# amazon-science/instruct-video-to-video

Hardware: AMD Instinct MI355X
Metric: denoised video-frames/sec (16f@256x384, 50 DDIM steps) (higher is better)
Workload: dtype fp16; 1 GPU; C2: 1 clip/step = VAE-encode + 50 DDIM steps (3-way CFG, text 7.5 / video 1.5) + VAE-decode, 16 frames @ 256x384, random-init full-width UNet+VAE; 5 independent clips in flight per GPU (stacked into every UNet launch, B = 3 x clips); frames=16, height=256, width=384, ddim_steps=50, clips_per_gpu=5, parallelism=clip-parallel x1, one all_gather, hip_graph=True, cfg_branch_streams=False, concurrent_clips=5, clip_mode=stacked, driver_mode=False, full=False

## Files before the change

### include/insv2v_hip.h

```cpp
#ifndef INSV2V_HIP_H
#define INSV2V_HIP_H

#include <stdint.h>

#ifdef __cplusplus
extern "C" {
#endif

typedef void* insv2v_stream_t;

#define INSV2V_OK 0
#define INSV2V_EINVAL (-1)
#define INSV2V_EUNSUPPORTED (-2)

#define INSV2V_ACT_NONE 0
#define INSV2V_ACT_SILU 1
#define INSV2V_ACT_GEGLU 2
#define INSV2V_ACT_QUICK_GELU 3

#define INSV2V_ACT_RELU 4
#define INSV2V_ACT_SIGMOID 5
#define INSV2V_ACT_TANH 6

#define INSV2V_MODE_LINEAR 0
#define INSV2V_MODE_CONV3X3 1

int insv2v_abi_version(void);
int insv2v_init(void);

typedef struct insv2v_gemm_desc {
    const void* a;
    const void* a2;
    const void* w;
    void* c;
    const float* bias;
    const float* row_bias;
    const void* residual;
    const float* row_stats;
    const float* col_sum;
    int64_t lda, lda2, ldw, ldc, ldr, ld_rb;
    int64_t a_bs, w_bs, c_bs, r_bs;
    void* workspace;
    int64_t workspace_bytes;
    int32_t M, N, K;
    int32_t k_split;
    int32_t rows_per_group;
    int32_t rb_mod;
    int32_t act;
    int32_t c_fp32;
    int32_t mode;
    int32_t NB, IH, IW, OH, OW, Cin;
    int32_t stride, pad_t, pad_l, upsample;
    int32_t batch;
    int32_t tile;
    int32_t split_k;
    float alpha;
    const float* gn_ab;
    int32_t gn_images_per_sample;
    int32_t gn_silu;
    float* stats_out;
    float* stats_scratch;
    int32_t stats_parts;
    float ln_eps;
    int64_t w_group_stride;
    int32_t w_group_rows;
    int32_t reserved0;
} insv2v_gemm_desc;
int insv2v_gemm(const insv2v_gemm_desc* d, insv2v_stream_t stream);
int64_t insv2v_set_operand_window(int64_t bytes);
int insv2v_gemm_stats_parts(const insv2v_gemm_desc* d);
int insv2v_conv3x3_fuses_groupnorm(const insv2v_gemm_desc* d);

typedef struct insv2v_winograd_in_desc {
    const void* x;
    const void* x2;
    const float* gn_ab;
    void* v;
    int64_t ldx, ldx2;
    int64_t v_group_rows;
    int32_t NB, H, W, C, C1;
    int32_t gn_images_per_sample;
    int32_t gn_silu;
    int32_t upsample;
} insv2v_winograd_in_desc;
int insv2v_winograd_input(const insv2v_winograd_in_desc* d, insv2v_stream_t stream);
typedef struct insv2v_winograd_out_desc {
    const void* m;
    const float* bias;
    const float* row_bias;
    const void* residual;
    void* y;
    int64_t m_group_rows;
    int64_t ldr, ldy, ld_rb;
    int32_t NB, H, W, Cout;
    int32_t rows_per_group;
    int32_t upsample;
} insv2v_winograd_out_desc;
int insv2v_winograd_output(const insv2v_winograd_out_desc* d, insv2v_stream_t stream);

typedef struct insv2v_ffn_desc {
    const void* x;
    void* out;
    const void* wstream;
    int64_t ldx, ldo;
    int32_t M, C, hidden;
    float eps;
    const void* post_residual;
    int64_t ld_post;
    int32_t post;
} insv2v_ffn_desc;
int insv2v_ffn_fused(const insv2v_ffn_desc* d, insv2v_stream_t stream);
int64_t insv2v_ffn_stream_elems(int32_t C, int32_t hidden, int32_t post);

typedef struct insv2v_rowlin_desc {
    const void* x;
    void* out;
    const void* residual;
    const void* wstream;
    int64_t ldx, ldo, ldr;
    int32_t M, N, K;
    int32_t layernorm, frame_bias, rows_per_frame, frames;
    float eps;
    float* stats_out;
    float stats_eps;
    const float* gn_ab;
    int32_t gn_rows;
} insv2v_rowlin_desc;
int insv2v_rowlin(const insv2v_rowlin_desc* d, insv2v_stream_t stream);
int64_t insv2v_rowlin_stream_elems(int32_t N, int32_t K);

typedef struct insv2v_tattn_desc {
    const void* x;
    void* out;
    const void* wstream;
    int64_t ldx, ldo;
    int32_t samples, HW, C, heads, frames;
    float eps;
    float scale;
} insv2v_tattn_desc;
int insv2v_tattn_fused(const insv2v_tattn_desc* d, insv2v_stream_t stream);
int64_t insv2v_tattn_stream_elems(int32_t C, int32_t heads, int32_t frames);
int insv2v_tattn_attn(const insv2v_tattn_desc* d, insv2v_stream_t stream);
int64_t insv2v_tattn_attn_stream_elems(int32_t C, int32_t heads, int32_t frames);

typedef struct insv2v_xattn_desc {
    const void* x;
    void* out;
    const void* wstream;
    const void* kvstream;
    int64_t ldx, ldo;
    int32_t M, rows_per_sample, C, heads, ctx_len;
    float eps;
    float scale;
    const void* pre_residual;
    int64_t ld_pre;
} insv2v_xattn_desc;
int insv2v_xattn_fused(const insv2v_xattn_desc* d, insv2v_stream_t stream);
int64_t insv2v_xattn_stream_elems(int32_t C, int32_t heads, int32_t per_sample_kv);
int insv2v_xattn_attn(const insv2v_xattn_desc* d, insv2v_stream_t stream);
int64_t insv2v_xattn_attn_stream_elems(int32_t C, int32_t heads, int32_t per_sample_kv);

typedef struct insv2v_groupnorm_desc {
    const void* x;
    const void* x2;
    void* y;
    const float* gamma;
    const float* beta;
    float* partials;
    int64_t ldx, ldx2, ldy;
    int32_t nsamples, rows_per_sample, C, C1, G;
    int32_t nchunks;
    int32_t silu;
    float eps;
    float* ab;
    int32_t stats_only;
} insv2v_groupnorm_desc;
int insv2v_groupnorm(const insv2v_groupnorm_desc* d, insv2v_stream_t stream);

typedef struct insv2v_layernorm_desc {
    const void* x;
    void* y;
    const float* gamma;
    const float* beta;
    const float* pe;
    int64_t ldx, ldy;
    int32_t rows, C;
    int32_t rows_per_frame, frames, pe_start;
    float eps;
} insv2v_layernorm_desc;
int insv2v_layernorm(const insv2v_layernorm_desc* d, insv2v_stream_t stream);
int insv2v_layernorm_stats(const void* x, float* stats, int64_t ldx, int32_t rows, int32_t C, float eps,
                           insv2v_stream_t stream);

typedef struct insv2v_attention_desc {
    const void* q;
    const void* k;
    const void* v;
    void* o;
    int64_t q_rs, k_rs, v_rs, o_rs;
    int64_t q_outer, q_step, kv_outer, kv_step, o_outer, o_step;
    int32_t q_inner, kv_inner, o_inner;
    int32_t batch, heads, head_dim, seq_q, seq_k;
    float scale;
    int32_t causal;
    const void* q_bias;
    const void* k_bias;
    const void* v_bias;
    int64_t bias_rs;
} insv2v_attention_desc;
int insv2v_attention(const insv2v_attention_desc* d, insv2v_stream_t stream);

int insv2v_embed_tokens(const int64_t* ids, const void* tok, const void* pos, void* out, int32_t rows, int32_t L,
                        int32_t C, int32_t vocab, insv2v_stream_t stream);

int insv2v_softmax_rows(const void* x, void* y, int64_t ldx, int64_t ldy, int32_t rows, int32_t cols,
                        float scale, insv2v_stream_t stream);
int insv2v_softmax_rows_padded(const void* x, void* y, int64_t ldx, int64_t ldy, int32_t rows, int32_t cols, int32_t valid,
                               float scale, insv2v_stream_t stream);

int insv2v_timestep_embedding(const float* t, void* out, int32_t batch, int32_t dim, float shift,
                              insv2v_stream_t stream);

int insv2v_tap_gather(const float* y9, int64_t ld9, const float* bias, float* out, int64_t ldo, int32_t NB, int32_t H, int32_t W,
                      int32_t cout, insv2v_stream_t stream);

int insv2v_build_unet_input(const float* latent, const float* img_cond, void* out, float* t_out,
                            float timestep, int32_t nbranch, int32_t F, int32_t h, int32_t w, int32_t ldo,
                            int64_t branch_rows, int32_t t_stride, insv2v_stream_t stream);

typedef struct insv2v_step_desc {
    const float* eps_in;
    const float* latent;
    const float* latent_ref;
    const float* delta_q;
    const float* noise;
    const float* rescale_stats;
    float* latent_out;
    float* pred_x0;
    float* eps_out;
    int32_t nbranch, F, h, w, R;
    int32_t correct;
    float text_cfg, img_cfg;
    float sqrt_a, sqrt_1ma;
    float c_x0, c_eps, c_xt, c_noise;
    float guidance_rescale;
    int64_t branch_stride;
    int64_t noise_seed, noise_stream;
    int32_t noise_on;
} insv2v_step_desc;
int insv2v_cfg_step(const insv2v_step_desc* d, insv2v_stream_t stream);
typedef struct insv2v_mstep_desc {
    const float* eps_in;
    const float* latent;
    const float* latent_ref;
    const float* delta_q;
    const float* noise;
    const float* rescale_stats;
    float* latent_out;
    float* pred_x0;
    float* eps_out;
    int32_t nbranch, F, h, w, R;
    int32_t correct;
    float text_cfg, img_cfg;
    float sqrt_a, sqrt_1ma;
    float c_x0, c_eps, c_xt, c_noise;
    float guidance_rescale;
    int64_t branch_stride;
    int64_t noise_seed, noise_stream;
    int32_t noise_on;
    const float* x0_hist;
    float c_hist;
} insv2v_mstep_desc;
int insv2v_cfg_step_ms(const insv2v_mstep_desc* d, insv2v_stream_t stream);
int insv2v_cfg_stats(const float* eps_in, float* stats, int32_t F, int32_t h, int32_t w, float text_cfg,
                     float img_cfg, int64_t branch_stride, insv2v_stream_t stream);

int insv2v_warp_image(const float* image, const float* flow, float* out, int32_t N, int32_t C, int32_t H,
                      int32_t W, insv2v_stream_t stream);
int insv2v_resize_flow(const float* flow, float* out, int32_t N, int32_t h, int32_t w, int32_t H, int32_t W,
                       insv2v_stream_t stream);
int insv2v_flow_correction(const float* eps_cfg, const float* latent, const float* latent_ref,
                           const float* flows, float* delta_q, int32_t F, int32_t R, int32_t h, int32_t w,
                           float sqrt_a, float sqrt_1ma, insv2v_stream_t stream);

int insv2v_nchw_to_nhwc_f16(const float* x, void* y, int32_t N, int32_t C, int32_t H, int32_t W, int32_t ldo,
                            float scale, insv2v_stream_t stream);
int insv2v_nhwc_to_nchw_f32(const void* x, int32_t x_is_fp32, float* y, int32_t N, int32_t C, int32_t H,
                            int32_t W, int32_t ldx, float scale, insv2v_stream_t stream);
int insv2v_posterior_sample(const float* moments, const float* noise, float* z, int32_t N, int32_t H,
                            int32_t W, int32_t ldm, float scale, insv2v_stream_t stream);
int insv2v_posterior_sample_seeded(const float* moments, float* z, int32_t N, int32_t H, int32_t W, int32_t ldm, float scale,
                                   int64_t seed, int64_t stream, int64_t offset, insv2v_stream_t hip_stream);

int insv2v_randn(float* out, int64_t n, int64_t seed, int64_t stream, int64_t offset, int32_t raw, insv2v_stream_t hip_stream);

typedef struct insv2v_im2col_desc {
    const void* x;
    const void* x2;
    void* out;
    int64_t ldx, ldx2, ldo;
    int32_t N, IH, IW, C, C1, KH, KW, stride_h, stride_w, pad_h, pad_w, OH, OW;
} insv2v_im2col_desc;
int insv2v_im2col(const insv2v_im2col_desc* d, insv2v_stream_t stream);
int insv2v_instance_norm(const void* x, void* y, float* partials, int32_t N, int32_t HW, int32_t C, int64_t ldx, int64_t ldy,
                         int32_t nchunks, float eps, int32_t relu, insv2v_stream_t stream);
#define INSV2V_EW_RELU 1
#define INSV2V_EW_ADD_RELU 2
#define INSV2V_EW_TANH 3
#define INSV2V_EW_GRU_RH 4
#define INSV2V_EW_GRU_OUT 5
int insv2v_ew(int32_t op, const void* a, const void* b, const void* c, void* out, int64_t rows, int32_t C, int64_t lda, int64_t ldb,
              int64_t ldc, int64_t ldo, insv2v_stream_t stream);
int insv2v_avgpool2x2(const float* x, float* y, int64_t n, int32_t h, int32_t w, insv2v_stream_t stream);
typedef struct insv2v_corr_lookup_desc {
    const float* pyr0;
    const float* pyr1;
    const float* pyr2;
    const float* pyr3;
    const float* coords;
    void* out;
    int64_t ldo;
    int32_t B, h, w, levels, radius;
} insv2v_corr_lookup_desc;
int insv2v_corr_lookup(const insv2v_corr_lookup_desc* d, insv2v_stream_t stream);
int insv2v_raft_flow_rows(float* coords1, const float* delta, int64_t ldd, void* rows, int64_t ldf, int32_t ncols, int32_t B, int32_t h,
                          int32_t w, insv2v_stream_t stream);
int insv2v_convex_upsample(const float* coords1, const void* mask, int64_t ldm, float* out, int32_t B, int32_t h, int32_t w,
                           insv2v_stream_t stream);

#ifdef __cplusplus
}
#endif
#endif
```

### instruct-video-to-video_amd/build.py

```python
#!/usr/bin/env python3
import os
import subprocess
import sys
from concurrent.futures import ThreadPoolExecutor

HERE = os.path.dirname(os.path.abspath(__file__))
CSRC = os.path.join(HERE, "csrc")
OUT = os.path.join(HERE, "insv2v", "libinsv2v_hip.so")
SOURCES = ["gemm.hip", "gemm_q8.hip", "gemm_r8.hip", "gemm_w4.hip", "rows_ffn.hip", "rows_tattn.hip", "rows_xattn.hip", "norm.hip", "attention.hip", "elementwise.hip", "raft.hip", "winograd.hip"]
FLAGS = ["--offload-arch=gfx950", "-O3", "-std=c++17", "-fPIC", "-Wall", "-Wno-unused-function"]
EXTRA_FLAGS = {src: ["-fno-slp-vectorize"] for src in ("gemm_q8.hip", "gemm_r8.hip", "gemm_w4.hip", "rows_ffn.hip", "rows_tattn.hip", "rows_xattn.hip")}


def _newer(a, b):
    return not os.path.exists(b) or os.path.getmtime(a) > os.path.getmtime(b)


def build(force=False, verbose=True):
    hipcc = os.environ.get("HIPCC", "/opt/rocm/bin/hipcc")
    objdir = os.path.join(HERE, "build")
    os.makedirs(objdir, exist_ok=True)
    deps = [os.path.join(CSRC, "common.h"), os.path.join(CSRC, "gemm_dma.h"), os.path.join(CSRC, "rows_common.h"), os.path.join(CSRC, "rng.h"), os.path.join(HERE, "..", "include", "insv2v_hip.h")]
    jobs = []
    for src in SOURCES:
        s, o = os.path.join(CSRC, src), os.path.join(objdir, src + ".o")
        if force or _newer(s, o) or any(_newer(d, o) for d in deps):
            jobs.append([hipcc, *FLAGS, *EXTRA_FLAGS.get(src, []), "-c", s, "-o", o])
    def run(cmd):
        if verbose:
            print(" ".join(cmd), flush=True)
        subprocess.check_call(cmd)
    with ThreadPoolExecutor(max_workers=4) as ex:
        list(ex.map(run, jobs))
    objs = [os.path.join(objdir, s + ".o") for s in SOURCES]
    if jobs or not os.path.exists(OUT) or any(_newer(o, OUT) for o in objs):
        run([hipcc, "--offload-arch=gfx950", "-shared", "-fPIC", *objs, "-o", OUT])
    return OUT


if __name__ == "__main__":
    print(build(force="--force" in sys.argv))
```

### instruct-video-to-video_amd/csrc/norm.hip

```cpp
#include "common.h"
#include <cstdlib>

struct Moments {
    float n, mean, m2;
};
__device__ __forceinline__ Moments merge(Moments a, Moments b) {
    if (b.n == 0.f) return a;
    if (a.n == 0.f) return b;
    Moments r;
    r.n = a.n + b.n;
    float d = b.mean - a.mean;
    r.mean = a.mean + d * (b.n / r.n);
    r.m2 = a.m2 + b.m2 + d * d * (a.n * b.n / r.n);
    return r;
}

__device__ __forceinline__ half8 load8(const half_t* x, const half_t* x2, int64_t ldx, int64_t ldx2, int C1,
                                       int64_t row, int c0) {
    const half_t* p = (c0 < C1) ? x + row * ldx + c0 : x2 + row * ldx2 + (c0 - C1);
    return *(const half8*)p;
}

__global__ void gn_partial_kernel(insv2v_groupnorm_desc p, int CC, int P, int rows_per_chunk) {
    extern __shared__ __attribute__((aligned(16))) char smem[];
    Moments* sm = (Moments*)smem;
    const int tid = threadIdx.x, cc = tid % CC, pl = tid / CC;
    const int sample = blockIdx.y, chunk = blockIdx.x;
    const int C1 = p.x2 ? p.C1 : p.C;
    const half_t* x = (const half_t*)p.x;
    const half_t* x2 = (const half_t*)p.x2;
    const int64_t row0 = (int64_t)sample * p.rows_per_sample;
    const int r0 = chunk * rows_per_chunk;
    const int r1 = min(r0 + rows_per_chunk, p.rows_per_sample);
    const int c0 = cc * 8;

    half8 kv = load8(x, x2, p.ldx, p.ldx2, C1, row0, c0);
    float k[8], s[8], q[8];
#pragma unroll
    for (int e = 0; e < 8; ++e) { k[e] = (float)kv[e]; s[e] = 0.f; q[e] = 0.f; }
    int cnt = 0;
    int r = r0 + pl;
    for (; r + 3 * P < r1; r += 4 * P) {
        half8 v[4];
#pragma unroll
        for (int u = 0; u < 4; ++u) v[u] = load8(x, x2, p.ldx, p.ldx2, C1, row0 + r + u * P, c0);
#pragma unroll
        for (int u = 0; u < 4; ++u)
#pragma unroll
            for (int e = 0; e < 8; ++e) {
                float d = (float)v[u][e] - k[e];
                s[e] += d;
                q[e] += d * d;
            }
        cnt += 4;
    }
    for (; r < r1; r += P) {
        half8 v = load8(x, x2, p.ldx, p.ldx2, C1, row0 + r, c0);
#pragma unroll
        for (int e = 0; e < 8; ++e) {
            float d = (float)v[e] - k[e];
            s[e] += d;
            q[e] += d * d;
        }
        ++cnt;
    }
#pragma unroll
    for (int e = 0; e < 8; ++e) {
        Moments m;
        m.n = (float)cnt;
        float inv = cnt ? 1.f / cnt : 0.f;
        m.mean = k[e] + s[e] * inv;
        m.m2 = fmaxf(q[e] - s[e] * s[e] * inv, 0.f);
        sm[pl * p.C + c0 + e] = m;
    }
    __syncthreads();
    for (int c = tid; c < p.C; c += blockDim.x) {
        Moments m = sm[c];
        for (int j = 1; j < P; ++j) m = merge(m, sm[j * p.C + c]);
        sm[c] = m;
    }
    __syncthreads();
    const int cpg = p.C / p.G;
    for (int g = tid; g < p.G; g += blockDim.x) {
        Moments m = sm[g * cpg];
        for (int j = 1; j < cpg; ++j) m = merge(m, sm[g * cpg + j]);
        float* out = p.partials + (int64_t)p.nsamples * p.G * 2 +
                     (((int64_t)sample * p.nchunks + chunk) * p.G + g) * 3;
        out[0] = m.n;
        out[1] = m.mean;
        out[2] = m.m2;
    }
}

__global__ __launch_bounds__(256) void gn_finalize_kernel(insv2v_groupnorm_desc p) {
    const int lane = threadIdx.x & 63, wid = threadIdx.x >> 6;
    const int sample = blockIdx.y, g = blockIdx.x * 4 + wid;
    if (g >= p.G) return;
    const float* in = p.partials + (int64_t)p.nsamples * p.G * 2 + ((int64_t)sample * p.nchunks * p.G + g) * 3;
    Moments m = {0.f, 0.f, 0.f};
    for (int c = lane; c < p.nchunks; c += 64) {
        const float* q = in + (int64_t)c * p.G * 3;
        Moments b = {q[0], q[1], q[2]};
        m = merge(m, b);
    }
#pragma unroll
    for (int o = 32; o > 0; o >>= 1) {
        Moments b = {__shfl_xor(m.n, o, 64), __shfl_xor(m.mean, o, 64), __shfl_xor(m.m2, o, 64)};
        m = merge(m, b);
    }
    if (lane == 0) {
        float var = m.m2 / m.n;
        p.partials[((int64_t)sample * p.G + g) * 2 + 0] = m.mean;
        p.partials[((int64_t)sample * p.G + g) * 2 + 1] = rsqrtf(var + p.eps);
    }
    if (p.ab) {
        const float mean = m.mean, rstd = rsqrtf(m.m2 / m.n + p.eps);
        const int cpg = p.C / p.G;
        for (int c = lane; c < cpg; c += 64) {
            const int ch = g * cpg + c;
            const float a = rstd * p.gamma[ch];
            p.ab[((int64_t)sample * p.C + ch) * 2 + 0] = a;
            p.ab[((int64_t)sample * p.C + ch) * 2 + 1] = p.beta[ch] - mean * a;
        }
    }
}

__global__ void gn_apply_kernel(insv2v_groupnorm_desc p, int CC, int P) {
    const int tid = threadIdx.x, cc = tid % CC, pl = tid / CC;
    const int sample = blockIdx.y;
    const int C1 = p.x2 ? p.C1 : p.C;
    const half_t* x = (const half_t*)p.x;
    const half_t* x2 = (const half_t*)p.x2;
    half_t* y = (half_t*)p.y;
    const int64_t row0 = (int64_t)sample * p.rows_per_sample;
    const int c0 = cc * 8, cpg = p.C / p.G;
    float a[8], b[8];
#pragma unroll
    for (int e = 0; e < 8; ++e) {
        int c = c0 + e, g = c / cpg;
        float mean = p.partials[((int64_t)sample * p.G + g) * 2 + 0];
        float rstd = p.partials[((int64_t)sample * p.G + g) * 2 + 1];
        a[e] = rstd * p.gamma[c];
        b[e] = p.beta[c] - mean * a[e];
    }
    const int step = gridDim.x * P;
    int r = blockIdx.x * P + pl;
    auto finish = [&](half8 v, int row) {
        half8 o;
#pragma unroll
        for (int e = 0; e < 8; ++e) {
            float t = (float)v[e] * a[e] + b[e];
            if (p.silu) t = silu_f(t);
            o[e] = (half_t)t;
        }
        *(half8*)(y + (row0 + row) * p.ldy + c0) = o;
    };
    for (; r + 3 * step < p.rows_per_sample; r += 4 * step) {
        half8 v[4];
#pragma unroll
        for (int u = 0; u < 4; ++u) v[u] = load8(x, x2, p.ldx, p.ldx2, C1, row0 + r + u * step, c0);
#pragma unroll
        for (int u = 0; u < 4; ++u) finish(v[u], r + u * step);
    }
    for (; r < p.rows_per_sample; r += step) finish(load8(x, x2, p.ldx, p.ldx2, C1, row0 + r, c0), r);
}

#define GNS_MAXCH 16
template <int VW>
__global__ __launch_bounds__(256) void gn_small_kernel(insv2v_groupnorm_desc p) {
    typedef half_t vec_t __attribute__((ext_vector_type(VW)));
    __shared__ float red[8];
    __shared__ float sgam[256], sbet[256];
    const int tid = threadIdx.x, lane = tid & 63, wid = tid >> 6;
    const int g = blockIdx.x, sample = blockIdx.y;
    const int cpg = p.C / p.G, cpr = cpg / VW;
    const int nchunk = p.rows_per_sample * cpr;
    const int C1 = p.x2 ? p.C1 : p.C;
    const half_t* x = (const half_t*)p.x;
    const half_t* x2 = (const half_t*)p.x2;
    const int64_t row0 = (int64_t)sample * p.rows_per_sample;
    if (tid < cpg) { sgam[tid] = p.gamma[g * cpg + tid]; sbet[tid] = p.beta[g * cpg + tid]; }
    vec_t v[GNS_MAXCH];
    float s = 0.f;
    const int rs = tid < nchunk ? tid / cpr : 0, cs = tid < nchunk ? tid - rs * cpr : 0;
    const int dr = 256 / cpr, dc = 256 - dr * cpr;
    int rr = rs, cc = cs;
#pragma unroll
    for (int i = 0; i < GNS_MAXCH; ++i) {
        const bool ok = tid + 256 * i < nchunk;
        const int r = ok ? rr : rs, c0 = g * cpg + (ok ? cc : cs) * VW;
        const half_t* src = c0 < C1 ? x + (row0 + r) * p.ldx + c0 : x2 + (row0 + r) * p.ldx2 + (c0 - C1);
        v[i] = *(const vec_t*)src;
        rr += dr; cc += dc;
        if (cc >= cpr) { cc -= cpr; ++rr; }
    }
#pragma unroll
    for (int i = 0; i < GNS_MAXCH; ++i) {
        if (tid + 256 * i >= nchunk) {
#pragma unroll
            for (int e = 0; e < VW; ++e) v[i][e] = (half_t)0.f;
        }
#pragma unroll
        for (int e = 0; e < VW; ++e) s += (float)v[i][e];
    }
    s = wave_sum(s);
    if (lane == 0) red[wid] = s;
    __syncthreads();
    const float n = (float)p.rows_per_sample * cpg;
    const float mean = (red[0] + red[1] + red[2] + red[3]) / n;
    float q = 0.f;
#pragma unroll
    for (int i = 0; i < GNS_MAXCH; ++i) {
        if (tid + 256 * i < nchunk) {
#pragma unroll
            for (int e = 0; e < VW; ++e) {
                const float d = (float)v[i][e] - mean;
                q += d * d;
            }
        }
    }
    q = wave_sum(q);
    if (lane == 0) red[4 + wid] = q;
    __syncthreads();
    const float rstd = rsqrtf((red[4] + red[5] + red[6] + red[7]) / n + p.eps);
    half_t* y = (half_t*)p.y;
    rr = rs; cc = cs;
#pragma unroll
    for (int i = 0; i < GNS_MAXCH; ++i) {
        const int idx = tid + 256 * i;
        const int r = rr, c0 = g * cpg + cc * VW;
        rr += dr; cc += dc;
        if (cc >= cpr) { cc -= cpr; ++rr; }
        if (idx < nchunk) {
            vec_t o;
#pragma unroll
            for (int e = 0; e < VW; ++e) {
                float t = ((float)v[i][e] - mean) * rstd * sgam[c0 - g * cpg + e] + sbet[c0 - g * cpg + e];
                if (p.silu) t = silu_f(t);
                o[e] = (half_t)t;
            }
            *(vec_t*)(y + (row0 + r) * p.ldy + c0) = o;
        }
    }
}

#define GNF_MAXCH 15
template <int NT>
__global__ __launch_bounds__(NT) void gn_frame_kernel(insv2v_groupnorm_desc p) {
    extern __shared__ __attribute__((aligned(16))) char smem[];
    const int tid = threadIdx.x;
    const int sample = blockIdx.x;
    const int CS = gridDim.y, Cw = p.C / CS, Gw = p.G / CS, coff = blockIdx.y * Cw;
    const int crow = Cw >> 3;
    const int cpr = (p.C / p.G) >> 3;
    const int nchunk = p.rows_per_sample * crow;
    float* part = (float*)smem;
    float* gstat = part + nchunk;
    float* sgam = gstat + 2 * Gw;
    float* sbet = sgam + Cw;
    for (int c = tid; c < Cw; c += NT) { sgam[c] = p.gamma[coff + c]; sbet[c] = p.beta[coff + c]; }
    const half_t* x = (const half_t*)p.x + (int64_t)sample * p.rows_per_sample * p.ldx + coff;
    half_t* y = (half_t*)p.y + (int64_t)sample * p.rows_per_sample * p.ldy + coff;
    const int r0 = tid / crow, c0 = tid - r0 * crow;
    const int dr = NT / crow, dc = NT - dr * crow;
    half8 v[GNF_MAXCH];
    {
        int rr = r0, cc = c0;
#pragma unroll
        for (int i = 0; i < GNF_MAXCH; ++i) {
            const bool ok = tid + NT * i < nchunk;
            v[i] = *(const half8*)(x + (int64_t)(ok ? rr : r0) * p.ldx + (ok ? cc : c0) * 8);
            rr += dr; cc += dc;
            if (cc >= crow) { cc -= crow; ++rr; }
        }
    }
    const int TPG = NT / Gw;
    const int rg = tid / TPG, rp = tid - rg * TPG;
    const int ng = p.rows_per_sample * cpr;
    const float inv_n = 1.f / ((float)p.rows_per_sample * (float)(p.C / p.G));
    auto group_total = [&]() {
        float s = 0.f;
        for (int e = rp; e < ng; e += TPG) {
            const int r = e / cpr, j = e - r * cpr;
            s += part[r * crow + rg * cpr + j];
        }
        for (int o = TPG >> 1; o > 0; o >>= 1) s += __shfl_xor(s, o, 64);
        return s;
    };
#pragma unroll
    for (int i = 0; i < GNF_MAXCH; ++i) {
        if (tid + NT * i < nchunk) {
            float s = 0.f;
#pragma unroll
            for (int e = 0; e < 8; ++e) s += (float)v[i][e];
            part[tid + NT * i] = s;
        }
    }
    __syncthreads();
    {
        const float m = group_total() * inv_n;
        if (rp == 0) gstat[rg] = m;
    }
    __syncthreads();
    {
        int cc = c0;
#pragma unroll
        for (int i = 0; i < GNF_MAXCH; ++i) {
            if (tid + NT * i < nchunk) {
                const float m = gstat[cc / cpr];
                float q = 0.f;
#pragma unroll
                for (int e = 0; e < 8; ++e) { const float d = (float)v[i][e] - m; q = fmaf(d, d, q); }
                part[tid + NT * i] = q;
            }
            cc += dc;
            if (cc >= crow) cc -= crow;
        }
    }
    __syncthreads();
    {
        const float var = group_total() * inv_n;
        if (rp == 0) gstat[Gw + rg] = rsqrtf(var + p.eps);
    }
    __syncthreads();
    {
        int rr = r0, cc = c0;
#pragma unroll
        for (int i = 0; i < GNF_MAXCH; ++i) {
            if (tid + NT * i < nchunk) {
                const int g = cc / cpr;
                const float m = gstat[g], rs = gstat[Gw + g];
                half8 o;
#pragma unroll
                for (int e = 0; e < 8; ++e) {
                    float t = ((float)v[i][e] - m) * rs * sgam[cc * 8 + e] + sbet[cc * 8 + e];
                    if (p.silu) t = silu_f(t);
                    o[e] = (half_t)t;
                }
                *(half8*)(y + (int64_t)rr * p.ldy + cc * 8) = o;
            }
            rr += dr; cc += dc;
            if (cc >= crow) { cc -= crow; ++rr; }
        }
    }
}

template <int NT>
static int launch_gn_frame(const insv2v_groupnorm_desc& d, hipStream_t s, int CS = 1) {
    const size_t lds = ((size_t)d.rows_per_sample * (d.C / CS / 8) + 2 * (d.G / CS) + 2 * (d.C / CS)) * sizeof(float);
    static bool attr_set = false;
    if (!attr_set) {
        hipError_t e = hipFuncSetAttribute((const void*)gn_frame_kernel<NT>, hipFuncAttributeMaxDynamicSharedMemorySize, 96 * 1024);
        if (e != hipSuccess) return (int)e;
        attr_set = true;
    }
    if (lds > 96 * 1024) return INSV2V_EUNSUPPORTED;
    hipLaunchKernelGGL(gn_frame_kernel<NT>, dim3(d.nsamples, CS), dim3(NT), lds, s, d);
    return launch_status();
}

extern "C" int insv2v_groupnorm(const insv2v_groupnorm_desc* dp, insv2v_stream_t stream) {
    if (!one_device()) return INSV2V_EINVAL;
    if (!dp) return INSV2V_EINVAL;
    insv2v_groupnorm_desc d = *dp;
    if (!d.x || !d.gamma || !d.beta || !d.partials) return INSV2V_EINVAL;
    if (d.stats_only ? !d.ab : !d.y) return INSV2V_EINVAL;
    if (d.C <= 0 || d.G <= 0 || (d.C % d.G) || (d.C & 7) || d.C > 8192) return INSV2V_EINVAL;
    if ((d.ldx & 7) || (d.ldy & 7) || d.nsamples <= 0 || d.rows_per_sample <= 0) return INSV2V_EINVAL;
    if (d.x2 && ((d.C1 & 7) || d.C1 <= 0 || d.C1 >= d.C || (d.ldx2 & 7))) return INSV2V_EINVAL;
    if (d.nchunks <= 0) return INSV2V_EINVAL;
    hipStream_t s = as_stream(stream);
    {
        static const int frame_on = getenv("INSV2V_GN_FRAME") ? atoi(getenv("INSV2V_GN_FRAME")) : 1;
        const int cpg = d.C / d.G;
        const int64_t nchunk = (int64_t)d.rows_per_sample * (d.C / 8);
        if (frame_on && !d.stats_only && !d.ab && !d.x2 && (cpg % 8) == 0 && d.nsamples >= 128 && nchunk >= 2048 && nchunk <= 1024 * GNF_MAXCH &&
            (d.G == 32 || d.G == 16) && d.C <= 2560) {
            static const int split_env = getenv("INSV2V_GN_FRAME_SPLIT") ? atoi(getenv("INSV2V_GN_FRAME_SPLIT")) : 0;
            int CS = split_env > 0 ? split_env : (nchunk > 512 * GNF_MAXCH ? 4 : nchunk > 256 * GNF_MAXCH ? 2 : 1);
            while (CS > 1 && (d.G % CS || nchunk / CS < 1024)) CS >>= 1;
            const int64_t nc = nchunk / CS;
            const int rc = nc <= 256 * GNF_MAXCH ? launch_gn_frame<256>(d, s, CS) : nc <= 512 * GNF_MAXCH ? launch_gn_frame<512>(d, s, CS) : launch_gn_frame<1024>(d, s, CS);
            if (rc != INSV2V_EUNSUPPORTED) return rc;
        }
    }
    {
        const int cpg = d.C / d.G;
        const int vw = (cpg % 8 == 0) ? 8 : ((cpg % 4 == 0) ? 4 : 0);
        const bool src_ok = !d.x2 || (d.C1 % (vw ? vw : 1) == 0);
        if (!d.stats_only && !d.ab && vw && cpg >= 16 && cpg <= 256 && src_ok && (int64_t)d.rows_per_sample * (cpg / vw) <= 256 * GNS_MAXCH) {
            if (vw == 8) hipLaunchKernelGGL(gn_small_kernel<8>, dim3(d.G, d.nsamples), dim3(256), 0, s, d);
            else hipLaunchKernelGGL(gn_small_kernel<4>, dim3(d.G, d.nsamples), dim3(256), 0, s, d);
            return launch_status();
        }
    }
    const int CC = d.C / 8;
    if (CC > 1024) return INSV2V_EUNSUPPORTED;
    int P = 256 / CC;
    if (P < 1) P = 1;
    if (P > 16) P = 16;
    const int threads = CC * P;
    int nchunks = d.nchunks;
    if (nchunks > d.rows_per_sample) nchunks = d.rows_per_sample;
    d.nchunks = nchunks;
    const int rows_per_chunk = (d.rows_per_sample + nchunks - 1) / nchunks;
    size_t lds = (size_t)P * d.C * sizeof(Moments);
    if (lds > 64 * 1024) return INSV2V_EUNSUPPORTED;
    hipLaunchKernelGGL(gn_partial_kernel, dim3(nchunks, d.nsamples), dim3(threads), lds, s, d, CC, P, rows_per_chunk);
    hipLaunchKernelGGL(gn_finalize_kernel, dim3((d.G + 3) / 4, d.nsamples), dim3(256), 0, s, d);
    if (d.stats_only) return launch_status();
    long want = ((long)d.rows_per_sample + P * 4 - 1) / (P * 4);
    long cap = 4096 / d.nsamples;
    if (cap < 1) cap = 1;
    int gx = (int)(want < cap ? want : cap);
    hipLaunchKernelGGL(gn_apply_kernel, dim3(gx, d.nsamples), dim3(threads), 0, s, d, CC, P);
    return launch_status();
}

#define LN_MAXCH 4
#define LN_ROWS 4
template <int NCH>
__global__ __launch_bounds__(256) void layernorm_kernel(insv2v_layernorm_desc p) {
    const int lane = threadIdx.x & 63, wid = threadIdx.x >> 6;
    const int row0 = (blockIdx.x * 4 + wid) * LN_ROWS;
    if (row0 >= p.rows) return;
    const int CC = p.C >> 3;
    half8 v[LN_ROWS][NCH];
#pragma unroll
    for (int r = 0; r < LN_ROWS; ++r) {
        const int row = min(row0 + r, p.rows - 1);
        const half_t* x = (const half_t*)p.x + (int64_t)row * p.ldx;
#pragma unroll
        for (int i = 0; i < NCH; ++i) {
            const int ch = lane + 64 * i;
            const half8 z = {0, 0, 0, 0, 0, 0, 0, 0};
            const half8 t = *(const half8*)(x + (ch < CC ? ch : 0) * 8);
            v[r][i] = ch < CC ? t : z;
        }
    }
    float mean[LN_ROWS], rstd[LN_ROWS];
#pragma unroll
    for (int r = 0; r < LN_ROWS; ++r) {
        float s = 0.f;
#pragma unroll
        for (int i = 0; i < NCH; ++i)
#pragma unroll
            for (int e = 0; e < 8; ++e) s += (float)v[r][i][e];
        mean[r] = s;
    }
#pragma unroll
    for (int o = 32; o > 0; o >>= 1)
#pragma unroll
        for (int r = 0; r < LN_ROWS; ++r) mean[r] += __shfl_xor(mean[r], o, 64);
#pragma unroll
    for (int r = 0; r < LN_ROWS; ++r) {
        mean[r] /= p.C;
        float s = 0.f;
#pragma unroll
        for (int i = 0; i < NCH; ++i) {
            if (lane + 64 * i < CC) {
#pragma unroll
                for (int e = 0; e < 8; ++e) {
                    float d = (float)v[r][i][e] - mean[r];
                    s += d * d;
                }
            }
        }
        rstd[r] = s;
    }
#pragma unroll
    for (int o = 32; o > 0; o >>= 1)
#pragma unroll
        for (int r = 0; r < LN_ROWS; ++r) rstd[r] += __shfl_xor(rstd[r], o, 64);
#pragma unroll
    for (int r = 0; r < LN_ROWS; ++r) rstd[r] = rsqrtf(rstd[r] / p.C + p.eps);
#pragma unroll
    for (int i = 0; i < NCH; ++i) {
        const int ch = lane + 64 * i;
        if (ch >= CC) continue;
        float g[8], b[8];
        const float4 g0 = *(const float4*)(p.gamma + ch * 8), g1 = *(const float4*)(p.gamma + ch * 8 + 4);
        const float4 b0 = *(const float4*)(p.beta + ch * 8), b1 = *(const float4*)(p.beta + ch * 8 + 4);
        g[0] = g0.x; g[1] = g0.y; g[2] = g0.z; g[3] = g0.w; g[4] = g1.x; g[5] = g1.y; g[6] = g1.z; g[7] = g1.w;
        b[0] = b0.x; b[1] = b0.y; b[2] = b0.z; b[3] = b0.w; b[4] = b1.x; b[5] = b1.y; b[6] = b1.z; b[7] = b1.w;
#pragma unroll
        for (int r = 0; r < LN_ROWS; ++r) {
            const int row = row0 + r;
            if (row >= p.rows) break;
            const float* pe = p.pe ? p.pe + (int64_t)((row / p.rows_per_frame) % p.frames + p.pe_start) * p.C + ch * 8 : nullptr;
            half8 o;
#pragma unroll
            for (int e = 0; e < 8; ++e) {
                float t = ((float)v[r][i][e] - mean[r]) * rstd[r] * g[e] + b[e];
                if (pe) t += pe[e];
                o[e] = (half_t)t;
            }
            *(half8*)((half_t*)p.y + (int64_t)row * p.ldy + ch * 8) = o;
        }
    }
}

template <int NCH>
__global__ __launch_bounds__(256) void ln_stats_kernel(const half_t* xp, float* stats, int64_t ldx, int rows, int C, float eps) {
    const int lane = threadIdx.x & 63, wid = threadIdx.x >> 6;
    const int row0 = (blockIdx.x * 4 + wid) * LN_ROWS;
    if (row0 >= rows) return;
    const int CC = C >> 3;
    half8 v[LN_ROWS][NCH];
#pragma unroll
    for (int r = 0; r < LN_ROWS; ++r) {
        const half_t* x = xp + (int64_t)min(row0 + r, rows - 1) * ldx;
#pragma unroll
        for (int i = 0; i < NCH; ++i) {
            const int ch = lane + 64 * i;
            const half8 z = {0, 0, 0, 0, 0, 0, 0, 0};
            const half8 t = *(const half8*)(x + (ch < CC ? ch : 0) * 8);
            v[r][i] = ch < CC ? t : z;
        }
    }
    float mean[LN_ROWS], var[LN_ROWS];
#pragma unroll
    for (int r = 0; r < LN_ROWS; ++r) {
        float s = 0.f;
#pragma unroll
        for (int i = 0; i < NCH; ++i)
#pragma unroll
            for (int e = 0; e < 8; ++e) s += (float)v[r][i][e];
        mean[r] = s;
    }
#pragma unroll
    for (int o = 32; o > 0; o >>= 1)
#pragma unroll
        for (int r = 0; r < LN_ROWS; ++r) mean[r] += __shfl_xor(mean[r], o, 64);
#pragma unroll
    for (int r = 0; r < LN_ROWS; ++r) {
        mean[r] /= C;
        float s = 0.f;
#pragma unroll
        for (int i = 0; i < NCH; ++i) {
            if (lane + 64 * i < CC) {
#pragma unroll
                for (int e = 0; e < 8; ++e) {
                    const float d = (float)v[r][i][e] - mean[r];
                    s += d * d;
                }
            }
        }
        var[r] = s;
    }
#pragma unroll
    for (int o = 32; o > 0; o >>= 1)
#pragma unroll
        for (int r = 0; r < LN_ROWS; ++r) var[r] += __shfl_xor(var[r], o, 64);
    if (lane < LN_ROWS && row0 + lane < rows) {
        float m = mean[0], q = var[0];
#pragma unroll
        for (int r = 1; r < LN_ROWS; ++r)
            if (lane == r) { m = mean[r]; q = var[r]; }
        *(float2*)(stats + 2 * (int64_t)(row0 + lane)) = make_float2(m, rsqrtf(q / C + eps));
    }
}

extern "C" int insv2v_layernorm_stats(const void* x, float* stats, int64_t ldx, int32_t rows, int32_t C, float eps,
                                      insv2v_stream_t stream) {
    if (!x || !stats || rows <= 0 || (C & 7) || C <= 0 || C > 64 * 8 * LN_MAXCH || (ldx & 7)) return INSV2V_EINVAL;
    const int nch = (C / 8 + 63) / 64;
    dim3 grid((rows + 4 * LN_ROWS - 1) / (4 * LN_ROWS));
    hipStream_t s = as_stream(stream);
    const half_t* xp = (const half_t*)x;
    switch (nch) {
        case 1: hipLaunchKernelGGL(ln_stats_kernel<1>, grid, dim3(256), 0, s, xp, stats, ldx, rows, C, eps); break;
        case 2: hipLaunchKernelGGL(ln_stats_kernel<2>, grid, dim3(256), 0, s, xp, stats, ldx, rows, C, eps); break;
        case 3: hipLaunchKernelGGL(ln_stats_kernel<3>, grid, dim3(256), 0, s, xp, stats, ldx, rows, C, eps); break;
        default: hipLaunchKernelGGL(ln_stats_kernel<4>, grid, dim3(256), 0, s, xp, stats, ldx, rows, C, eps); break;
    }
    return launch_status();
}

extern "C" int insv2v_layernorm(const insv2v_layernorm_desc* dp, insv2v_stream_t stream) {
    if (!dp) return INSV2V_EINVAL;
    insv2v_layernorm_desc d = *dp;
    if (!d.x || !d.y || !d.gamma || !d.beta || d.rows <= 0) return INSV2V_EINVAL;
    if ((d.C & 7) || d.C <= 0 || d.C > 64 * 8 * LN_MAXCH || (d.ldx & 7) || (d.ldy & 7)) return INSV2V_EINVAL;
    if (d.pe && (d.rows_per_frame <= 0 || d.frames <= 0 || d.pe_start < 0)) return INSV2V_EINVAL;
    const int nch = (d.C / 8 + 63) / 64;
    dim3 grid((d.rows + 4 * LN_ROWS - 1) / (4 * LN_ROWS));
    hipStream_t s = as_stream(stream);
    switch (nch) {
        case 1: hipLaunchKernelGGL(layernorm_kernel<1>, grid, dim3(256), 0, s, d); break;
        case 2: hipLaunchKernelGGL(layernorm_kernel<2>, grid, dim3(256), 0, s, d); break;
        case 3: hipLaunchKernelGGL(layernorm_kernel<3>, grid, dim3(256), 0, s, d); break;
        default: hipLaunchKernelGGL(layernorm_kernel<4>, grid, dim3(256), 0, s, d); break;
    }
    return launch_status();
}

template <bool PAD>
__global__ __launch_bounds__(256) void softmax_rows_kernel(const half_t* x, half_t* y, int64_t ldx, int64_t ldy,
                                                           int cols, int valid, float scale) {
    __shared__ float red[8];
    const int row = blockIdx.x, tid = threadIdx.x, lane = tid & 63, wid = tid >> 6;
    const half_t* xr = x + (int64_t)row * ldx;
    half_t* yr = y + (int64_t)row * ldy;
    const int CC = cols >> 3;
    float mx = -3.0e38f;
    for (int ch = tid; ch < CC; ch += 256) {
        half8 v = *(const half8*)(xr + ch * 8);
#pragma unroll
        for (int e = 0; e < 8; ++e)
            if (!PAD || ch * 8 + e < valid) mx = fmaxf(mx, (float)v[e]);
    }
    mx = wave_max(mx);
    if (lane == 0) red[wid] = mx;
    __syncthreads();
    mx = fmaxf(fmaxf(red[0], red[1]), fmaxf(red[2], red[3]));
    const float c = scale * 1.4426950408889634f;
    float sum = 0.f;
    for (int ch = tid; ch < CC; ch += 256) {
        half8 v = *(const half8*)(xr + ch * 8);
#pragma unroll
        for (int e = 0; e < 8; ++e)
            if (!PAD || ch * 8 + e < valid) sum += exp2f(((float)v[e] - mx) * c);
    }
    sum = wave_sum(sum);
    if (lane == 0) red[4 + wid] = sum;
    __syncthreads();
    const float inv = 1.f / (red[4] + red[5] + red[6] + red[7]);
    for (int ch = tid; ch < CC; ch += 256) {
        half8 v = *(const half8*)(xr + ch * 8);
        half8 o;
#pragma unroll
        for (int e = 0; e < 8; ++e) o[e] = (!PAD || ch * 8 + e < valid) ? (half_t)(exp2f(((float)v[e] - mx) * c) * inv) : (half_t)0.f;
        *(half8*)(yr + ch * 8) = o;
    }
}

extern "C" int insv2v_softmax_rows(const void* x, void* y, int64_t ldx, int64_t ldy, int32_t rows, int32_t cols,
                                   float scale, insv2v_stream_t stream) {
    if (!x || !y || rows <= 0 || cols <= 0 || (cols & 7) || (ldx & 7) || (ldy & 7)) return INSV2V_EINVAL;
    if (scale < 0.f) return INSV2V_EINVAL;
    hipLaunchKernelGGL(softmax_rows_kernel<false>, dim3(rows), dim3(256), 0, as_stream(stream), (const half_t*)x,
                       (half_t*)y, ldx, ldy, cols, cols, scale);
    return launch_status();
}

extern "C" int insv2v_softmax_rows_padded(const void* x, void* y, int64_t ldx, int64_t ldy, int32_t rows, int32_t cols, int32_t valid,
                                          float scale, insv2v_stream_t stream) {
    if (!x || !y || rows <= 0 || cols <= 0 || (cols & 7) || (ldx & 7) || (ldy & 7) || ldx < cols || ldy < cols) return INSV2V_EINVAL;
    if (valid <= 0 || valid > cols || scale < 0.f) return INSV2V_EINVAL;
    hipLaunchKernelGGL(softmax_rows_kernel<true>, dim3(rows), dim3(256), 0, as_stream(stream), (const half_t*)x,
                       (half_t*)y, ldx, ldy, cols, valid, scale);
    return launch_status();
}
```

### instruct-video-to-video_amd/csrc/winograd.hip

```cpp
#include "common.h"

namespace {

template <bool UP> __device__ __forceinline__ int lds_px(int sp) { return UP ? sp : sp ^ ((sp >> 1) & 1); }

template <bool NORM, bool UP>
__global__ __launch_bounds__(256) void wino_input_kernel(const half_t* __restrict__ x, const half_t* __restrict__ x2, const float* __restrict__ ab,
                                                         half_t* __restrict__ V, int64_t ldx, int64_t ldx2, int C1, int C, int NB, int H, int W,
                                                         int ipb, int images_per_sample, int silu, int64_t group_rows, int band_tr) {
    extern __shared__ __attribute__((aligned(16))) char smem[];
    const int tid = threadIdx.x, chunk = tid & 7, item0 = tid >> 3;
    const int nb0 = (int)blockIdx.x * ipb, c0 = (int)blockIdx.y * 64;
    const int trows = UP ? H : (H + 1) >> 1;
    const int tr0 = (int)blockIdx.z * band_tr, tr1 = min(tr0 + band_tr, trows);
    const bool whole = band_tr >= trows;
    const int row0 = whole ? 0 : (UP ? tr0 - 1 : 2 * tr0 - 1);
    const int nrows = whole ? H : (UP ? (tr1 - tr0) + 2 : 2 * (tr1 - tr0) + 2);
    const int HW = H * W, SW = nrows * W;
    const int SWs = UP ? SW : (SW + 1) & ~1;
    const bool second = x2 != nullptr && c0 >= C1;
    const half_t* src = second ? x2 + (c0 - C1) + chunk * 8 : x + c0 + chunk * 8;
    const int64_t ld = second ? ldx2 : ldx;
    const int nimg = min(ipb, NB - nb0);
    for (int it = item0; it < nimg * SW; it += 32) {
        const int img = it / SW, sp = it - img * SW;
        const int iy = row0 + sp / W;
        if ((unsigned)iy >= (unsigned)H) continue;
        half8 v = *(const half8*)(src + ((int64_t)(nb0 + img) * HW + sp + row0 * W) * ld);
        if (NORM) {
            const float* p = ab + ((int64_t)((nb0 + img) / images_per_sample) * C + c0 + chunk * 8) * 2;
            const float4 p0 = *(const float4*)p, p1 = *(const float4*)(p + 4), p2 = *(const float4*)(p + 8), p3 = *(const float4*)(p + 12);
            const float sc[8] = {p0.x, p0.z, p1.x, p1.z, p2.x, p2.z, p3.x, p3.z}, sh[8] = {p0.y, p0.w, p1.y, p1.w, p2.y, p2.w, p3.y, p3.w};
#pragma unroll
            for (int e = 0; e < 8; ++e) {
                float f = fmaf((float)v[e], sc[e], sh[e]);
                if (silu) f = silu_f(f);
                v[e] = (half_t)f;
            }
        }
        *(half8*)(smem + ((int64_t)img * SWs + lds_px<UP>(sp)) * 128 + chunk * 16) = v;
    }
    __syncthreads();
    if constexpr (UP) {
        const int bt = (tr1 - tr0) * W;
        for (int it = item0; it < nimg * bt; it += 32) {
            const int img = it / bt, tb_ = it - img * bt;
            const int y = tr0 + tb_ / W, xx = tb_ - (tb_ / W) * W;
            const int t = y * W + xx;
            const char* base = smem + (int64_t)img * SWs * 128 + chunk * 16;
            float hz[3][3][8];
#pragma unroll
            for (int r = 0; r < 3; ++r) {
                const int iy = y - 1 + r;
                float d[3][8];
#pragma unroll
                for (int c = 0; c < 3; ++c) {
                    const int ix = xx - 1 + c;
                    const bool ok = (unsigned)iy < (unsigned)H && (unsigned)ix < (unsigned)W;
                    half8 v = {0, 0, 0, 0, 0, 0, 0, 0};
                    if (ok) v = *(const half8*)(base + lds_px<UP>((iy - row0) * W + ix) * 128);
#pragma unroll
                    for (int e = 0; e < 8; ++e) d[c][e] = (float)v[e];
                }
#pragma unroll
                for (int e = 0; e < 8; ++e) {
                    hz[r][0][e] = d[0][e] - d[1][e];
                    hz[r][1][e] = 2.f * d[1][e];
                    hz[r][2][e] = d[1][e] - d[2][e];
                }
            }
            const int64_t trow = (int64_t)(nb0 + img) * HW + t;
            half_t* dst = V + trow * C + c0 + chunk * 8;
#pragma unroll
            for (int j = 0; j < 3; ++j) {
                half8 o[3];
#pragma unroll
                for (int e = 0; e < 8; ++e) {
                    o[0][e] = (half_t)(hz[0][j][e] - hz[1][j][e]);
                    o[1][e] = (half_t)(2.f * hz[1][j][e]);
                    o[2][e] = (half_t)(hz[1][j][e] - hz[2][j][e]);
                }
#pragma unroll
                for (int i = 0; i < 3; ++i) *(half8*)(dst + (int64_t)(i * 3 + j) * group_rows * C) = o[i];
            }
        }
        return;
    }
    const int th = (H + 1) >> 1, tw = (W + 1) >> 1, ntile = th * tw;
    const int bt = (tr1 - tr0) * tw;
    for (int it = item0; it < nimg * bt; it += 32) {
        const int img = it / bt, tb_ = it - img * bt;
        const int ty = tr0 + tb_ / tw, tx = tb_ - (tb_ / tw) * tw;
        const int t = ty * tw + tx;
        const char* base = smem + (int64_t)img * SWs * 128 + chunk * 16;
        float hz[4][4][8];
#pragma unroll
        for (int r = 0; r < 4; ++r) {
            const int iy = 2 * ty - 1 + r;
            float d[4][8];
#pragma unroll
            for (int c = 0; c < 4; ++c) {
                const int ix = 2 * tx - 1 + c;
                const bool ok = (unsigned)iy < (unsigned)H && (unsigned)ix < (unsigned)W;
                half8 v = {0, 0, 0, 0, 0, 0, 0, 0};
                if (ok) v = *(const half8*)(base + lds_px<UP>((iy - row0) * W + ix) * 128);
#pragma unroll
                for (int e = 0; e < 8; ++e) d[c][e] = (float)v[e];
            }
#pragma unroll
            for (int e = 0; e < 8; ++e) {
                hz[r][0][e] = d[0][e] - d[2][e];
                hz[r][1][e] = d[1][e] + d[2][e];
                hz[r][2][e] = d[2][e] - d[1][e];
                hz[r][3][e] = d[1][e] - d[3][e];
            }
        }
        const int64_t trow = (int64_t)(nb0 + img) * ntile + t;
        half_t* dst = V + trow * C + c0 + chunk * 8;
#pragma unroll
        for (int j = 0; j < 4; ++j) {
            half8 o[4];
#pragma unroll
            for (int e = 0; e < 8; ++e) {
                o[0][e] = (half_t)(hz[0][j][e] - hz[2][j][e]);
                o[1][e] = (half_t)(hz[1][j][e] + hz[2][j][e]);
                o[2][e] = (half_t)(hz[2][j][e] - hz[1][j][e]);
                o[3][e] = (half_t)(hz[1][j][e] - hz[3][j][e]);
            }
#pragma unroll
            for (int i = 0; i < 4; ++i) *(half8*)(dst + (int64_t)(i * 4 + j) * group_rows * C) = o[i];
        }
    }
}

template <bool RES, bool RB, bool UP>
__global__ __launch_bounds__(256) void wino_output_kernel(const half_t* __restrict__ Mo, const float* __restrict__ bias, const float* __restrict__ row_bias,
                                                          const half_t* __restrict__ res, half_t* __restrict__ y, int64_t group_rows, int64_t ntiles_total,
                                                          int Cout, int H, int W, int64_t ld_rb, int rows_per_group, int64_t ldr, int64_t ldy) {
    const int c8 = Cout >> 3;
    const int64_t idx = (int64_t)blockIdx.x * 256 + threadIdx.x;
    const int64_t tile = idx / c8;
    if (tile >= ntiles_total) return;
    const int ch = (int)(idx - tile * c8) * 8;
    const int th = UP ? H : (H + 1) >> 1, tw = UP ? W : (W + 1) >> 1, ntile = th * tw;
    const int OW = UP ? 2 * W : W, OH = UP ? 2 * H : H;
    const int nb = (int)(tile / ntile), t = (int)(tile - (int64_t)nb * ntile);
    const int ty = t / tw, tx = t - ty * tw;
    const half_t* src = Mo + tile * Cout + ch;
    float s[2][4][8];
    if constexpr (UP) {
#pragma unroll
        for (int j = 0; j < 3; ++j) {
            half8 m[3];
#pragma unroll
            for (int i = 0; i < 3; ++i) m[i] = *(const half8*)(src + (int64_t)(i * 3 + j) * group_rows * Cout);
            const int jj = j == 2 ? 3 : j;
#pragma unroll
            for (int e = 0; e < 8; ++e) {
                s[0][jj][e] = (float)m[0][e] + (float)m[1][e];
                s[1][jj][e] = (float)m[1][e] - (float)m[2][e];
            }
        }
#pragma unroll
        for (int e = 0; e < 8; ++e) s[0][2][e] = s[1][2][e] = 0.f;
    } else {
#pragma unroll
        for (int j = 0; j < 4; ++j) {
            half8 m[4];
#pragma unroll
            for (int i = 0; i < 4; ++i) m[i] = *(const half8*)(src + (int64_t)(i * 4 + j) * group_rows * Cout);
#pragma unroll
            for (int e = 0; e < 8; ++e) {
                s[0][j][e] = (float)m[0][e] + (float)m[1][e] + (float)m[2][e];
                s[1][j][e] = (float)m[1][e] - (float)m[2][e] - (float)m[3][e];
            }
        }
    }
    float b[8];
    {
        const float4 b0 = bias ? *(const float4*)(bias + ch) : make_float4(0.f, 0.f, 0.f, 0.f), b1 = bias ? *(const float4*)(bias + ch + 4) : make_float4(0.f, 0.f, 0.f, 0.f);
        b[0] = b0.x; b[1] = b0.y; b[2] = b0.z; b[3] = b0.w; b[4] = b1.x; b[5] = b1.y; b[6] = b1.z; b[7] = b1.w;
    }
    const int64_t m00 = ((int64_t)nb * OH + 2 * ty) * OW + 2 * tx;
    if (RB) {
        const float* rb = row_bias + (m00 / rows_per_group) * ld_rb + ch;
        const float4 r0 = *(const float4*)rb, r1 = *(const float4*)(rb + 4);
        b[0] += r0.x; b[1] += r0.y; b[2] += r0.z; b[3] += r0.w; b[4] += r1.x; b[5] += r1.y; b[6] += r1.z; b[7] += r1.w;
    }
#pragma unroll
    for (int i = 0; i < 2; ++i)
#pragma unroll
        for (int jj = 0; jj < 2; ++jj) {
            if (!UP && (2 * ty + i >= OH || 2 * tx + jj >= OW)) continue;
            const int64_t m = m00 + (int64_t)i * OW + jj;
            float v[8];
#pragma unroll
            for (int e = 0; e < 8; ++e)
                v[e] = (jj == 0 ? s[i][0][e] + s[i][1][e] + s[i][2][e] : s[i][1][e] - s[i][2][e] - s[i][3][e]) + b[e];
            if (RES) {
                const half8 r = *(const half8*)(res + m * ldr + ch);
#pragma unroll
                for (int e = 0; e < 8; ++e) v[e] += (float)r[e];
            }
            half8 o;
#pragma unroll
            for (int e = 0; e < 8; ++e) o[e] = (half_t)v[e];
            *(half8*)(y + m * ldy + ch) = o;
        }
}

}

extern "C" int insv2v_winograd_input(const insv2v_winograd_in_desc* dp, insv2v_stream_t stream) {
    if (!dp) return INSV2V_EINVAL;
    const insv2v_winograd_in_desc& d = *dp;
    if (!d.x || !d.v || d.NB <= 0 || d.H <= 0 || d.W <= 0 || d.C <= 0) return INSV2V_EINVAL;
    if ((d.C % 64) || (d.x2 && (d.C1 <= 0 || d.C1 >= d.C || (d.C1 % 64)))) return INSV2V_EUNSUPPORTED;
    if ((d.ldx & 7) || ((uintptr_t)d.x & 15) || ((uintptr_t)d.v & 15) || (d.x2 && ((d.ldx2 & 7) || ((uintptr_t)d.x2 & 15)))) return INSV2V_EINVAL;
    if (d.gn_ab && (d.gn_images_per_sample <= 0 || ((uintptr_t)d.gn_ab & 15))) return INSV2V_EINVAL;
    const int HW = d.H * d.W, ntile = d.upsample ? HW : ((d.H + 1) / 2) * ((d.W + 1) / 2);
    const int HWs = d.upsample ? HW : (HW + 1) & ~1;
    const int64_t tiles = (int64_t)d.NB * ntile;
    if (d.v_group_rows < tiles) return INSV2V_EINVAL;
    const int trows = d.upsample ? d.H : (d.H + 1) / 2;
    int band_tr = trows, ipb = 1;
    if (HWs * 128 <= 64 * 1024) {
        ipb = 32 / ntile;
        if (ipb < 1) ipb = 1;
        while (ipb > 1 && ipb * HWs * 128 > 64 * 1024) --ipb;
    } else {
        const int max_rows = 64 * 1024 / (d.W * 128);
        band_tr = d.upsample ? max_rows - 2 : (max_rows - 2) / 2;
        if (band_tr < 1) return INSV2V_EUNSUPPORTED;
    }
    const int nbands = (trows + band_tr - 1) / band_tr;
    const int srows = nbands == 1 ? d.H : (d.upsample ? band_tr + 2 : 2 * band_tr + 2);
    const dim3 grid((unsigned)((d.NB + ipb - 1) / ipb), (unsigned)(d.C / 64), (unsigned)nbands);
    const int slots = srows * d.W;
    const size_t lds = (size_t)ipb * (d.upsample ? slots : (slots + 1) & ~1) * 128;
#define WINO_IN(NORM, UP)                                                                                                                             \
    hipLaunchKernelGGL((wino_input_kernel<NORM, UP>), grid, dim3(256), lds, as_stream(stream), (const half_t*)d.x, (const half_t*)d.x2, d.gn_ab, (half_t*)d.v, \
                       d.ldx, d.ldx2, d.x2 ? d.C1 : d.C, d.C, d.NB, d.H, d.W, ipb, d.gn_ab ? d.gn_images_per_sample : 1, d.gn_ab ? d.gn_silu : 0, d.v_group_rows, band_tr)
    if (d.gn_ab) { if (d.upsample) WINO_IN(true, true); else WINO_IN(true, false); }
    else { if (d.upsample) WINO_IN(false, true); else WINO_IN(false, false); }
#undef WINO_IN
    return launch_status();
}

extern "C" int insv2v_winograd_output(const insv2v_winograd_out_desc* dp, insv2v_stream_t stream) {
    if (!dp) return INSV2V_EINVAL;
    const insv2v_winograd_out_desc& d = *dp;
    if (!d.m || !d.y || d.NB <= 0 || d.H <= 0 || d.W <= 0 || d.Cout <= 0) return INSV2V_EINVAL;
    if (d.Cout & 7) return INSV2V_EUNSUPPORTED;
    if ((d.ldy & 7) || ((uintptr_t)d.m & 15) || ((uintptr_t)d.y & 15) || (d.residual && ((d.ldr & 7) || ((uintptr_t)d.residual & 15)))) return INSV2V_EINVAL;
    if ((d.bias && ((uintptr_t)d.bias & 15)) || (d.row_bias && (((uintptr_t)d.row_bias & 15) || (d.ld_rb & 3) || d.rows_per_group <= 0 || d.rows_per_group % (d.H * d.W * (d.upsample ? 4 : 1)))))
        return INSV2V_EINVAL;
    const int64_t tiles = d.upsample ? (int64_t)d.NB * d.H * d.W : (int64_t)d.NB * ((d.H + 1) / 2) * ((d.W + 1) / 2);
    if (d.m_group_rows < tiles) return INSV2V_EINVAL;
    const int64_t n = tiles * (d.Cout / 8);
    const dim3 grid((unsigned)((n + 255) / 256));
#define WINO_OUT(RES, RB, UP)                                                                                                                        \
    hipLaunchKernelGGL((wino_output_kernel<RES, RB, UP>), grid, dim3(256), 0, as_stream(stream), (const half_t*)d.m, d.bias, d.row_bias, (const half_t*)d.residual, \
                       (half_t*)d.y, d.m_group_rows, tiles, d.Cout, d.H, d.W, d.ld_rb, d.rows_per_group, d.ldr, d.ldy)
    if (d.upsample) {
        if (d.residual) { if (d.row_bias) WINO_OUT(true, true, true); else WINO_OUT(true, false, true); }
        else { if (d.row_bias) WINO_OUT(false, true, true); else WINO_OUT(false, false, true); }
    } else {
        if (d.residual) { if (d.row_bias) WINO_OUT(true, true, false); else WINO_OUT(true, false, false); }
        else { if (d.row_bias) WINO_OUT(false, true, false); else WINO_OUT(false, false, false); }
    }
#undef WINO_OUT
    return launch_status();
}
```

### instruct-video-to-video_amd/insv2v/_lib.py

```python
import ctypes as C
import os

import torch

ABI_VERSION = 14
_HERE = os.path.dirname(os.path.abspath(__file__))
LIB_PATH = os.environ.get("INSV2V_LIB", os.path.join(_HERE, "libinsv2v_hip.so"))

c_i32, c_i64, c_f32, c_p = C.c_int32, C.c_int64, C.c_float, C.c_void_p


class GemmDesc(C.Structure):
    _fields_ = [("a", c_p), ("a2", c_p), ("w", c_p), ("c", c_p), ("bias", c_p), ("row_bias", c_p), ("residual", c_p),
                ("row_stats", c_p), ("col_sum", c_p),
                ("lda", c_i64), ("lda2", c_i64), ("ldw", c_i64), ("ldc", c_i64), ("ldr", c_i64), ("ld_rb", c_i64),
                ("a_bs", c_i64), ("w_bs", c_i64), ("c_bs", c_i64), ("r_bs", c_i64),
                ("workspace", c_p), ("workspace_bytes", c_i64),
                ("M", c_i32), ("N", c_i32), ("K", c_i32), ("k_split", c_i32), ("rows_per_group", c_i32),
                ("rb_mod", c_i32), ("act", c_i32), ("c_fp32", c_i32), ("mode", c_i32),
                ("NB", c_i32), ("IH", c_i32), ("IW", c_i32), ("OH", c_i32), ("OW", c_i32), ("Cin", c_i32),
                ("stride", c_i32), ("pad_t", c_i32), ("pad_l", c_i32), ("upsample", c_i32),
                ("batch", c_i32), ("tile", c_i32), ("split_k", c_i32), ("alpha", c_f32),
                ("gn_ab", c_p), ("gn_images_per_sample", c_i32), ("gn_silu", c_i32),
                ("stats_out", c_p), ("stats_scratch", c_p), ("stats_parts", c_i32), ("ln_eps", c_f32),
                ("w_group_stride", c_i64), ("w_group_rows", c_i32), ("reserved0", c_i32)]


class WinogradInDesc(C.Structure):
    _fields_ = [("x", c_p), ("x2", c_p), ("gn_ab", c_p), ("v", c_p), ("ldx", c_i64), ("ldx2", c_i64), ("v_group_rows", c_i64),
                ("NB", c_i32), ("H", c_i32), ("W", c_i32), ("C", c_i32), ("C1", c_i32), ("gn_images_per_sample", c_i32), ("gn_silu", c_i32), ("upsample", c_i32)]


class WinogradOutDesc(C.Structure):
    _fields_ = [("m", c_p), ("bias", c_p), ("row_bias", c_p), ("residual", c_p), ("y", c_p), ("m_group_rows", c_i64),
                ("ldr", c_i64), ("ldy", c_i64), ("ld_rb", c_i64), ("NB", c_i32), ("H", c_i32), ("W", c_i32), ("Cout", c_i32), ("rows_per_group", c_i32), ("upsample", c_i32)]


class FfnDesc(C.Structure):
    _fields_ = [("x", c_p), ("out", c_p), ("wstream", c_p), ("ldx", c_i64), ("ldo", c_i64),
                ("M", c_i32), ("C", c_i32), ("hidden", c_i32), ("eps", c_f32), ("post_residual", c_p), ("ld_post", c_i64), ("post", c_i32)]


class RowLinDesc(C.Structure):
    _fields_ = [("x", c_p), ("out", c_p), ("residual", c_p), ("wstream", c_p), ("ldx", c_i64), ("ldo", c_i64), ("ldr", c_i64),
                ("M", c_i32), ("N", c_i32), ("K", c_i32), ("layernorm", c_i32), ("frame_bias", c_i32), ("rows_per_frame", c_i32),
                ("frames", c_i32), ("eps", c_f32), ("stats_out", c_p), ("stats_eps", c_f32), ("gn_ab", c_p), ("gn_rows", c_i32)]


class TattnDesc(C.Structure):
    _fields_ = [("x", c_p), ("out", c_p), ("wstream", c_p), ("ldx", c_i64), ("ldo", c_i64),
                ("samples", c_i32), ("HW", c_i32), ("C", c_i32), ("heads", c_i32), ("frames", c_i32), ("eps", c_f32), ("scale", c_f32)]


class XattnDesc(C.Structure):
    _fields_ = [("x", c_p), ("out", c_p), ("wstream", c_p), ("kvstream", c_p), ("ldx", c_i64), ("ldo", c_i64),
                ("M", c_i32), ("rows_per_sample", c_i32), ("C", c_i32), ("heads", c_i32), ("ctx_len", c_i32), ("eps", c_f32), ("scale", c_f32),
                ("pre_residual", c_p), ("ld_pre", c_i64)]


class GroupNormDesc(C.Structure):
    _fields_ = [("x", c_p), ("x2", c_p), ("y", c_p), ("gamma", c_p), ("beta", c_p), ("partials", c_p),
                ("ldx", c_i64), ("ldx2", c_i64), ("ldy", c_i64),
                ("nsamples", c_i32), ("rows_per_sample", c_i32), ("C", c_i32), ("C1", c_i32), ("G", c_i32),
                ("nchunks", c_i32), ("silu", c_i32), ("eps", c_f32), ("ab", c_p), ("stats_only", c_i32)]


class LayerNormDesc(C.Structure):
    _fields_ = [("x", c_p), ("y", c_p), ("gamma", c_p), ("beta", c_p), ("pe", c_p),
                ("ldx", c_i64), ("ldy", c_i64), ("rows", c_i32), ("C", c_i32),
                ("rows_per_frame", c_i32), ("frames", c_i32), ("pe_start", c_i32), ("eps", c_f32)]


class AttentionDesc(C.Structure):
    _fields_ = [("q", c_p), ("k", c_p), ("v", c_p), ("o", c_p),
                ("q_rs", c_i64), ("k_rs", c_i64), ("v_rs", c_i64), ("o_rs", c_i64),
                ("q_outer", c_i64), ("q_step", c_i64), ("kv_outer", c_i64), ("kv_step", c_i64),
                ("o_outer", c_i64), ("o_step", c_i64),
                ("q_inner", c_i32), ("kv_inner", c_i32), ("o_inner", c_i32),
                ("batch", c_i32), ("heads", c_i32), ("head_dim", c_i32), ("seq_q", c_i32), ("seq_k", c_i32),
                ("scale", c_f32), ("causal", c_i32), ("q_bias", c_p), ("k_bias", c_p), ("v_bias", c_p), ("bias_rs", c_i64)]


class StepDesc(C.Structure):
    _fields_ = [("eps_in", c_p), ("latent", c_p), ("latent_ref", c_p), ("delta_q", c_p), ("noise", c_p),
                ("rescale_stats", c_p), ("latent_out", c_p), ("pred_x0", c_p), ("eps_out", c_p),
                ("nbranch", c_i32), ("F", c_i32), ("h", c_i32), ("w", c_i32), ("R", c_i32), ("correct", c_i32),
                ("text_cfg", c_f32), ("img_cfg", c_f32), ("sqrt_a", c_f32), ("sqrt_1ma", c_f32),
                ("c_x0", c_f32), ("c_eps", c_f32), ("c_xt", c_f32), ("c_noise", c_f32), ("guidance_rescale", c_f32),
                ("branch_stride", c_i64), ("noise_seed", c_i64), ("noise_stream", c_i64), ("noise_on", c_i32)]


class MStepDesc(C.Structure):
    _fields_ = StepDesc._fields_ + [("x0_hist", c_p), ("c_hist", c_f32)]


class Im2colDesc(C.Structure):
    _fields_ = [("x", c_p), ("x2", c_p), ("out", c_p), ("ldx", c_i64), ("ldx2", c_i64), ("ldo", c_i64),
                ("N", c_i32), ("IH", c_i32), ("IW", c_i32), ("C", c_i32), ("C1", c_i32), ("KH", c_i32), ("KW", c_i32),
                ("stride_h", c_i32), ("stride_w", c_i32), ("pad_h", c_i32), ("pad_w", c_i32), ("OH", c_i32), ("OW", c_i32)]


class CorrLookupDesc(C.Structure):
    _fields_ = [("pyr0", c_p), ("pyr1", c_p), ("pyr2", c_p), ("pyr3", c_p), ("coords", c_p), ("out", c_p), ("ldo", c_i64),
                ("B", c_i32), ("h", c_i32), ("w", c_i32), ("levels", c_i32), ("radius", c_i32)]


SIGNATURES = {
    "insv2v_abi_version": (c_i32, []),
    "insv2v_init": (c_i32, []),
    "insv2v_gemm": (c_i32, [C.POINTER(GemmDesc), c_p]),
    "insv2v_gemm_stats_parts": (c_i32, [C.POINTER(GemmDesc)]),
    "insv2v_set_operand_window": (c_i64, [c_i64]),
    "insv2v_conv3x3_fuses_groupnorm": (c_i32, [C.POINTER(GemmDesc)]),
    "insv2v_winograd_input": (c_i32, [C.POINTER(WinogradInDesc), c_p]),
    "insv2v_winograd_output": (c_i32, [C.POINTER(WinogradOutDesc), c_p]),
    "insv2v_ffn_fused": (c_i32, [C.POINTER(FfnDesc), c_p]),
    "insv2v_ffn_stream_elems": (c_i64, [c_i32, c_i32, c_i32]),
    "insv2v_rowlin": (c_i32, [C.POINTER(RowLinDesc), c_p]),
    "insv2v_rowlin_stream_elems": (c_i64, [c_i32, c_i32]),
    "insv2v_tattn_fused": (c_i32, [C.POINTER(TattnDesc), c_p]),
    "insv2v_tattn_stream_elems": (c_i64, [c_i32, c_i32, c_i32]),
    "insv2v_tattn_attn": (c_i32, [C.POINTER(TattnDesc), c_p]),
    "insv2v_tattn_attn_stream_elems": (c_i64, [c_i32, c_i32, c_i32]),
    "insv2v_xattn_fused": (c_i32, [C.POINTER(XattnDesc), c_p]),
    "insv2v_xattn_stream_elems": (c_i64, [c_i32, c_i32, c_i32]),
    "insv2v_xattn_attn": (c_i32, [C.POINTER(XattnDesc), c_p]),
    "insv2v_xattn_attn_stream_elems": (c_i64, [c_i32, c_i32, c_i32]),
    "insv2v_groupnorm": (c_i32, [C.POINTER(GroupNormDesc), c_p]),
    "insv2v_layernorm": (c_i32, [C.POINTER(LayerNormDesc), c_p]),
    "insv2v_layernorm_stats": (c_i32, [c_p, c_p, c_i64, c_i32, c_i32, c_f32, c_p]),
    "insv2v_attention": (c_i32, [C.POINTER(AttentionDesc), c_p]),
    "insv2v_embed_tokens": (c_i32, [c_p, c_p, c_p, c_p, c_i32, c_i32, c_i32, c_i32, c_p]),
    "insv2v_softmax_rows": (c_i32, [c_p, c_p, c_i64, c_i64, c_i32, c_i32, c_f32, c_p]),
    "insv2v_softmax_rows_padded": (c_i32, [c_p, c_p, c_i64, c_i64, c_i32, c_i32, c_i32, c_f32, c_p]),
    "insv2v_timestep_embedding": (c_i32, [c_p, c_p, c_i32, c_i32, c_f32, c_p]),
    "insv2v_build_unet_input": (c_i32, [c_p, c_p, c_p, c_p, c_f32, c_i32, c_i32, c_i32, c_i32, c_i32, c_i64, c_i32, c_p]),
    "insv2v_cfg_step": (c_i32, [C.POINTER(StepDesc), c_p]),
    "insv2v_cfg_step_ms": (c_i32, [C.POINTER(MStepDesc), c_p]),
    "insv2v_cfg_stats": (c_i32, [c_p, c_p, c_i32, c_i32, c_i32, c_f32, c_f32, c_i64, c_p]),
    "insv2v_warp_image": (c_i32, [c_p, c_p, c_p, c_i32, c_i32, c_i32, c_i32, c_p]),
    "insv2v_tap_gather": (c_i32, [c_p, c_i64, c_p, c_p, c_i64, c_i32, c_i32, c_i32, c_i32, c_p]),
    "insv2v_resize_flow": (c_i32, [c_p, c_p, c_i32, c_i32, c_i32, c_i32, c_i32, c_p]),
    "insv2v_flow_correction": (c_i32, [c_p, c_p, c_p, c_p, c_p, c_i32, c_i32, c_i32, c_i32, c_f32, c_f32, c_p]),
    "insv2v_nchw_to_nhwc_f16": (c_i32, [c_p, c_p, c_i32, c_i32, c_i32, c_i32, c_i32, c_f32, c_p]),
    "insv2v_nhwc_to_nchw_f32": (c_i32, [c_p, c_i32, c_p, c_i32, c_i32, c_i32, c_i32, c_i32, c_f32, c_p]),
    "insv2v_posterior_sample": (c_i32, [c_p, c_p, c_p, c_i32, c_i32, c_i32, c_i32, c_f32, c_p]),
    "insv2v_posterior_sample_seeded": (c_i32, [c_p, c_p, c_i32, c_i32, c_i32, c_i32, c_f32, c_i64, c_i64, c_i64, c_p]),
    "insv2v_randn": (c_i32, [c_p, c_i64, c_i64, c_i64, c_i64, c_i32, c_p]),
    "insv2v_im2col": (c_i32, [C.POINTER(Im2colDesc), c_p]),
    "insv2v_instance_norm": (c_i32, [c_p, c_p, c_p, c_i32, c_i32, c_i32, c_i64, c_i64, c_i32, c_f32, c_i32, c_p]),
    "insv2v_ew": (c_i32, [c_i32, c_p, c_p, c_p, c_p, c_i64, c_i32, c_i64, c_i64, c_i64, c_i64, c_p]),
    "insv2v_avgpool2x2": (c_i32, [c_p, c_p, c_i64, c_i32, c_i32, c_p]),
    "insv2v_corr_lookup": (c_i32, [C.POINTER(CorrLookupDesc), c_p]),
    "insv2v_raft_flow_rows": (c_i32, [c_p, c_p, c_i64, c_p, c_i64, c_i32, c_i32, c_i32, c_i32, c_p]),
    "insv2v_convex_upsample": (c_i32, [c_p, c_p, c_i64, c_p, c_i32, c_i32, c_i32, c_p]),
}

_lib = None


class HipKernelError(RuntimeError):
    pass


def load():
    global _lib
    if _lib is not None:
        return _lib
    if not os.path.exists(LIB_PATH):
        raise HipKernelError(
            f"{LIB_PATH} not found: build it with `python instruct-video-to-video_amd/build.py` "
            "(or __graft_entry__.build()). There is no CPU fallback for the insv2v hot path.")
    lib = C.CDLL(LIB_PATH)
    for name, (res, args) in SIGNATURES.items():
        fn = getattr(lib, name)
        fn.restype, fn.argtypes = res, args
    if lib.insv2v_abi_version() != ABI_VERSION:
        raise HipKernelError("libinsv2v_hip.so ABI version mismatch; rebuild the library")
    _lib = lib
    return lib


def check(status, what):
    if status != 0:
        kind = {-1: "invalid argument", -2: "unsupported configuration"}.get(status, f"hipError {status}")
        raise HipKernelError(f"{what}: {kind}")
```

### instruct-video-to-video_amd/insv2v/ops.py

```python
import ctypes as C

import os
import torch

from . import _lib
from .rng import as_int64
from ._lib import GemmDesc, GroupNormDesc, LayerNormDesc, AttentionDesc, StepDesc, MStepDesc, FfnDesc, RowLinDesc, TattnDesc, XattnDesc, WinogradInDesc, WinogradOutDesc, check

ACT_NONE, ACT_SILU, ACT_GEGLU, ACT_QUICK_GELU = 0, 1, 2, 3
ACT_RELU, ACT_SIGMOID, ACT_TANH = 4, 5, 6
EW_RELU, EW_ADD_RELU, EW_TANH, EW_GRU_RH, EW_GRU_OUT = 1, 2, 3, 4, 5
_byref = C.byref


def _stream():
    return torch.cuda.current_stream().cuda_stream


_REC = None


def set_launch_recorder(rec):
    global _REC
    _REC = rec
# ... 112 lines not shown
    elif row_stats is not None:
        d.row_stats = _req(row_stats, torch.float32, "gemm.row_stats").data_ptr()
        d.col_sum = _req(col_sum, torch.float32, "gemm.col_sum").data_ptr()
    d.rb_mod = rb_mod
    d.M, d.N, d.K, d.act, d.c_fp32, d.alpha, d.tile = M, N, K, act, int(out.dtype == torch.float32), alpha, tile
    d.batch, d.a_bs, d.w_bs, d.c_bs, d.r_bs = batch, a_bs, w_bs, c_bs, r_bs
    if batch == 1:
        ws = _workspace(a.device)
        d.workspace, d.workspace_bytes, d.split_k = ws.data_ptr(), ws.numel() * 4, split_k
    stats = None
    if emit_stats:
        key = (M, N, K, d.lda, d.ldc, d.ldr, residual is not None, act, tile, out.dtype, a.data_ptr() % 16, out.data_ptr() % 16, batch, split_k,
               residual.data_ptr() % 16 if residual is not None else 0,
               row_bias is not None, rows_per_group, d.ld_rb, rb_mod, a2 is not None, row_stats is not None)
        nparts = _STATS_PARTS_CACHE.get(key)
        if nparts is None:
            nparts = _STATS_PARTS_CACHE[key] = int(lib.insv2v_gemm_stats_parts(_byref(d)))
        if nparts > 0:
            stats = RowStats(torch.empty((nparts, M, 2), device=a.device, dtype=torch.float32), nparts, ln_eps)
            d.stats_out = stats.parts.data_ptr()
    with _timed("gemm_kernel", 2.0 * M * N * K * batch, ("lin", M, N, K, batch, act, residual is not None)):
        rc = lib.insv2v_gemm(_byref(d), _stream())
        if rc == -2 and stats is not None:
            stats, d.stats_out = None, None
            rc = lib.insv2v_gemm(_byref(d), _stream())
        check(rc, "insv2v_gemm")
    del scratch
    if emit_stats:
        return out, (stats if stats is not None else layernorm_stats(out, ln_eps))
    return out


def copy_rows(dst, src):
    with _timed("copy", 0.0, ("copy", src.shape[0], src.shape[1])):
        dst.copy_(src)
    return dst


def ffn_fused_supported(C, hidden):
    return int(_lib.load().insv2v_ffn_stream_elems(C, hidden, 0)) > 0


def ffn_fused(x, wstream, hidden, eps=1e-5, out=None, post_residual=None):
    lib = _lib.load()
    _req(x, torch.float16, "ffn.x"), _req(wstream, torch.float16, "ffn.wstream")
    M, C = x.shape
    if wstream.numel() != int(lib.insv2v_ffn_stream_elems(C, hidden, int(post_residual is not None))):
        raise _lib.HipKernelError(f"ffn_fused: weight stream of {wstream.numel()} halfs does not match C={C}, hidden={hidden}, post={post_residual is not None}")
    if out is None:
        out = torch.empty((M, C), device=x.device, dtype=torch.float16)
    d = FfnDesc()
    d.x, d.out, d.wstream, d.ldx, d.ldo = x.data_ptr(), out.data_ptr(), wstream.data_ptr(), x.stride(0), out.stride(0)
    d.M, d.C, d.hidden, d.eps = M, C, hidden, eps
    if post_residual is not None:
        d.post, d.post_residual, d.ld_post = 1, _req(post_residual, torch.float16, "ffn.post_residual").data_ptr(), post_residual.stride(0)
    with _timed("gemm_kernel", 2.0 * M * C * 3 * hidden + (2.0 * M * C * C if post_residual is not None else 0.0), ("ffn", M, C, hidden)):
        check(lib.insv2v_ffn_fused(_byref(d), _stream()), "insv2v_ffn_fused")
    return out


def rowlin_supported(N, K):
    return int(_lib.load().insv2v_rowlin_stream_elems(N, K)) > 0


def rowlin(x, wstream, N, *, layernorm=False, residual=None, frames=0, rows_per_frame=0, eps=1e-5, out=None, emit_stats=False, stats_eps=1e-5,
           gn_ab=None, gn_rows=0):
    lib = _lib.load()
    _req(x, torch.float16, "rowlin.x"), _req(wstream, torch.float16, "rowlin.wstream")
    M, K = x.shape
    if wstream.numel() != int(lib.insv2v_rowlin_stream_elems(N, K)):
        raise _lib.HipKernelError(f"rowlin: weight stream of {wstream.numel()} halfs does not match N={N}, K={K}")
    if out is None:
        out = torch.empty((M, N), device=x.device, dtype=torch.float16)
    d = RowLinDesc()
    d.x, d.out, d.wstream, d.ldx, d.ldo = x.data_ptr(), out.data_ptr(), wstream.data_ptr(), x.stride(0), out.stride(0)
    if residual is not None:
        d.residual, d.ldr = _req(residual, torch.float16, "rowlin.residual").data_ptr(), residual.stride(0)
    d.M, d.N, d.K, d.layernorm, d.eps = M, N, K, int(layernorm), eps
    d.frame_bias, d.rows_per_frame, d.frames = int(frames > 0), rows_per_frame, frames
    if gn_ab is not None:
        d.gn_ab, d.gn_rows = _req(gn_ab, torch.float32, "rowlin.gn_ab").data_ptr(), gn_rows
    stats = None
    if emit_stats:
        stats = torch.empty((M, 2), device=x.device, dtype=torch.float32)
        d.stats_out, d.stats_eps = stats.data_ptr(), stats_eps
    with _timed("gemm_kernel", 2.0 * M * N * K, ("rowlin", M, N, K, int(layernorm), residual is not None)):
        check(lib.insv2v_rowlin(_byref(d), _stream()), "insv2v_rowlin")
    return (out, stats) if emit_stats else out


def tattn_fused_supported(C, heads, frames):
    return int(_lib.load().insv2v_tattn_stream_elems(C, heads, frames)) > 0


def tattn_fused(x, wstream, samples, HW, heads, frames, eps=1e-5, out=None):
    lib = _lib.load()
    _req(x, torch.float16, "tattn.x"), _req(wstream, torch.float16, "tattn.wstream")
    M, C = x.shape
    if M != samples * frames * HW:
        raise _lib.HipKernelError(f"tattn_fused: {M} rows != {samples} samples x {frames} frames x {HW} pixels")
    if wstream.numel() != int(lib.insv2v_tattn_stream_elems(C, heads, frames)):
        raise _lib.HipKernelError(f"tattn_fused: weight stream of {wstream.numel()} halfs does not match C={C}, heads={heads}, frames={frames}")
    if out is None:
        out = torch.empty((M, C), device=x.device, dtype=torch.float16)
    d = TattnDesc()
    d.x, d.out, d.wstream, d.ldx, d.ldo = x.data_ptr(), out.data_ptr(), wstream.data_ptr(), x.stride(0), out.stride(0)
    d.samples, d.HW, d.C, d.heads, d.frames, d.eps, d.scale = samples, HW, C, heads, frames, eps, (C // heads) ** -0.5
    with _timed("gemm_kernel", 2.0 * M * C * 4 * C + 4.0 * M * frames * C, ("tattn", M, C, heads, frames)):
        check(lib.insv2v_tattn_fused(_byref(d), _stream()), "insv2v_tattn_fused")
    return out


def tattn_attn_supported(C, heads, frames):
    return int(_lib.load().insv2v_tattn_attn_stream_elems(C, heads, frames)) > 0


def tattn_attn(x, wstream, samples, HW, heads, frames, eps=1e-5, out=None):
    lib = _lib.load()
    _req(x, torch.float16, "tattn_attn.x"), _req(wstream, torch.float16, "tattn_attn.wstream")
    M, C = x.shape
    if M != samples * frames * HW:
        raise _lib.HipKernelError(f"tattn_attn: {M} rows != {samples} samples x {frames} frames x {HW} pixels")
    if wstream.numel() != int(lib.insv2v_tattn_attn_stream_elems(C, heads, frames)):
        raise _lib.HipKernelError(f"tattn_attn: weight stream of {wstream.numel()} halfs does not match C={C}, heads={heads}, frames={frames}")
    if out is None:
        out = torch.empty((M, C), device=x.device, dtype=torch.float16)
    d = TattnDesc()
    d.x, d.out, d.wstream, d.ldx, d.ldo = x.data_ptr(), out.data_ptr(), wstream.data_ptr(), x.stride(0), out.stride(0)
    d.samples, d.HW, d.C, d.heads, d.frames, d.eps, d.scale = samples, HW, C, heads, frames, eps, (C // heads) ** -0.5
    with _timed("gemm_kernel", 2.0 * M * C * 3 * C + 4.0 * M * frames * C, ("tattn_attn", M, C, heads, frames)):
        check(lib.insv2v_tattn_attn(_byref(d), _stream()), "insv2v_tattn_attn")
    return out


def xattn_fused_supported(C, heads, ctx_len, rows_per_sample):
    return int(_lib.load().insv2v_xattn_stream_elems(C, heads, 0)) > 0 and 64 < ctx_len <= 96 and rows_per_sample > 0


def xattn_fused(x, wstream, kvstream, rows_per_sample, heads, ctx_len, eps=1e-5, out=None, pre_residual=None):
    lib = _lib.load()
    _req(x, torch.float16, "xattn.x"), _req(wstream, torch.float16, "xattn.wstream"), _req(kvstream, torch.float16, "xattn.kvstream")
    M, C = x.shape
    if M % rows_per_sample or kvstream.shape[0] != M // rows_per_sample:
        raise _lib.HipKernelError(f"xattn_fused: {M} rows, {rows_per_sample} per sample, K/V streams of {kvstream.shape[0]} samples")
    if wstream.numel() != int(lib.insv2v_xattn_stream_elems(C, heads, 2 if pre_residual is not None else 0)) or \
            kvstream[0].numel() != int(lib.insv2v_xattn_stream_elems(C, heads, 1)):
        raise _lib.HipKernelError(f"xattn_fused: weight / K-V streams do not match C={C}, heads={heads}")
    if out is None:
        out = torch.empty((M, C), device=x.device, dtype=torch.float16)
    d = XattnDesc()
    d.x, d.out, d.wstream, d.kvstream, d.ldx, d.ldo = x.data_ptr(), out.data_ptr(), wstream.data_ptr(), kvstream.data_ptr(), x.stride(0), out.stride(0)
    d.M, d.rows_per_sample, d.C, d.heads, d.ctx_len, d.eps, d.scale = M, rows_per_sample, C, heads, ctx_len, eps, (C // heads) ** -0.5
    if pre_residual is not None:
        d.pre_residual, d.ld_pre = _req(pre_residual, torch.float16, "xattn.pre_residual").data_ptr(), pre_residual.stride(0)
    with _timed("gemm_kernel", (6.0 if pre_residual is not None else 4.0) * M * C * C + 4.0 * M * ctx_len * C, ("xattn", M, C, heads, ctx_len, pre_residual is not None)):
        check(lib.insv2v_xattn_fused(_byref(d), _stream()), "insv2v_xattn_fused")
    return out


def xattn_attn_supported(C, heads, ctx_len, rows_per_sample):
    return int(_lib.load().insv2v_xattn_attn_stream_elems(C, heads, 0)) > 0 and 64 < ctx_len <= 96 and rows_per_sample > 0


def xattn_attn(x, wstream, kvstream, rows_per_sample, heads, ctx_len, eps=1e-5, out=None):
    lib = _lib.load()
    _req(x, torch.float16, "xattn_attn.x"), _req(wstream, torch.float16, "xattn_attn.wstream"), _req(kvstream, torch.float16, "xattn_attn.kvstream")
    M, C = x.shape
    if M % rows_per_sample or kvstream.shape[0] != M // rows_per_sample:
        raise _lib.HipKernelError(f"xattn_attn: {M} rows, {rows_per_sample} per sample, K/V streams of {kvstream.shape[0]} samples")
    if wstream.numel() != int(lib.insv2v_xattn_attn_stream_elems(C, heads, 0)) or kvstream[0].numel() != int(lib.insv2v_xattn_attn_stream_elems(C, heads, 1)):
        raise _lib.HipKernelError(f"xattn_attn: weight / K-V streams do not match C={C}, heads={heads}")
    if out is None:
        out = torch.empty((M, C), device=x.device, dtype=torch.float16)
    d = XattnDesc()
    d.x, d.out, d.wstream, d.kvstream, d.ldx, d.ldo = x.data_ptr(), out.data_ptr(), wstream.data_ptr(), kvstream.data_ptr(), x.stride(0), out.stride(0)
    d.M, d.rows_per_sample, d.C, d.heads, d.ctx_len, d.eps, d.scale = M, rows_per_sample, C, heads, ctx_len, eps, (C // heads) ** -0.5
    with _timed("gemm_kernel", 2.0 * M * C * C + 4.0 * M * ctx_len * C, ("xattn_attn", M, C, heads, ctx_len)):
        check(lib.insv2v_xattn_attn(_byref(d), _stream()), "insv2v_xattn_attn")
    return out


def _conv_geometry(geom, stride, pad, upsample, out_size=None):
    NB, IH, IW = geom
    if out_size is not None:
        if not upsample:
            raise ValueError("conv3x3: out_size is the target of the nearest-x2 upsample (upsample=True)")
        return int(out_size[0]), int(out_size[1])
    IHu, IWu = (IH * 2, IW * 2) if upsample else (IH, IW)
    pt, pl = pad
    if pt == 0 and stride == 2:
        return (IHu + 1 - 3) // 2 + 1, (IWu + 1 - 3) // 2 + 1
    return (IHu + 2 * pt - 3) // stride + 1, (IWu + 2 * pl - 3) // stride + 1


_FUSE_CACHE = {}


class operand_window:

    def __init__(self, nbytes):
        self.nbytes = int(nbytes)

    def __enter__(self):
        self.prev = int(_lib.load().insv2v_set_operand_window(self.nbytes))
        _STATS_PARTS_CACHE.clear()

    def __exit__(self, *exc):
        _lib.load().insv2v_set_operand_window(self.prev)
        _STATS_PARTS_CACHE.clear()
        return False


def tap_weights(w):
    cout, cin = w.shape[:2]
    if cout > 4 or tuple(w.shape[2:]) != (3, 3):
        raise ValueError(f"tap_weights: a 3x3 convolution with <= 4 output channels, got {tuple(w.shape)}")
    wt = torch.zeros(40, cin, dtype=torch.float32)
    wt[:36].reshape(9, 4, cin)[:, :cout] = w.detach().float().cpu().permute(2, 3, 0, 1).reshape(9, cout, cin)
    return wt.half()


def conv3x3_narrow(x, geom, wtap, bias, cout):
    lib = _lib.load()
    NB, H, W = geom
    y9 = gemm(x, wtap, None, out_fp32=True)
    out = torch.empty((x.shape[0], cout), device=x.device, dtype=torch.float32)
    with _timed("elementwise", 0.0, ("tapgather", x.shape[0], cout)):
        check(lib.insv2v_tap_gather(y9.data_ptr(), y9.stride(0), _ptr(bias), out.data_ptr(), out.stride(0), NB, H, W, cout, _stream()), "insv2v_tap_gather")
    return out


def conv3x3_fuses_groupnorm(geom, cin, cout, k_split=0):
    key = (tuple(geom), cin, cout, k_split)
    if key not in _FUSE_CACHE:
        lib = _lib.load()
        NB, IH, IW = geom
        d = GemmDesc()
        d.M, d.N, d.K, d.batch, d.mode = NB * IH * IW, cout, 9 * cin, 1, 1
        d.NB, d.IH, d.IW, d.OH, d.OW, d.Cin = NB, IH, IW, IH, IW, cin
        d.stride, d.pad_t, d.pad_l, d.k_split = 1, 1, 1, k_split
        d.workspace, d.workspace_bytes = 1, WORKSPACE_BYTES
        _FUSE_CACHE[key] = bool(lib.insv2v_conv3x3_fuses_groupnorm(_byref(d)))
    return _FUSE_CACHE[key]


def conv3x3(x, geom, w, bias=None, *, x2=None, stride=1, pad=(1, 1), upsample=False, residual=None, row_bias=None,
            rows_per_group=0, out_fp32=False, tile=0, split_k=0, gn_ab=None, gn_images_per_sample=0, gn_silu=False, out=None, act=ACT_NONE,
            out_size=None):
    lib = _lib.load()
    _req(x, torch.float16, "conv.x"), _req(w, torch.float16, "conv.w")
    NB, IH, IW = geom
    pt, pl = pad
    OH, OW = _conv_geometry(geom, stride, pad, upsample, out_size)
    N = w.shape[0]
    cin = x.shape[1] + (x2.shape[1] if x2 is not None else 0)
    M = NB * OH * OW
    if out is None:
        out = torch.empty((M, N), device=x.device, dtype=torch.float32 if out_fp32 else torch.float16)
    d = GemmDesc()
    d.a, d.w, d.c = x.data_ptr(), w.data_ptr(), out.data_ptr()
    d.lda, d.ldw, d.ldc = x.stride(0), w.stride(0), out.stride(0)
    if x2 is not None:
        d.a2, d.lda2, d.k_split = _req(x2, torch.float16, "conv.x2").data_ptr(), x2.stride(0), x.shape[1]
    if bias is not None:
        d.bias = _req(bias, torch.float32, "conv.bias").data_ptr()
    if row_bias is not None:
        d.row_bias, d.ld_rb, d.rows_per_group = _req(row_bias, torch.float32, "conv.row_bias").data_ptr(), row_bias.stride(0), rows_per_group
    if residual is not None:
        d.residual, d.ldr = _req(residual, torch.float16, "conv.residual").data_ptr(), residual.stride(0)
    d.M, d.N, d.K, d.c_fp32, d.alpha, d.tile, d.batch, d.act = M, N, 9 * cin, int(out_fp32), 1.0, tile, 1, act
    d.mode, d.NB, d.IH, d.IW, d.OH, d.OW, d.Cin = 1, NB, IH, IW, OH, OW, cin
    d.stride, d.pad_t, d.pad_l, d.upsample = stride, pt, pl, int(upsample)
    if gn_ab is not None:
        d.gn_ab = _req(gn_ab, torch.float32, "conv.gn_ab").data_ptr()
        d.gn_images_per_sample, d.gn_silu = gn_images_per_sample, int(gn_silu)
    ws = _workspace(x.device)
    d.workspace, d.workspace_bytes, d.split_k = ws.data_ptr(), ws.numel() * 4, split_k
    with _timed("gemm_kernel", 2.0 * M * N * 9 * cin, ("conv", M, N, 9 * cin, stride, int(upsample), residual is not None)):
        check(lib.insv2v_gemm(_byref(d), _stream()), "insv2v_gemm(conv3x3)")
    return out, (NB, OH, OW)


def _gn_chunks(nsamples, rows_per_sample):
    return max(1, min(rows_per_sample // 32, max(1, 1024 // nsamples), 128))


_WINO_G = torch.tensor([[1.0, 0.0, 0.0], [0.5, 0.5, 0.5], [0.5, -0.5, 0.5], [0.0, 0.0, 1.0]])


def winograd_weights(w, device, upsample=False):
    u = torch.einsum("ai,ocij,bj->aboc", _WINO_G, w.float(), _WINO_G)
    if upsample:
        u = u[[0, 1, 3]][:, [0, 1, 3]]
    return u.reshape(-1, w.shape[0], w.shape[1]).to(device=device, dtype=torch.float16).contiguous()


def winograd_ok(geom, cin, c1=0, upsample=False, out_size=None):
    _, H, W = geom
    if upsample and out_size is not None and tuple(out_size) != (2 * H, 2 * W):
        return False
    return W <= 128 and cin % 64 == 0 and c1 % 64 == 0


def winograd_conv3x3(x, geom, U, bias=None, *, x2=None, gn_ab=None, gn_images_per_sample=0, gn_silu=False, row_bias=None, rows_per_group=0,
                     residual=None, out=None, tile=0, upsample=False):
    lib = _lib.load()
    _req(x, torch.float16, "winograd.x"), _req(U, torch.float16, "winograd.U")
    NB, H, W = geom
    C1 = x.shape[1]
    C = C1 + (x2.shape[1] if x2 is not None else 0)
    Cout = U.shape[1]
    ng = 9 if upsample else 16
    OH, OW = (2 * H, 2 * W) if upsample else (H, W)
    assert U.shape[0] == ng and U.shape[2] == C and x.shape[0] == NB * H * W
    tiles = NB * H * W if upsample else NB * ((H + 1) // 2) * ((W + 1) // 2)
    grows = -(-tiles // 256) * 256
    v = torch.empty((ng * grows, C), device=x.device, dtype=torch.float16)
    di = WinogradInDesc()
    di.x, di.v, di.ldx, di.v_group_rows = x.data_ptr(), v.data_ptr(), x.stride(0), grows
    if x2 is not None:
        di.x2, di.ldx2, di.C1 = _req(x2, torch.float16, "winograd.x2").data_ptr(), x2.stride(0), C1
    di.NB, di.H, di.W, di.C, di.upsample = NB, H, W, C, int(upsample)
    if gn_ab is not None:
        di.gn_ab, di.gn_images_per_sample, di.gn_silu = _req(gn_ab, torch.float32, "winograd.gn_ab").data_ptr(), gn_images_per_sample, int(gn_silu)
    with _timed("groupnorm", 0.0, ("wino_in", NB * H * W, C)):
        check(lib.insv2v_winograd_input(_byref(di), _stream()), "insv2v_winograd_input")
    m = torch.empty((ng * grows, Cout), device=x.device, dtype=torch.float16)
    d = GemmDesc()
    d.a, d.w, d.c = v.data_ptr(), U.data_ptr(), m.data_ptr()
    d.lda, d.ldw, d.ldc = C, C, Cout
    d.M, d.N, d.K, d.batch, d.alpha, d.tile = ng * grows, Cout, C, 1, 1.0, tile
    d.w_group_rows, d.w_group_stride = grows, Cout * C
    with _timed("gemm_kernel", 2.0 * NB * OH * OW * Cout * 9 * C, ("wino_gemm", ng * grows, Cout, C)):
        check(lib.insv2v_gemm(_byref(d), _stream()), "insv2v_gemm (grouped)")
    del v
    if out is None:
        out = torch.empty((NB * OH * OW, Cout), device=x.device, dtype=torch.float16)
    do = WinogradOutDesc()
    do.m, do.y, do.m_group_rows, do.ldy = m.data_ptr(), out.data_ptr(), grows, out.stride(0)
    if bias is not None:
        do.bias = _req(bias, torch.float32, "winograd.bias").data_ptr()
    if row_bias is not None:
        do.row_bias, do.ld_rb, do.rows_per_group = _req(row_bias, torch.float32, "winograd.row_bias").data_ptr(), row_bias.stride(0), rows_per_group
    if residual is not None:
        do.residual, do.ldr = _req(residual, torch.float16, "winograd.residual").data_ptr(), residual.stride(0)
    do.NB, do.H, do.W, do.Cout, do.upsample = NB, H, W, Cout, int(upsample)
    with _timed("groupnorm", 0.0, ("wino_out", NB * OH * OW, Cout)):
        check(lib.insv2v_winograd_output(_byref(do), _stream()), "insv2v_winograd_output")
    return out


def groupnorm(x, nsamples, rows_per_sample, gamma, beta, groups, eps, silu=False, x2=None):
    lib = _lib.load()
    _req(x, torch.float16, "groupnorm.x")
    C1 = x.shape[1]
    Ct = C1 + (x2.shape[1] if x2 is not None else 0)
    assert nsamples * rows_per_sample == x.shape[0]
    y = torch.empty((x.shape[0], Ct), device=x.device, dtype=torch.float16)
    nchunks = _gn_chunks(nsamples, rows_per_sample)
    scratch = torch.empty(nsamples * groups * (2 + 3 * nchunks), device=x.device, dtype=torch.float32)
    d = GroupNormDesc()
    d.x, d.y, d.gamma, d.beta, d.partials = x.data_ptr(), y.data_ptr(), gamma.data_ptr(), beta.data_ptr(), scratch.data_ptr()
    d.ldx, d.ldy = x.stride(0), y.stride(0)
    if x2 is not None:
        d.x2, d.ldx2, d.C1 = _req(x2, torch.float16, "groupnorm.x2").data_ptr(), x2.stride(0), C1
    d.nsamples, d.rows_per_sample, d.C, d.G, d.nchunks, d.silu, d.eps = nsamples, rows_per_sample, Ct, groups, nchunks, int(silu), eps
    with _timed("groupnorm", 0.0, ("gn", nsamples, rows_per_sample, Ct)):
        check(lib.insv2v_groupnorm(_byref(d), _stream()), "insv2v_groupnorm")
    return y


def groupnorm_stats(x, nsamples, rows_per_sample, gamma, beta, groups, eps, x2=None):
    lib = _lib.load()
    _req(x, torch.float16, "groupnorm.x")
    C1 = x.shape[1]
    Ct = C1 + (x2.shape[1] if x2 is not None else 0)
    assert nsamples * rows_per_sample == x.shape[0]
    nchunks = _gn_chunks(nsamples, rows_per_sample)
    scratch = torch.empty(nsamples * groups * (2 + 3 * nchunks), device=x.device, dtype=torch.float32)
    ab = torch.empty((nsamples, Ct, 2), device=x.device, dtype=torch.float32)
    d = GroupNormDesc()
    d.x, d.gamma, d.beta, d.partials, d.ab = x.data_ptr(), gamma.data_ptr(), beta.data_ptr(), scratch.data_ptr(), ab.data_ptr()
    d.ldx, d.stats_only = x.stride(0), 1
    if x2 is not None:
        d.x2, d.ldx2, d.C1 = _req(x2, torch.float16, "groupnorm.x2").data_ptr(), x2.stride(0), C1
    d.nsamples, d.rows_per_sample, d.C, d.G, d.nchunks, d.eps = nsamples, rows_per_sample, Ct, groups, nchunks, eps
    with _timed("groupnorm", 0.0, ("gnstats", nsamples, rows_per_sample, Ct)):
        check(lib.insv2v_groupnorm(_byref(d), _stream()), "insv2v_groupnorm(stats_only)")
    return ab


def layernorm(x, gamma, beta, eps=1e-5, pe=None, rows_per_frame=0, frames=0, pe_start=0):
    lib = _lib.load()
    _req(x, torch.float16, "layernorm.x")
    y = torch.empty_like(x)
    d = LayerNormDesc()
    d.x, d.y, d.gamma, d.beta = x.data_ptr(), y.data_ptr(), gamma.data_ptr(), beta.data_ptr()
    d.ldx, d.ldy, d.rows, d.C, d.eps = x.stride(0), y.stride(0), x.shape[0], x.shape[1], eps
    if pe is not None:
        d.pe, d.rows_per_frame, d.frames, d.pe_start = _req(pe, torch.float32, "layernorm.pe").data_ptr(), rows_per_frame, frames, pe_start
    with _timed("layernorm", 0.0, ("ln", x.shape[0], x.shape[1])):
        check(lib.insv2v_layernorm(_byref(d), _stream()), "insv2v_layernorm")
    return y


def layernorm_stats(x, eps=1e-5):
    lib = _lib.load()
    _req(x, torch.float16, "layernorm_stats.x")
    stats = torch.empty((x.shape[0], 2), device=x.device, dtype=torch.float32)
    with _timed("layernorm", 0.0, ("lnstats", x.shape[0], x.shape[1])):
        check(lib.insv2v_layernorm_stats(x.data_ptr(), stats.data_ptr(), x.stride(0), x.shape[0], x.shape[1], eps, _stream()),
              "insv2v_layernorm_stats")
    return stats


def attention(q_ptr, k_ptr, v_ptr, out, *, batch, heads, head_dim, seq_q, seq_k, scale,
              q_rs, k_rs, v_rs, o_rs, q_addr, kv_addr, o_addr, causal=False, qkv_bias=None):
    lib = _lib.load()
    d = AttentionDesc()
    if qkv_bias is not None:
        _req(qkv_bias, torch.float16, "attention.qkv_bias")
        cq = heads * head_dim
        if qkv_bias.shape[0] < max(seq_q, seq_k) or qkv_bias.shape[1] != 3 * cq:
            raise _lib.HipKernelError(f"attention: bias table {tuple(qkv_bias.shape)} for {max(seq_q, seq_k)} rows x 3 x {cq} columns")
        bp = qkv_bias.data_ptr()
        d.q_bias, d.k_bias, d.v_bias, d.bias_rs = bp, bp + 2 * cq, bp + 4 * cq, qkv_bias.stride(0)
    d.q, d.k, d.v, d.o = q_ptr, k_ptr, v_ptr, out.data_ptr()
    d.q_rs, d.k_rs, d.v_rs, d.o_rs = q_rs, k_rs, v_rs, o_rs
    d.q_inner, d.q_outer, d.q_step = q_addr
    d.kv_inner, d.kv_outer, d.kv_step = kv_addr
    d.o_inner, d.o_outer, d.o_step = o_addr
    d.batch, d.heads, d.head_dim, d.seq_q, d.seq_k, d.scale, d.causal = batch, heads, head_dim, seq_q, seq_k, scale, int(causal)
    with _timed("attn_kernel", 4.0 * batch * heads * seq_q * seq_k * head_dim, ("attn", batch, heads, head_dim, seq_q, seq_k)):
        check(lib.insv2v_attention(_byref(d), _stream()), "insv2v_attention")
    return out


def attention_short_supported(heads, head_dim, seq):
    return seq <= 16 and heads <= 16 and head_dim in (16, 32, 40, 64, 80, 128, 160) and heads * ((head_dim + 15) // 16) * 16 * 20 * 2 <= 64 * 1024


def embed_tokens(ids, tok, pos):
    lib = _lib.load()
    _req(tok, torch.float16, "embed.tok")
    _req(pos, torch.float16, "embed.pos")
    if ids.dtype != torch.int64 or not ids.is_cuda or not ids.is_contiguous():
        raise _lib.HipKernelError("embed.ids must be a contiguous int64 device tensor")
    n, L = ids.shape
    if L > pos.shape[0]:
        raise ValueError(f"Sequence length must be less than max_position_embeddings (got {L} > {pos.shape[0]})")
    out = torch.empty((n * L, tok.shape[1]), device=tok.device, dtype=torch.float16)
    check(lib.insv2v_embed_tokens(ids.data_ptr(), tok.data_ptr(), pos.data_ptr(), out.data_ptr(), n * L, L, tok.shape[1],
                                  tok.shape[0], _stream()), "insv2v_embed_tokens")
    return out


def softmax_rows(x, scale=1.0, valid=None):
    lib = _lib.load()
    _req(x, torch.float16, "softmax.x")
    x2 = x.reshape(-1, x.shape[-1])
    if valid is not None and valid != x2.shape[1]:
        check(lib.insv2v_softmax_rows_padded(x2.data_ptr(), x2.data_ptr(), x2.stride(0), x2.stride(0), x2.shape[0], x2.shape[1], valid,
                                             scale, _stream()), "insv2v_softmax_rows_padded")
        return x
    check(lib.insv2v_softmax_rows(x2.data_ptr(), x2.data_ptr(), x2.stride(0), x2.stride(0), x2.shape[0], x2.shape[1],
                                  scale, _stream()), "insv2v_softmax_rows")
    return x


def timestep_embedding(t_dev, dim, shift=0.0):
    lib = _lib.load()
    _req(t_dev, torch.float32, "timestep")
    out = torch.empty((t_dev.shape[0], dim), device=t_dev.device, dtype=torch.float16)
    check(lib.insv2v_timestep_embedding(t_dev.data_ptr(), out.data_ptr(), t_dev.shape[0], dim, shift, _stream()),
          "insv2v_timestep_embedding")
    return out


def build_unet_input(latent, img_cond, out, t_out, timestep, nbranch, branch_rows=0, t_stride=0):
    lib = _lib.load()
    F, _, h, w = latent.shape[-4:]
    check(lib.insv2v_build_unet_input(_req(latent, torch.float32, "latent").data_ptr(),
                                      _req(img_cond, torch.float32, "img_cond").data_ptr(), out.data_ptr(),
                                      _ptr(t_out), float(timestep), nbranch, F, h, w, out.shape[-1], branch_rows, t_stride, _stream()),
          "insv2v_build_unet_input")
    return out


def cfg_step(eps_in, latent, *, nbranch, text_cfg=1.0, img_cfg=1.0, sqrt_a=1.0, sqrt_1ma=0.0, coef=(0, 0, 0, 0),
             latent_out=None, pred_x0=None, eps_out=None, latent_ref=None, correct=0, delta_q=None, noise=None,
             rescale_stats=None, guidance_rescale=0.0, branch_stride=0, noise_seed=None, noise_stream=0, x0_hist=None, c_hist=0.0):
    kw = dict(nbranch=nbranch, text_cfg=text_cfg, img_cfg=img_cfg, sqrt_a=sqrt_a, sqrt_1ma=sqrt_1ma, coef=coef, latent_out=latent_out,
              pred_x0=pred_x0, eps_out=eps_out, latent_ref=latent_ref, correct=correct, delta_q=delta_q, noise=noise,
              rescale_stats=rescale_stats, guidance_rescale=guidance_rescale, branch_stride=branch_stride, noise_seed=noise_seed,
              noise_stream=noise_stream)
    if x0_hist is not None:
        return cfg_step_ms(eps_in, latent, x0_hist=x0_hist, c_hist=c_hist, **kw)
    if c_hist != 0.0:
        raise _lib.HipKernelError("cfg_step: c_hist != 0 needs x0_hist")
    lib = _lib.load()
    d = _fill_step_desc(StepDesc(), eps_in, latent, **kw)
    check(lib.insv2v_cfg_step(_byref(d), _stream()), "insv2v_cfg_step")


def cfg_step_ms(eps_in, latent, *, x0_hist=None, c_hist=0.0, **kw):
    lib = _lib.load()
    d = _fill_step_desc(MStepDesc(), eps_in, latent, **kw)
    if x0_hist is not None and (tuple(x0_hist.shape[-4:]) != tuple(latent.shape[-4:]) or not x0_hist.is_contiguous()):
        raise _lib.HipKernelError(f"cfg_step_ms: x0_hist {tuple(x0_hist.shape)} must be contiguous and shaped like the latent {tuple(latent.shape)}")
    d.x0_hist = _req(x0_hist, torch.float32, "x0_hist").data_ptr() if x0_hist is not None else None
    d.c_hist = c_hist
    check(lib.insv2v_cfg_step_ms(_byref(d), _stream()), "insv2v_cfg_step_ms")


def _fill_step_desc(d, eps_in, latent, *, nbranch, text_cfg=1.0, img_cfg=1.0, sqrt_a=1.0, sqrt_1ma=0.0, coef=(0, 0, 0, 0),
                    latent_out=None, pred_x0=None, eps_out=None, latent_ref=None, correct=0, delta_q=None, noise=None,
                    rescale_stats=None, guidance_rescale=0.0, branch_stride=0, noise_seed=None, noise_stream=0):
    F, _, h, w = latent.shape[-4:]
    d.eps_in, d.latent = _req(eps_in, torch.float32, "eps_in").data_ptr(), _req(latent, torch.float32, "latent").data_ptr()
    d.latent_ref, d.delta_q, d.noise, d.rescale_stats = _ptr(latent_ref), _ptr(delta_q), _ptr(noise), _ptr(rescale_stats)
    d.latent_out, d.pred_x0, d.eps_out = _ptr(latent_out), _ptr(pred_x0), _ptr(eps_out)
    d.nbranch, d.F, d.h, d.w, d.correct = nbranch, F, h, w, correct
    d.R = latent_ref.shape[-4] if latent_ref is not None else 0
    d.text_cfg, d.img_cfg, d.sqrt_a, d.sqrt_1ma = text_cfg, img_cfg, sqrt_a, sqrt_1ma
    d.c_x0, d.c_eps, d.c_xt, d.c_noise = coef
    d.guidance_rescale, d.branch_stride = guidance_rescale, branch_stride
    if noise_seed is not None:
        d.noise_seed, d.noise_stream, d.noise_on = as_int64(noise_seed), as_int64(noise_stream, "stream"), 1
    return d


def cfg_stats(eps_in, stats, F, h, w, text_cfg, img_cfg, branch_stride=0):
    lib = _lib.load()
    check(lib.insv2v_cfg_stats(eps_in.data_ptr(), stats.data_ptr(), F, h, w, text_cfg, img_cfg, branch_stride, _stream()), "insv2v_cfg_stats")


def warp_image(image, flow):
    lib = _lib.load()
    _req(image, torch.float32, "warp.image"), _req(flow, torch.float32, "warp.flow")
    image, flow = image.contiguous(), flow.contiguous()
    N, Cc, H, W = image.shape
    out = torch.empty_like(image)
    check(lib.insv2v_warp_image(image.data_ptr(), flow.data_ptr(), out.data_ptr(), N, Cc, H, W, _stream()), "insv2v_warp_image")
    return out


def resize_flow(flow, size):
    lib = _lib.load()
    _req(flow, torch.float32, "resize_flow.flow")
    flow = flow.contiguous()
    N, _, h, w = flow.shape
    H, W = size
    out = torch.empty((N, 2, H, W), device=flow.device, dtype=torch.float32)
    check(lib.insv2v_resize_flow(flow.data_ptr(), out.data_ptr(), N, h, w, H, W, _stream()), "insv2v_resize_flow")
    return out


def flow_correction(eps_cfg, latent, latent_ref, flows, sqrt_a, sqrt_1ma):
    lib = _lib.load()
    F, _, h, w = latent.shape[-4:]
    R = latent_ref.shape[-4]
    out = torch.empty((F - R, 4, h, w), device=latent.device, dtype=torch.float32)
    check(lib.insv2v_flow_correction(eps_cfg.data_ptr(), latent.data_ptr(), latent_ref.data_ptr(), flows.data_ptr(),
                                     out.data_ptr(), F, R, h, w, sqrt_a, sqrt_1ma, _stream()), "insv2v_flow_correction")
    return out


def nchw_to_nhwc_f16(x, ldo, scale=1.0):
    lib = _lib.load()
    _req(x, torch.float32, "nchw_to_nhwc.x")
    x = x.contiguous()
    N, Cc, H, W = x.shape
    out = torch.empty((N * H * W, ldo), device=x.device, dtype=torch.float16)
    check(lib.insv2v_nchw_to_nhwc_f16(x.data_ptr(), out.data_ptr(), N, Cc, H, W, ldo, scale, _stream()), "insv2v_nchw_to_nhwc_f16")
    return out


def nhwc_to_nchw_f32(x, N, Cc, H, W, scale=1.0):
    lib = _lib.load()
    out = torch.empty((N, Cc, H, W), device=x.device, dtype=torch.float32)
    check(lib.insv2v_nhwc_to_nchw_f32(x.data_ptr(), int(x.dtype == torch.float32), out.data_ptr(), N, Cc, H, W,
                                      x.stride(0), scale, _stream()), "insv2v_nhwc_to_nchw_f32")
    return out


def posterior_sample(moments, noise, N, H, W, scale, seed=None, stream=0, offset=0):
    lib = _lib.load()
    _req(moments, torch.float32, "posterior.moments")
    z = torch.empty((N, 4, H, W), device=moments.device, dtype=torch.float32)
    if seed is not None:
        if noise is not None:
            raise _lib.HipKernelError("posterior_sample: pass noise or seed, not both")
        check(lib.insv2v_posterior_sample_seeded(moments.data_ptr(), z.data_ptr(), N, H, W, moments.stride(0), scale,
                                                 as_int64(seed), as_int64(stream, "stream"), int(offset), _stream()), "insv2v_posterior_sample_seeded")
        return z
    _req(noise, torch.float32, "posterior.noise")
    check(lib.insv2v_posterior_sample(moments.data_ptr(), noise.contiguous().data_ptr(), z.data_ptr(), N, H, W,
                                      moments.stride(0), scale, _stream()), "insv2v_posterior_sample")
    return z


def randn(shape_or_out, seed, stream, offset=0, raw=False, device=None):
    lib = _lib.load()
    if torch.is_tensor(shape_or_out):
        out = shape_or_out
        if not (out.is_cuda and out.is_contiguous() and (out.dtype == torch.float32 or (raw and out.dtype == torch.int32))):
            raise _lib.HipKernelError(f"randn: expected a contiguous CUDA float32 tensor, got {out.device} {out.dtype}")
    else:
        shape = (shape_or_out,) if isinstance(shape_or_out, int) else tuple(shape_or_out)
        out = torch.empty(shape, device=device if device is not None else torch.device("cuda", torch.cuda.current_device()),
                          dtype=torch.int32 if raw else torch.float32)
    check(lib.insv2v_randn(out.data_ptr(), out.numel(), as_int64(seed), as_int64(stream, "stream"), int(offset), int(bool(raw)), _stream()),
          "insv2v_randn")
    return out


def im2col(x, geom, C, kh, kw, stride=1, pad=(0, 0), x2=None):
    lib = _lib.load()
    _req(x, torch.float16, "im2col.x")
    N, IH, IW = geom
    OH, OW = (IH + 2 * pad[0] - kh) // stride + 1, (IW + 2 * pad[1] - kw) // stride + 1
    out = torch.empty((N * OH * OW, kh * kw * C), device=x.device, dtype=torch.float16)
    d = _lib.Im2colDesc()
    d.x, d.out, d.ldx, d.ldo = x.data_ptr(), out.data_ptr(), x.stride(0), out.stride(0)
    if x2 is not None:
        _req(x2, torch.float16, "im2col.x2")
        d.x2, d.ldx2, d.C1 = x2.data_ptr(), x2.stride(0), C - x2.shape[1]
    else:
        d.C1 = C
    d.N, d.IH, d.IW, d.C, d.KH, d.KW = N, IH, IW, C, kh, kw
    d.stride_h = d.stride_w = stride
    d.pad_h, d.pad_w, d.OH, d.OW = pad[0], pad[1], OH, OW
    with _timed("im2col", 0.0, ("im2col", N * OH * OW, kh * kw * C)):
        check(lib.insv2v_im2col(_byref(d), _stream()), "insv2v_im2col")
    return out, (N, OH, OW)


def instance_norm(x, N, HW, relu=False, eps=1e-5):
    lib = _lib.load()
    _req(x, torch.float16, "instance_norm.x")
    Cc = x.shape[1]
    nchunks = max(1, min(64, HW // 64))
    part = torch.empty((N * nchunks * Cc * 2,), device=x.device, dtype=torch.float32)
    y = torch.empty((x.shape[0], Cc), device=x.device, dtype=torch.float16)
    with _timed("instnorm", 0.0, ("instnorm", N, HW, Cc)):
        check(lib.insv2v_instance_norm(x.data_ptr(), y.data_ptr(), part.data_ptr(), N, HW, Cc, x.stride(0), y.stride(0), nchunks, eps,
                                       int(relu), _stream()), "insv2v_instance_norm")
    return y


def ew(op, a, b=None, c=None, out=None):
    lib = _lib.load()
# ... 45 lines not shown
```

### instruct-video-to-video_amd/insv2v/unet.py

```python
import math
import os

import torch

from . import ops
from . import fused
from .fused import check_operand_windows, pack_ffn_stream, pack_linear_stream, pack_tattn_stream, pack_tattn_qkv_stream

CPAD = 64
FUSE_GN = os.environ.get("INSV2V_FUSE_GN", "0") != "0"
FUSE_FFN = os.environ.get("INSV2V_FUSE_FFN", "1") != "0"
FUSE_FFN_POST = os.environ.get("INSV2V_FUSE_FFN_POST", "1") != "0"
DEDUP_CFG = os.environ.get("INSV2V_DEDUP_CFG", "1") != "0"
WINOGRAD = os.environ.get("INSV2V_WINOGRAD", "1") != "0"
WINOGRAD_MIN_CIN = int(os.environ.get("INSV2V_WINOGRAD_MIN_CIN", "1280"))
WINOGRAD_MIN_ROWS = int(os.environ.get("INSV2V_WINOGRAD_MIN_ROWS", "4608"))
WINOGRAD_UP_MIN_CIN = int(os.environ.get("INSV2V_WINOGRAD_UP_MIN_CIN", "640"))
MERGE_FF2_POST = os.environ.get("INSV2V_MERGE_FF2_POST", "1") != "0"
NARROW_CONV_OUT = os.environ.get("INSV2V_NARROW_CONV_OUT", "1") != "0"
NARROW_CONV_MIN_ROWS = int(os.environ.get("INSV2V_NARROW_CONV_MIN_ROWS", "16384"))
ROWLIN = os.environ.get("INSV2V_ROWLIN", "1") != "0"
ROWLIN_640 = os.environ.get("INSV2V_ROWLIN_640", "1") != "0"
ROWLIN_640_MIN_ROWS = int(os.environ.get("INSV2V_ROWLIN_640_MIN_ROWS", "55296"))


def _rowlin_640_pays(rows):
    return rows >= ROWLIN_640_MIN_ROWS or rows < 12288
FUSE_TATTN = os.environ.get("INSV2V_FUSE_TATTN", "1") != "0"
FUSE_TATTN_640 = os.environ.get("INSV2V_FUSE_TATTN_640", "1") != "0"
TATTN_MIN_FRAMES = int(os.environ.get("INSV2V_TATTN_MIN_FRAMES", "16"))
ROWLIN_GN = os.environ.get("INSV2V_ROWLIN_GN", "1") != "0"
FUSE_XATTN = os.environ.get("INSV2V_FUSE_XATTN", "1") != "0"
FUSE_XATTN_640 = os.environ.get("INSV2V_FUSE_XATTN_640", "1") != "0"
FUSE_XATTN_PRE = os.environ.get("INSV2V_FUSE_XATTN_PRE", "1") != "0"
ATTN_PE_BIAS = os.environ.get("INSV2V_ATTN_PE_BIAS", "1") != "0"


def rowlin_stream(w, bias, device, table=None):
    w = w.reshape(w.shape[0], -1)
    if not (ROWLIN and ops.rowlin_supported(w.shape[0], w.shape[1])) or (w.shape[1] == 640 and not ROWLIN_640):
        return None
    return _dev(pack_linear_stream(w.detach().half().float(), bias, table), torch.float16, device)


class Act:
    __slots__ = ("t", "B", "F", "H", "W")

    def __init__(self, t, B, F, H, W):
        self.t, self.B, self.F, self.H, self.W = t, B, F, H, W

    @property
    def hw(self):
        return self.H * self.W

    def like(self, t, H=None, W=None):
        return Act(t, self.B, self.F, self.H if H is None else H, self.W if W is None else W)


def _dev(t, dtype, device):
    return t.detach().to(device=device, dtype=dtype).contiguous()


def prep_linear(sd, key, device, bias=True):
    w = _dev(sd[key + ".weight"].reshape(sd[key + ".weight"].shape[0], -1), torch.float16, device)
    b = _dev(sd[key + ".bias"], torch.float32, device) if bias and (key + ".bias") in sd else None
    return w, b


def prep_conv3x3(sd, key, device, cin_pad=None):
    w = sd[key + ".weight"].detach().float()
    cout, cin = w.shape[:2]
    cp = cin_pad or ((cin + CPAD - 1) // CPAD * CPAD)
    wk = torch.zeros(cout, 3, 3, cp)
    wk[..., :cin] = w.permute(0, 2, 3, 1)
    return _dev(wk.reshape(cout, 9 * cp), torch.float16, device), _dev(sd[key + ".bias"], torch.float32, device)


def prep_norm(sd, key, device):
    return _dev(sd[key + ".weight"], torch.float32, device), _dev(sd[key + ".bias"], torch.float32, device)


def interleave32(t):
    n = t.shape[0] // 2
    h, g = t[:n], t[n:]
    rest = t.shape[1:]
    return torch.stack([h.reshape(n // 32, 32, *rest), g.reshape(n // 32, 32, *rest)], dim=1).reshape(2 * n, *rest)


def fold_layernorm(w, gamma, beta, bias=None):
    w = w.detach().float()
    wf = (w * gamma.detach().float()[None, :]).half()
    col = wf.float().sum(1)
    b = w @ beta.detach().float()
    if bias is not None:
        b = b + bias.detach().float()
    return wf, col, b


class FeedForwardW:

    def __init__(self, sd, key, device, norm_key, post_key=None):
        wf, col, b = fold_layernorm(sd[key + ".net.0.proj.weight"], sd[norm_key + ".weight"], sd[norm_key + ".bias"],
                                    sd[key + ".net.0.proj.bias"])
        self.w1 = _dev(interleave32(wf), torch.float16, device)
        self.cs1 = _dev(interleave32(col), torch.float32, device)
        self.b1 = _dev(interleave32(b), torch.float32, device)
        self.w2, self.b2 = prep_linear(sd, key + ".net.2", device)
        self.hidden, self.stream, self.stream_post = self.w2.shape[1], None, None
        self.w2p = self.b2p = None
        if FUSE_FFN and ops.ffn_fused_supported(self.w2.shape[0], self.hidden):
            w2f, b2f = sd[key + ".net.2.weight"].half().float(), sd[key + ".net.2.bias"]
            self.stream = _dev(pack_ffn_stream(wf.float(), b, w2f, b2f), torch.float16, device)
            if post_key is not None and FUSE_FFN_POST:
                self.stream_post = _dev(pack_ffn_stream(wf.float(), b, w2f, b2f, post=(sd[post_key + ".weight"].half().float(), sd[post_key + ".bias"])),
                                        torch.float16, device)

        if self.stream is None and post_key is not None and MERGE_FF2_POST and self.hidden % 64 == 0:
            wp = sd[post_key + ".weight"].detach().float().reshape(sd[post_key + ".weight"].shape[0], -1)
            w2f, b2f = sd[key + ".net.2.weight"].detach().float(), sd[key + ".net.2.bias"].detach().float()
            self.w2p = _dev(torch.cat([wp @ w2f, wp], 1), torch.float16, device)
            self.b2p = _dev(wp @ b2f + sd[post_key + ".bias"].detach().float(), torch.float32, device)

    def with_proj_out_gemm(self, x, stats, module_input):
        g = ops.gemm(x, self.w1, self.b1, act=ops.ACT_GEGLU, row_stats=stats if stats is not None else ops.layernorm_stats(x), col_sum=self.cs1)
        return ops.gemm(g, self.w2p, self.b2p, a2=x, residual=module_input)

    def with_proj_out(self, x, module_input):
        return ops.ffn_fused(x, self.stream_post, self.hidden, post_residual=module_input)

    def __call__(self, x, residual, stats=None):
        if self.stream is not None and (residual is x or residual is None) and x.is_contiguous():
            return ops.ffn_fused(x, self.stream, self.hidden)
        if residual is None:
            residual = x
        g = ops.gemm(x, self.w1, self.b1, act=ops.ACT_GEGLU, row_stats=stats if stats is not None else ops.layernorm_stats(x), col_sum=self.cs1)
        return ops.gemm(g, self.w2, self.b2, residual=residual)


class ResBlock:

    def __init__(self, sd, key, cin, cout, groups, eps, device, temb_slice):
        self.cin, self.cout, self.groups, self.eps = cin, cout, groups, eps
        self.n1 = prep_norm(sd, key + ".norm1", device)
        self.n2 = prep_norm(sd, key + ".norm2", device)
        self.w1, self.b1 = prep_conv3x3(sd, key + ".conv1", device)
        self.w2, self.b2 = prep_conv3x3(sd, key + ".conv2", device)
        self.u1 = ops.winograd_weights(sd[key + ".conv1.weight"].detach(), device) if (WINOGRAD and cin >= WINOGRAD_MIN_CIN and cin % 64 == 0) else None
        self.u2 = ops.winograd_weights(sd[key + ".conv2.weight"].detach(), device) if (WINOGRAD and cout >= WINOGRAD_MIN_CIN and cout % 64 == 0) else None
        self.sc = prep_linear(sd, key + ".conv_shortcut", device) if (key + ".conv_shortcut.weight") in sd else None
        self.temb_slice = temb_slice

    def __call__(self, x, temb_all, skip=None, out=None):
        rows = x.F * x.hw
        geom = (x.B * x.F, x.H, x.W)
        x2 = skip.t if skip is not None else None
        c1 = x.t.shape[1]
        tb = temb_all[:, self.temb_slice[0]:self.temb_slice[1]]
        wino = x.t.shape[0] >= WINOGRAD_MIN_ROWS
        if self.u1 is not None and wino and ops.winograd_ok(geom, self.cin, c1 if x2 is not None else 0):
            ab = ops.groupnorm_stats(x.t, x.B, rows, *self.n1, self.groups, self.eps, x2=x2)
            h = ops.winograd_conv3x3(x.t, geom, self.u1, self.b1, x2=x2, gn_ab=ab, gn_images_per_sample=x.F, gn_silu=True, row_bias=tb, rows_per_group=rows)
        elif FUSE_GN and ops.conv3x3_fuses_groupnorm(geom, self.cin, self.cout, c1 if x2 is not None else 0):
            ab = ops.groupnorm_stats(x.t, x.B, rows, *self.n1, self.groups, self.eps, x2=x2)
            h, _ = ops.conv3x3(x.t, geom, self.w1, self.b1, x2=x2, row_bias=tb, rows_per_group=rows,
                               gn_ab=ab, gn_images_per_sample=x.F, gn_silu=True)
        else:
            n = ops.groupnorm(x.t, x.B, rows, *self.n1, self.groups, self.eps, silu=True, x2=x2)
            h, _ = ops.conv3x3(n, geom, self.w1, self.b1, row_bias=tb, rows_per_group=rows)
        if self.sc is not None:
            res = ops.gemm(x.t, self.sc[0], self.sc[1], a2=x2)
        else:
            res = x.t
        if self.u2 is not None and wino and ops.winograd_ok(geom, self.cout):
            ab = ops.groupnorm_stats(h, x.B, rows, *self.n2, self.groups, self.eps)
            out = ops.winograd_conv3x3(h, geom, self.u2, self.b2, gn_ab=ab, gn_images_per_sample=x.F, gn_silu=True, residual=res, out=out)
        elif FUSE_GN and ops.conv3x3_fuses_groupnorm(geom, self.cout, self.cout):
            ab = ops.groupnorm_stats(h, x.B, rows, *self.n2, self.groups, self.eps)
            out, _ = ops.conv3x3(h, geom, self.w2, self.b2, residual=res, gn_ab=ab, gn_images_per_sample=x.F, gn_silu=True, out=out)
        else:
            n = ops.groupnorm(h, x.B, rows, *self.n2, self.groups, self.eps, silu=True)
            out, _ = ops.conv3x3(n, geom, self.w2, self.b2, residual=res, out=out)
        return x.like(out)


class SpatialTransformer:

    def __init__(self, sd, key, ch, heads, groups, device):
        self.ch, self.heads, self.groups = ch, heads, groups
        self.norm = prep_norm(sd, key + ".norm", device)
        self.proj_in = prep_linear(sd, key + ".proj_in", device)
        self.proj_out = prep_linear(sd, key + ".proj_out", device)
        b = key + ".transformer_blocks.0"
        wf, col, bb = fold_layernorm(torch.cat([sd[f"{b}.attn1.to_{n}.weight"].float() for n in "qkv"], 0),
                                     sd[f"{b}.norm1.weight"], sd[f"{b}.norm1.bias"])
        self.wqkv, self.qkv_cs, self.qkv_b = _dev(wf, torch.float16, device), _dev(col, torch.float32, device), _dev(bb, torch.float32, device)
        self.wo1 = prep_linear(sd, f"{b}.attn1.to_out.0", device)
        wf, col, bb = fold_layernorm(sd[f"{b}.attn2.to_q.weight"], sd[f"{b}.norm2.weight"], sd[f"{b}.norm2.bias"])
        self.wq2, self.q2_cs, self.q2_b = _dev(wf, torch.float16, device), _dev(col, torch.float32, device), _dev(bb, torch.float32, device)
        self.wkv2 = _dev(torch.cat([sd[f"{b}.attn2.to_{n}.weight"].float() for n in "kv"], 0), torch.float16, device)
        self.wo2 = prep_linear(sd, f"{b}.attn2.to_out.0", device)
        self.ff = FeedForwardW(sd, b + ".ff", device, b + ".norm3", post_key=key + ".proj_out")
        self.rl = None
        if ROWLIN and ops.rowlin_supported(ch, ch) and (ch != 640 or ROWLIN_640):
            lin = lambda k: (sd[k + ".weight"], sd[k + ".bias"])
            self.rl = dict(proj_in=rowlin_stream(*lin(key + ".proj_in"), device), proj_out=rowlin_stream(*lin(key + ".proj_out"), device),
                           qkv=rowlin_stream(self.wqkv.float(), self.qkv_b, device), wo1=rowlin_stream(*lin(f"{b}.attn1.to_out.0"), device),
                           q2=rowlin_stream(self.wq2.float(), self.q2_b, device), wo2=rowlin_stream(*lin(f"{b}.attn2.to_out.0"), device))
        self.xa_stream, self.xa640_stream, self.xa_pre_stream = None, None, None
        if self.rl is not None and FUSE_XATTN and ops.xattn_fused_supported(ch, heads, 77, 128):
            self.xa_stream = fused.pack_xattn_stream(self.wq2.float(), self.q2_b, *lin(f"{b}.attn2.to_out.0")).to(device)
            if FUSE_XATTN_PRE:
                self.xa_pre_stream = fused.pack_xattn_stream(self.wq2.float(), self.q2_b, *lin(f"{b}.attn2.to_out.0"),
                                                             pre=lin(f"{b}.attn1.to_out.0")).to(device)
        elif self.rl is not None and FUSE_XATTN_640 and ops.xattn_attn_supported(ch, heads, 77, 128):
            self.xa640_stream = fused.pack_xattn_q_stream(self.wq2.float(), self.q2_b).to(device)

    def project_context(self, ctx2d, ctx_len=0):
        kv = ops.gemm(ctx2d, self.wkv2)
        if self.xa_stream is not None and ctx_len and 64 < ctx_len <= 96:
            return kv, fused.pack_xattn_kv(kv, kv.shape[0] // ctx_len, ctx_len, self.ch, self.heads)
        if self.xa640_stream is not None and ctx_len and 64 < ctx_len <= 96:
            return kv, fused.pack_xattn640_kv(kv, kv.shape[0] // ctx_len, ctx_len, self.ch, self.heads)
        return kv

    def __call__(self, x, kv, ctx_len, shared=0):
        C, hd, BF, HW = self.ch, self.ch // self.heads, x.B * x.F, x.hw
        scale = hd ** -0.5
        rl = self.rl if (C != 640 or _rowlin_640_pays(x.t.shape[0])) else None
        a = None
        if rl is not None and ROWLIN_GN and shared > 0 and x.B == 3 * shared:
            r1, r2 = shared * x.F * HW, 2 * shared * x.F * HW
            ab = ops.groupnorm_stats(x.t[:r2], 2 * shared * x.F, HW, *self.norm, self.groups, 1e-6)
            h, st = torch.empty((x.t.shape[0], C), device=x.t.device, dtype=torch.float16), None
            ops.rowlin(x.t[:r2], rl["proj_in"], C, gn_ab=ab, gn_rows=HW, out=h[:r2])
            qkv = ops.rowlin(h[:r2], rl["qkv"], 3 * C, layernorm=True)
            a = torch.empty((x.t.shape[0], C), device=h.device, dtype=torch.float16)
            p = qkv.data_ptr()
            ops.attention(p, p + 2 * C, p + 4 * C, a[:r2], batch=2 * shared * x.F, heads=self.heads, head_dim=hd, seq_q=HW, seq_k=HW,
                          scale=scale, q_rs=3 * C, k_rs=3 * C, v_rs=3 * C, o_rs=C,
                          q_addr=(1, HW * 3 * C, 0), kv_addr=(1, HW * 3 * C, 0), o_addr=(1, HW * C, 0))
            ops.copy_rows(h[r2:], h[r1:r2])
            ops.copy_rows(a[r2:], a[r1:r2])
        elif rl is not None and ROWLIN_GN:
            ab = ops.groupnorm_stats(x.t, BF, HW, *self.norm, self.groups, 1e-6)
            h, st = ops.rowlin(x.t, rl["proj_in"], C, gn_ab=ab, gn_rows=HW), None
            qkv = ops.rowlin(h, rl["qkv"], 3 * C, layernorm=True)
        elif rl is not None:
            n = ops.groupnorm(x.t, BF, HW, *self.norm, self.groups, 1e-6)
            h, st = ops.rowlin(n, rl["proj_in"], C), None
            qkv = ops.rowlin(h, rl["qkv"], 3 * C, layernorm=True)
        else:
            n = ops.groupnorm(x.t, BF, HW, *self.norm, self.groups, 1e-6)
            h, st = ops.gemm(n, *self.proj_in, emit_stats=True)
            qkv = ops.gemm(h, self.wqkv, self.qkv_b, row_stats=st, col_sum=self.qkv_cs)
        if a is None:
            a = torch.empty((x.t.shape[0], C), device=h.device, dtype=torch.float16)
            p = qkv.data_ptr()
            ops.attention(p, p + 2 * C, p + 4 * C, a, batch=BF, heads=self.heads, head_dim=hd, seq_q=HW, seq_k=HW,
                          scale=scale, q_rs=3 * C, k_rs=3 * C, v_rs=3 * C, o_rs=C,
                          q_addr=(1, HW * 3 * C, 0), kv_addr=(1, HW * 3 * C, 0), o_addr=(1, HW * C, 0))
        kv, kv_frag = kv if isinstance(kv, tuple) else (kv, None)
        if rl is None:
            kv_frag = None
        xa = kv_frag is not None and ops.xattn_fused_supported(C, self.heads, ctx_len, x.F * HW)
        if xa:
            if self.xa_pre_stream is not None and h.is_contiguous():
                h2 = ops.xattn_fused(a, self.xa_pre_stream, kv_frag, x.F * HW, self.heads, ctx_len, pre_residual=h)
            else:
                h = ops.rowlin(a, rl["wo1"], C, residual=h)
                h2 = ops.xattn_fused(h, self.xa_stream, kv_frag, x.F * HW, self.heads, ctx_len)
            if self.ff.stream_post is not None:
                return x.like(self.ff.with_proj_out(h2, x.t))
            h = self.ff(h2, None) if self.ff.stream is not None else self.ff(h2, h2, ops.layernorm_stats(h2))
            return x.like(ops.rowlin(h, rl["proj_out"], C, residual=x.t))
        if kv_frag is not None and self.xa640_stream is not None and ops.xattn_attn_supported(C, self.heads, ctx_len, x.F * HW):
            h = ops.rowlin(a, rl["wo1"], C, residual=h)
            a = ops.xattn_attn(h, self.xa640_stream, kv_frag, x.F * HW, self.heads, ctx_len)
            if self.ff.stream is not None:
                h = self.ff(ops.rowlin(a, rl["wo2"], C, residual=h), None)
            else:
                h, st = ops.rowlin(a, rl["wo2"], C, residual=h, emit_stats=True)
                if self.ff.w2p is not None:
                    return x.like(self.ff.with_proj_out_gemm(h, st, x.t))
                h = self.ff(h, h, st)
            return x.like(ops.rowlin(h, rl["proj_out"], C, residual=x.t))
        if rl is not None:
            h = ops.rowlin(a, rl["wo1"], C, residual=h)
            q = ops.rowlin(h, rl["q2"], C, layernorm=True)
        else:
            h, st = ops.gemm(a, *self.wo1, residual=h, emit_stats=True)
            q = ops.gemm(h, self.wq2, self.q2_b, row_stats=st, col_sum=self.q2_cs)
        a = torch.empty_like(a)
        kp = kv.data_ptr()
        ops.attention(q.data_ptr(), kp, kp + 2 * C, a, batch=BF, heads=self.heads, head_dim=hd, seq_q=HW, seq_k=ctx_len,
                      scale=scale, q_rs=C, k_rs=2 * C, v_rs=2 * C, o_rs=C,
                      q_addr=(1, HW * C, 0), kv_addr=(x.F, ctx_len * 2 * C, 0), o_addr=(1, HW * C, 0))
        if rl is not None:
            if self.ff.stream_post is not None:
                return x.like(self.ff.with_proj_out(ops.rowlin(a, rl["wo2"], C, residual=h), x.t))
            if self.ff.stream is not None:
                h = self.ff(ops.rowlin(a, rl["wo2"], C, residual=h), None)
            else:
                h, st = ops.rowlin(a, rl["wo2"], C, residual=h, emit_stats=True)
                if self.ff.w2p is not None:
                    return x.like(self.ff.with_proj_out_gemm(h, st, x.t))
                h = self.ff(h, h, st)
            return x.like(ops.rowlin(h, rl["proj_out"], C, residual=x.t))
        h, st = ops.gemm(a, *self.wo2, residual=h, emit_stats=True)
        if self.ff.w2p is not None:
            return x.like(self.ff.with_proj_out_gemm(h, st, x.t))
        h = self.ff(h, h, st)
        return x.like(ops.gemm(h, *self.proj_out, residual=x.t))


def sinusoid_table(d_model, max_len):
    pos = torch.arange(max_len).unsqueeze(1)
    div = torch.exp(torch.arange(0, d_model, 2) * (-math.log(10000.0) / d_model))
    pe = torch.zeros(max_len, d_model)
    pe[:, 0::2] = torch.sin(pos * div)
    pe[:, 1::2] = torch.cos(pos * div)
    return pe


class MotionModule:

    def __init__(self, sd, key, ch, groups, device, num_attention_heads=8, num_transformer_block=2,
                 attention_block_types=("Temporal_Self", "Temporal_Self"), temporal_position_encoding=True,
                 temporal_position_encoding_max_len=24, temporal_attention_dim_div=1, **unused):
        if not temporal_position_encoding or any(t != "Temporal_Self" for t in attention_block_types):
            raise NotImplementedError("only Temporal_Self attention with positional encoding is used by InsV2V")
        k = key + ".temporal_transformer"
        self.ch, self.heads, self.groups = ch, num_attention_heads, groups
        self.max_len = temporal_position_encoding_max_len
        self.norm = prep_norm(sd, k + ".norm", device)
        self.proj_in = prep_linear(sd, k + ".proj_in", device)
        self.proj_out = prep_linear(sd, k + ".proj_out", device)
        self.blocks = []
        for bi in range(num_transformer_block):
            b = f"{k}.transformer_blocks.{bi}"
            attns = []
            for ai in range(len(attention_block_types)):
                ab = f"{b}.attention_blocks.{ai}"
                wraw = torch.cat([sd[f"{ab}.to_{n}.weight"].float() for n in "qkv"], 0)
                pe_key = f"{ab}.pos_encoder.pe"
                pe = sd[pe_key].reshape(-1, ch).float() if pe_key in sd else sinusoid_table(ch, self.max_len)
                wf, col, bb = fold_layernorm(wraw, sd[f"{b}.norms.{ai}.weight"], sd[f"{b}.norms.{ai}.bias"])
                attns.append(dict(wqkv=_dev(wf, torch.float16, device), cs=_dev(col, torch.float32, device),
                                  b=_dev(bb, torch.float32, device), wo=prep_linear(sd, f"{ab}.to_out.0", device),
                                  pe_bias=_dev(pe @ wraw.t(), torch.float32, device),
                                  rl_wo=rowlin_stream(sd[f"{ab}.to_out.0.weight"], sd[f"{ab}.to_out.0.bias"], device),
                                  host=(wf.float(), bb.float(), (pe @ wraw.t()).float()), rl_qkv={}, rl_tattn={}, pe_half={},
                                  host_o=(sd[f"{ab}.to_out.0.weight"].detach().half().float(), sd[f"{ab}.to_out.0.bias"].detach().float())))
            last = bi == num_transformer_block - 1
            self.blocks.append(dict(attns=attns, ff=FeedForwardW(sd, b + ".ff", device, b + ".ff_norm", post_key=(k + ".proj_out") if last else None)))
        self.device = device
        self.rl = None
        if ROWLIN and ops.rowlin_supported(ch, ch) and (ch != 640 or ROWLIN_640):
            self.rl = dict(proj_in=rowlin_stream(sd[k + ".proj_in.weight"], sd[k + ".proj_in.bias"], device),
                           proj_out=rowlin_stream(sd[k + ".proj_out.weight"], sd[k + ".proj_out.bias"], device))

    def _tattn_stream(self, at, start, F):
        st = at["rl_tattn"].get((start, F))
        if st is None:
            wf, bb, pe_bias = at["host"]
            wo, bo = at["host_o"]
            st = at["rl_tattn"][(start, F)] = _dev(pack_tattn_stream(wf, pe_bias[start:start + F] + bb[None, :], wo, bo), torch.float16, self.device)
        return st

    def _tattn_qkv_stream(self, at, start, F):
        st = at["rl_tattn"].get((start, F, "qkv"))
        if st is None:
            wf, bb, pe_bias = at["host"]
            st = at["rl_tattn"][(start, F, "qkv")] = _dev(pack_tattn_qkv_stream(wf, pe_bias[start:start + F] + bb[None, :]), torch.float16, self.device)
        return st

    def _qkv_stream(self, at, start, F):
        st = at["rl_qkv"].get((start, F))
        if st is None:
            wf, bb, pe_bias = at["host"]
            st = at["rl_qkv"][(start, F)] = rowlin_stream(wf, None, self.device, table=pe_bias[start:start + F] + bb[None, :])
        return st

    def __call__(self, x, start=0):
        C, hd, HW, F = self.ch, self.ch // self.heads, x.hw, x.F
        if start + F > self.max_len:
            start -= self.max_len
        if start < 0:
            raise ValueError(f"start_index must be non-negative, but got {start}")
        rl = self.rl if (C != 640 or _rowlin_640_pays(x.t.shape[0])) else None
        rl_frames = rl is not None and F <= 16
        win = rl is not None and F >= TATTN_MIN_FRAMES
        fused_attn = win and FUSE_TATTN and ops.tattn_fused_supported(C, self.heads, F)
        fused_640 = win and FUSE_TATTN_640 and ops.tattn_attn_supported(C, self.heads, F)
        row_flow = rl_frames or fused_attn or fused_640
        if rl is not None and ROWLIN_GN:
            ab = ops.groupnorm_stats(x.t, x.B * F, HW, *self.norm, self.groups, 1e-6)
            h, st = ops.rowlin(x.t, rl["proj_in"], C, gn_ab=ab, gn_rows=HW), None
        elif rl is not None:
            h, st = ops.rowlin(ops.groupnorm(x.t, x.B * F, HW, *self.norm, self.groups, 1e-6), rl["proj_in"], C), None
        else:
            h, st = ops.gemm(ops.groupnorm(x.t, x.B * F, HW, *self.norm, self.groups, 1e-6), *self.proj_in, emit_stats=True)
        if rl is not None and not row_flow:
            st = ops.layernorm_stats(h)
        for bi, blk in enumerate(self.blocks):
            for at in blk["attns"]:
                if fused_attn:
                    h = ops.tattn_fused(h, self._tattn_stream(at, start, F), x.B, HW, self.heads, F)
                    continue
                pe_half = None
                if fused_640 and h.is_contiguous():
                    a = ops.tattn_attn(h, self._tattn_qkv_stream(at, start, F), x.B, HW, self.heads, F)
                    if blk["ff"].stream is None and at is blk["attns"][-1]:
                        h, st = ops.rowlin(a, at["rl_wo"], C, residual=h, emit_stats=True)
                    else:
                        h = ops.rowlin(a, at["rl_wo"], C, residual=h)
                    continue
                if not rl_frames and rl is not None and st is None:
                    st = ops.layernorm_stats(h)
                if rl_frames:
                    qkv = ops.rowlin(h, self._qkv_stream(at, start, F), 3 * C, layernorm=True, frames=F, rows_per_frame=HW)
                elif ATTN_PE_BIAS and ops.attention_short_supported(self.heads, hd, F):
                    pe_half = at["pe_half"].get((start, F))
                    if pe_half is None:
                        pe_half = at["pe_half"][(start, F)] = at["pe_bias"][start:start + F].half().contiguous()
                    qkv = ops.gemm(h, at["wqkv"], at["b"], row_stats=st, col_sum=at["cs"])
                else:
                    qkv = ops.gemm(h, at["wqkv"], at["b"], row_stats=st, col_sum=at["cs"],
                                   row_bias=at["pe_bias"][start:start + F], rows_per_group=HW, rb_mod=F)
                a = torch.empty((x.t.shape[0], C), device=h.device, dtype=torch.float16)
                p = qkv.data_ptr()
                addr = (HW, F * HW * 3 * C, 3 * C)
                ops.attention(p, p + 2 * C, p + 4 * C, a, batch=x.B * HW, heads=self.heads, head_dim=hd, seq_q=F, seq_k=F,
                              scale=hd ** -0.5, q_rs=HW * 3 * C, k_rs=HW * 3 * C, v_rs=HW * 3 * C, o_rs=HW * C,
                              q_addr=addr, kv_addr=addr, o_addr=(HW, F * HW * C, C), qkv_bias=pe_half)
                if rl is not None:
                    if (blk["ff"].stream is None and at is blk["attns"][-1]) or (not rl_frames and at is not blk["attns"][-1]):
                        h, st = ops.rowlin(a, at["rl_wo"], C, residual=h, emit_stats=True)
                    else:
                        h, st = ops.rowlin(a, at["rl_wo"], C, residual=h), None
                else:
                    h, st = ops.gemm(a, *at["wo"], residual=h, emit_stats=True)
            if rl is not None and bi + 1 == len(self.blocks) and blk["ff"].stream_post is not None and h.is_contiguous():
                return x.like(blk["ff"].with_proj_out(h, x.t))
            if bi + 1 == len(self.blocks) and blk["ff"].w2p is not None:
                return x.like(blk["ff"].with_proj_out_gemm(h, st, x.t))
            h = blk["ff"](h, h, st)
            if bi + 1 < len(self.blocks) and not row_flow:
                st = ops.layernorm_stats(h)
        if rl is not None:
            return x.like(ops.rowlin(h, rl["proj_out"], C, residual=x.t))
        return x.like(ops.gemm(h, *self.proj_out, residual=x.t))


def plan_sizes(H, W, levels=4):
    if H < 1 or W < 1 or levels < 1:
        raise ValueError(f"UNet3DConditionModel: a latent of {H}x{W} pixels has a side that reaches 0")
    down = [(int(H), int(W))]
    for _ in range(levels - 1):
        h, w = down[-1]
        down.append(((h - 1) // 2 + 1, (w - 1) // 2 + 1))
    return dict(down=down, up=down[-2::-1])


class UNetOutput:
    def __init__(self, sample):
        self.sample = sample


class UNet3DConditionModel:

    def __init__(self, in_channels=4, out_channels=4, block_out_channels=(320, 640, 1280, 1280),
                 down_block_types=("CrossAttnDownBlock3D",) * 3 + ("DownBlock3D",),
                 up_block_types=("UpBlock3D",) + ("CrossAttnUpBlock3D",) * 3,
                 layers_per_block=2, norm_num_groups=32, norm_eps=1e-5, cross_attention_dim=1280,
                 attention_head_dim=8, flip_sin_to_cos=True, freq_shift=0, use_motion_module=True,
                 motion_module_resolutions=(1, 2, 4, 8), motion_module_mid_block=True,
                 motion_module_decoder_only=False, motion_module_type="Vanilla", motion_module_kwargs=None,
                 device="cuda", **unused):
        if not flip_sin_to_cos:
            raise NotImplementedError("flip_sin_to_cos=False")
        if motion_module_type != "Vanilla":
            raise ValueError
        self.cfg = dict(in_channels=in_channels, out_channels=out_channels, ch=list(block_out_channels),
# ... 176 lines not shown
```

Before: 16.28 frames/s.

## Emit GroupNorm partial stats from Winograd output and pipeline input staging

The Winograd output kernel can now accumulate per-group GroupNorm partial moments while writing the conv1 result. A small finalize kernel turns those into scale/shift pairs, so the ResBlock's second GroupNorm no longer needs a separate statistics pass that re-reads h. The Winograd input kernel is also rewritten as a persistent loop over work items that prefetches the next item's first loads while transforming the current one, with an occupancy hint in launch bounds. This adds scratch buffers, an extra finalize launch and more register pressure in the output and input kernels.

```diff
diff --git a/include/insv2v_hip.h b/include/insv2v_hip.h
--- a/include/insv2v_hip.h
+++ b/include/insv2v_hip.h
@@ -95,8 +95,11 @@
     int32_t NB, H, W, Cout;
     int32_t rows_per_group;
     int32_t upsample;
+    float* gn_partials;
+    int32_t gn_G, gn_rows_per_sample, gn_nchunks;
 } insv2v_winograd_out_desc;
 int insv2v_winograd_output(const insv2v_winograd_out_desc* d, insv2v_stream_t stream);
+int insv2v_winograd_out_gn_chunks(const insv2v_winograd_out_desc* d);
 
 typedef struct insv2v_ffn_desc {
     const void* x;
@@ -174,8 +177,10 @@
     float eps;
     float* ab;
     int32_t stats_only;
+    int32_t apply_only;
 } insv2v_groupnorm_desc;
 int insv2v_groupnorm(const insv2v_groupnorm_desc* d, insv2v_stream_t stream);
+int insv2v_groupnorm_finalize(const insv2v_groupnorm_desc* d, insv2v_stream_t stream);
 
 typedef struct insv2v_layernorm_desc {
     const void* x;
diff --git a/instruct-video-to-video_amd/build.py b/instruct-video-to-video_amd/build.py
--- a/instruct-video-to-video_amd/build.py
+++ b/instruct-video-to-video_amd/build.py
@@ -20,7 +20,7 @@
     hipcc = os.environ.get("HIPCC", "/opt/rocm/bin/hipcc")
     objdir = os.path.join(HERE, "build")
     os.makedirs(objdir, exist_ok=True)
-    deps = [os.path.join(CSRC, "common.h"), os.path.join(CSRC, "gemm_dma.h"), os.path.join(CSRC, "rows_common.h"), os.path.join(CSRC, "rng.h"), os.path.join(HERE, "..", "include", "insv2v_hip.h")]
+    deps = [os.path.join(CSRC, "common.h"), os.path.join(CSRC, "gemm_dma.h"), os.path.join(CSRC, "rows_common.h"), os.path.join(CSRC, "rng.h"), os.path.join(CSRC, "winograd_plan.h"), os.path.join(HERE, "..", "include", "insv2v_hip.h")]
     jobs = []
     for src in SOURCES:
         s, o = os.path.join(CSRC, src), os.path.join(objdir, src + ".o")
diff --git a/instruct-video-to-video_amd/csrc/norm.hip b/instruct-video-to-video_amd/csrc/norm.hip
--- a/instruct-video-to-video_amd/csrc/norm.hip
+++ b/instruct-video-to-video_amd/csrc/norm.hip
@@ -138,6 +138,11 @@
 #pragma unroll
     for (int e = 0; e < 8; ++e) {
         int c = c0 + e, g = c / cpg;
+        if (p.apply_only) {
+            a[e] = p.ab[((int64_t)sample * p.C + c) * 2 + 0];
+            b[e] = p.ab[((int64_t)sample * p.C + c) * 2 + 1];
+            continue;
+        }
         float mean = p.partials[((int64_t)sample * p.G + g) * 2 + 0];
         float rstd = p.partials[((int64_t)sample * p.G + g) * 2 + 1];
         a[e] = rstd * p.gamma[c];
@@ -363,13 +368,16 @@
     if (!one_device()) return INSV2V_EINVAL;
     if (!dp) return INSV2V_EINVAL;
     insv2v_groupnorm_desc d = *dp;
-    if (!d.x || !d.gamma || !d.beta || !d.partials) return INSV2V_EINVAL;
+    if (d.apply_only) {
+        if (!d.x || !d.y || !d.ab || d.stats_only) return INSV2V_EINVAL;
+    } else if (!d.x || !d.gamma || !d.beta || !d.partials) return INSV2V_EINVAL;
     if (d.stats_only ? !d.ab : !d.y) return INSV2V_EINVAL;
     if (d.C <= 0 || d.G <= 0 || (d.C % d.G) || (d.C & 7) || d.C > 8192) return INSV2V_EINVAL;
     if ((d.ldx & 7) || (d.ldy & 7) || d.nsamples <= 0 || d.rows_per_sample <= 0) return INSV2V_EINVAL;
     if (d.x2 && ((d.C1 & 7) || d.C1 <= 0 || d.C1 >= d.C || (d.ldx2 & 7))) return INSV2V_EINVAL;
-    if (d.nchunks <= 0) return INSV2V_EINVAL;
+    if (d.nchunks <= 0 && !d.apply_only) return INSV2V_EINVAL;
     hipStream_t s = as_stream(stream);
+    if (!d.apply_only)
     {
         static const int frame_on = getenv("INSV2V_GN_FRAME") ? atoi(getenv("INSV2V_GN_FRAME")) : 1;
         const int cpg = d.C / d.G;
@@ -384,6 +392,7 @@
             if (rc != INSV2V_EUNSUPPORTED) return rc;
         }
     }
+    if (!d.apply_only)
     {
         const int cpg = d.C / d.G;
         const int vw = (cpg % 8 == 0) ? 8 : ((cpg % 4 == 0) ? 4 : 0);
@@ -400,6 +409,13 @@
     if (P < 1) P = 1;
     if (P > 16) P = 16;
     const int threads = CC * P;
+    if (d.apply_only) {
+        long want = ((long)d.rows_per_sample + P * 4 - 1) / (P * 4);
+        long cap = 4096 / d.nsamples;
+        if (cap < 1) cap = 1;
+        hipLaunchKernelGGL(gn_apply_kernel, dim3((int)(want < cap ? want : cap), d.nsamples), dim3(threads), 0, s, d, CC, P);
+        return launch_status();
+    }
     int nchunks = d.nchunks;
     if (nchunks > d.rows_per_sample) nchunks = d.rows_per_sample;
     d.nchunks = nchunks;
@@ -417,6 +433,16 @@
     return launch_status();
 }
 
+extern "C" int insv2v_groupnorm_finalize(const insv2v_groupnorm_desc* dp, insv2v_stream_t stream) {
+    if (!one_device()) return INSV2V_EINVAL;
+    if (!dp) return INSV2V_EINVAL;
+    const insv2v_groupnorm_desc& d = *dp;
+    if (!d.partials || d.nsamples <= 0 || d.nchunks <= 0 || d.C <= 0 || d.G <= 0 || (d.C % d.G)) return INSV2V_EINVAL;
+    if (d.ab && (!d.gamma || !d.beta)) return INSV2V_EINVAL;
+    hipLaunchKernelGGL(gn_finalize_kernel, dim3((d.G + 3) / 4, d.nsamples), dim3(256), 0, as_stream(stream), d);
+    return launch_status();
+}
+
 #define LN_MAXCH 4
 #define LN_ROWS 4
 template <int NCH>
diff --git a/instruct-video-to-video_amd/csrc/winograd.hip b/instruct-video-to-video_amd/csrc/winograd.hip
--- a/instruct-video-to-video_amd/csrc/winograd.hip
+++ b/instruct-video-to-video_amd/csrc/winograd.hip
@@ -1,137 +1,265 @@
 #include "common.h"
+#include "winograd_plan.h"
 
 namespace {
 
 template <bool UP> __device__ __forceinline__ int lds_px(int sp) { return UP ? sp : sp ^ ((sp >> 1) & 1); }
 
+#define WINO_PF 4
+struct wino_item {
+    int nb0, c0, tr0, tr1, row0, nrows, nimg;
+};
+
 template <bool NORM, bool UP>
-__global__ __launch_bounds__(256) void wino_input_kernel(const half_t* __restrict__ x, const half_t* __restrict__ x2, const float* __restrict__ ab,
+__global__ __launch_bounds__(256, WINO_IN_WGS_PER_CU) void wino_input_kernel(const half_t* __restrict__ x, const half_t* __restrict__ x2, const float* __restrict__ ab,
                                                          half_t* __restrict__ V, int64_t ldx, int64_t ldx2, int C1, int C, int NB, int H, int W,
-                                                         int ipb, int images_per_sample, int silu, int64_t group_rows, int band_tr) {
+                                                         int ipb, int images_per_sample, int silu, int64_t group_rows, int band_tr, int nslices,
+                                                         int nbands, int nitems) {
     extern __shared__ __attribute__((aligned(16))) char smem[];
     const int tid = threadIdx.x, chunk = tid & 7, item0 = tid >> 3;
-    const int nb0 = (int)blockIdx.x * ipb, c0 = (int)blockIdx.y * 64;
     const int trows = UP ? H : (H + 1) >> 1;
-    const int tr0 = (int)blockIdx.z * band_tr, tr1 = min(tr0 + band_tr, trows);
     const bool whole = band_tr >= trows;
-    const int row0 = whole ? 0 : (UP ? tr0 - 1 : 2 * tr0 - 1);
-    const int nrows = whole ? H : (UP ? (tr1 - tr0) + 2 : 2 * (tr1 - tr0) + 2);
-    const int HW = H * W, SW = nrows * W;
-    const int SWs = UP ? SW : (SW + 1) & ~1;
-    const bool second = x2 != nullptr && c0 >= C1;
-    const half_t* src = second ? x2 + (c0 - C1) + chunk * 8 : x + c0 + chunk * 8;
-    const int64_t ld = second ? ldx2 : ldx;
-    const int nimg = min(ipb, NB - nb0);
-    for (int it = item0; it < nimg * SW; it += 32) {
-        const int img = it / SW, sp = it - img * SW;
-        const int iy = row0 + sp / W;
-        if ((unsigned)iy >= (unsigned)H) continue;
-        half8 v = *(const half8*)(src + ((int64_t)(nb0 + img) * HW + sp + row0 * W) * ld);
-        if (NORM) {
-            const float* p = ab + ((int64_t)((nb0 + img) / images_per_sample) * C + c0 + chunk * 8) * 2;
-            const float4 p0 = *(const float4*)p, p1 = *(const float4*)(p + 4), p2 = *(const float4*)(p + 8), p3 = *(const float4*)(p + 12);
-            const float sc[8] = {p0.x, p0.z, p1.x, p1.z, p2.x, p2.z, p3.x, p3.z}, sh[8] = {p0.y, p0.w, p1.y, p1.w, p2.y, p2.w, p3.y, p3.w};
+    const int HW = H * W;
+    auto decode = [&](int w) {
+        wino_item it;
+        const int q = w / nslices, band = q % nbands;
+        it.c0 = (w - q * nslices) * 64;
+        it.nb0 = (q / nbands) * ipb;
+        it.tr0 = band * band_tr;
+        it.tr1 = min(it.tr0 + band_tr, trows);
+        it.row0 = whole ? 0 : (UP ? it.tr0 - 1 : 2 * it.tr0 - 1);
+        it.nrows = whole ? H : (UP ? (it.tr1 - it.tr0) + 2 : 2 * (it.tr1 - it.tr0) + 2);
+        it.nimg = min(ipb, NB - it.nb0);
+        return it;
+    };
+    auto src_of = [&](const wino_item& it, int s, int& slot) -> const half_t* {
+        const int SW = it.nrows * W, SWs = UP ? SW : (SW + 1) & ~1;
+        const int img = s / SW, sp = s - img * SW;
+        const int iy = it.row0 + sp / W;
+        const bool second = x2 != nullptr && it.c0 >= C1;
+        const half_t* src = second ? x2 + (it.c0 - C1) + chunk * 8 : x + it.c0 + chunk * 8;
+        const int64_t ld = second ? ldx2 : ldx;
+        const bool ok = s < it.nimg * SW && (unsigned)iy < (unsigned)H;
+        slot = ok ? img * SWs + lds_px<UP>(sp) : -1;
+        return src + (ok ? (int64_t)(it.nb0 + img) * HW + sp + it.row0 * W : (int64_t)it.nb0 * HW + max(it.row0, 0) * W) * ld;
+    };
+    auto put = [&](int slot, half8 v) {
+        if (slot >= 0) *(half8*)(smem + (int64_t)slot * 128 + chunk * 16) = v;
+    };
+    auto norm_pass = [&](const wino_item& it) {
+        const int SW = it.nrows * W, n = it.nimg * SW;
+        float sc[8], sh[8];
+        int tab_sample = -1;
+#pragma unroll 1
+        for (int s = item0; s < n; s += 32) {
+            int slot;
+            src_of(it, s, slot);
+            if (slot < 0) continue;
+            const int sample = (it.nb0 + s / SW) / images_per_sample;
+            if (sample != tab_sample) {
+                const float* p = ab + ((int64_t)sample * C + it.c0 + chunk * 8) * 2;
+                const float4 p0 = *(const float4*)p, p1 = *(const float4*)(p + 4), p2 = *(const float4*)(p + 8), p3 = *(const float4*)(p + 12);
+                sc[0] = p0.x; sc[1] = p0.z; sc[2] = p1.x; sc[3] = p1.z; sc[4] = p2.x; sc[5] = p2.z; sc[6] = p3.x; sc[7] = p3.z;
+                sh[0] = p0.y; sh[1] = p0.w; sh[2] = p1.y; sh[3] = p1.w; sh[4] = p2.y; sh[5] = p2.w; sh[6] = p3.y; sh[7] = p3.w;
+                tab_sample = sample;
+            }
+            half8* q = (half8*)(smem + (int64_t)slot * 128 + chunk * 16);
+            half8 v = *q;
 #pragma unroll
             for (int e = 0; e < 8; ++e) {
                 float f = fmaf((float)v[e], sc[e], sh[e]);
                 if (silu) f = silu_f(f);
                 v[e] = (half_t)f;
             }
-        }
-        *(half8*)(smem + ((int64_t)img * SWs + lds_px<UP>(sp)) * 128 + chunk * 16) = v;
-    }
+            *q = v;
+        }
+    };
+    auto stage_rest = [&](const wino_item& it, int k0) {
+        const int n = it.nimg * it.nrows * W;
+        for (int s = item0 + 32 * k0; s < n; s += 32) {
+            int slot;
+            const half_t* src = src_of(it, s, slot);
+            put(slot, *(const half8*)src);
+        }
+    };
+    auto transform = [&](const wino_item& it) {
+        const int SW = it.nrows * W, SWs = UP ? SW : (SW + 1) & ~1;
+        const int row0 = it.row0, tr0 = it.tr0, nb0 = it.nb0, c0 = it.c0;
+        if constexpr (UP) {
+            const int bt = (it.tr1 - tr0) * W;
+            for (int s = item0; s < it.nimg * bt; s += 32) {
+                const int img = s / bt, tb_ = s - img * bt;
+                const int y = tr0 + tb_ / W, xx = tb_ - (tb_ / W) * W;
+                const int t = y * W + xx;
+                const char* base = smem + (int64_t)img * SWs * 128 + chunk * 16;
+                auto px = [&](int r, int cc) {
+                    const int iy = y - 1 + r, ix = xx - 1 + cc;
+                    half8 v = {0, 0, 0, 0, 0, 0, 0, 0};
+                    if ((unsigned)iy < (unsigned)H && (unsigned)ix < (unsigned)W) v = *(const half8*)(base + lds_px<UP>((iy - row0) * W + ix) * 128);
+                    return v;
+                };
+                const int64_t trow = (int64_t)(nb0 + img) * HW + t;
+                half_t* dst = V + trow * C + c0 + chunk * 8;
+#pragma unroll
+                for (int j = 0; j < 3; ++j) {
+                    float hz[3][8];
+#pragma unroll
+                    for (int r = 0; r < 3; ++r) {
+                        const half8 a = px(r, j == 0 ? 0 : 1), b = px(r, j == 2 ? 2 : 1);
+#pragma unroll
+                        for (int e = 0; e < 8; ++e) hz[r][e] = j == 1 ? 2.f * (float)a[e] : (float)a[e] - (float)b[e];
+                    }
+                    half8 o[3];
+#pragma unroll
+                    for (int e = 0; e < 8; ++e) {
+                        o[0][e] = (half_t)(hz[0][e] - hz[1][e]);
+                        o[1][e] = (half_t)(2.f * hz[1][e]);
+                        o[2][e] = (half_t)(hz[1][e] - hz[2][e]);
+                    }
+#pragma unroll
+                    for (int i = 0; i < 3; ++i) *(half8*)(dst + (int64_t)(i * 3 + j) * group_rows * C) = o[i];
+                }
+            }
+        } else {
+            const int th = (H + 1) >> 1, tw = (W + 1) >> 1, ntile = th * tw;
+            const int bt = (it.tr1 - tr0) * tw;
+            for (int s = item0; s < it.nimg * bt; s += 32) {
+                const int img = s / bt, tb_ = s - img * bt;
+                const int ty = tr0 + tb_ / tw, tx = tb_ - (tb_ / tw) * tw;
+                const int t = ty * tw + tx;
+                const char* base = smem + (int64_t)img * SWs * 128 + chunk * 16;
+                auto px = [&](int r, int cc) {
+                    const int iy = 2 * ty - 1 + r, ix = 2 * tx - 1 + cc;
+                    half8 v = {0, 0, 0, 0, 0, 0, 0, 0};
+                    if ((unsigned)iy < (unsigned)H && (unsigned)ix < (unsigned)W) v = *(const half8*)(base + lds_px<UP>((iy - row0) * W + ix) * 128);
+                    return v;
+                };
+                const int64_t trow = (int64_t)(nb0 + img) * ntile + t;
+                half_t* dst = V + trow * C + c0 + chunk * 8;
+#pragma unroll
+                for (int j = 0; j < 4; ++j) {
+                    float hz[4][8];
+#pragma unroll
+                    for (int r = 0; r < 4; ++r) {
+                        const half8 a = px(r, j == 0 ? 0 : j == 2 ? 2 : 1), b = px(r, j == 2 ? 1 : j == 3 ? 3 : 2);
+#pragma unroll
+                        for (int e = 0; e < 8; ++e) hz[r][e] = j == 1 ? (float)a[e] + (float)b[e] : (float)a[e] - (float)b[e];
+                    }
+                    half8 o[4];
+#pragma unroll
+                    for (int e = 0; e < 8; ++e) {
+                        o[0][e] = (half_t)(hz[0][e] - hz[2][e]);
+                        o[1][e] = (half_t)(hz[1][e] + hz[2][e]);
+                        o[2][e] = (half_t)(hz[2][e] - hz[1][e]);
+                        o[3][e] = (half_t)(hz[1][e] - hz[3][e]);
+                    }
+#pragma unroll
+                    for (int i = 0; i < 4; ++i) *(half8*)(dst + (int64_t)(i * 4 + j) * group_rows * C) = o[i];
+                }
+            }
+        }
+    };
+
+    int w = (int)blockIdx.x;
+    if (w >= nitems) return;
+    wino_item cur = decode(w);
+    stage_rest(cur, 0);
+    if (NORM) norm_pass(cur);
     __syncthreads();
+    for (;;) {
+        const int wn = w + (int)gridDim.x;
+        const bool more = wn < nitems;
+        wino_item nxt = cur;
+        half8 pf[WINO_PF];
+        int pslot[WINO_PF];
+        if (more) {
+            nxt = decode(wn);
+#pragma unroll
+            for (int k = 0; k < WINO_PF; ++k) pf[k] = *(const half8*)src_of(nxt, item0 + 32 * k, pslot[k]);
+        }
+        transform(cur);
+        if (!more) break;
+        __syncthreads();
+#pragma unroll
+        for (int k = 0; k < WINO_PF; ++k) put(pslot[k], pf[k]);
+        stage_rest(nxt, WINO_PF);
+        if (NORM) norm_pass(nxt);
+        __syncthreads();
+        cur = nxt;
+        w = wn;
+    }
+}
+
+template <bool RES, bool RB, bool UP>
+__device__ __forceinline__ void wino_out_tile(const half_t* __restrict__ Mo, const float* __restrict__ bias, const float* __restrict__ row_bias,
+                                              const half_t* __restrict__ res, half_t* __restrict__ y, int64_t group_rows, int64_t tile, int ch,
+                                              int Cout, int H, int W, int64_t ld_rb, int rows_per_group, int64_t ldr, int64_t ldy, half8 (&o)[2][2]) {
+    const int th = UP ? H : (H + 1) >> 1, tw = UP ? W : (W + 1) >> 1, ntile = th * tw;
+    const int OW = UP ? 2 * W : W, OH = UP ? 2 * H : H;
+    const int nb = (int)(tile / ntile), t = (int)(tile - (int64_t)nb * ntile);
+    const int ty = t / tw, tx = t - ty * tw;
+    const half_t* src = Mo + tile * Cout + ch;
+    float s[2][4][8];
     if constexpr (UP) {
-        const int bt = (tr1 - tr0) * W;
-        for (int it = item0; it < nimg * bt; it += 32) {
-            const int img = it / bt, tb_ = it - img * bt;
-            const int y = tr0 + tb_ / W, xx = tb_ - (tb_ / W) * W;
-            const int t = y * W + xx;
-            const char* base = smem + (int64_t)img * SWs * 128 + chunk * 16;
-            float hz[3][3][8];
-#pragma unroll
-            for (int r = 0; r < 3; ++r) {
-                const int iy = y - 1 + r;
-                float d[3][8];
-#pragma unroll
-                for (int c = 0; c < 3; ++c) {
-                    const int ix = xx - 1 + c;
-                    const bool ok = (unsigned)iy < (unsigned)H && (unsigned)ix < (unsigned)W;
-                    half8 v = {0, 0, 0, 0, 0, 0, 0, 0};
-                    if (ok) v = *(const half8*)(base + lds_px<UP>((iy - row0) * W + ix) * 128);
-#pragma unroll
-                    for (int e = 0; e < 8; ++e) d[c][e] = (float)v[e];
-                }
-#pragma unroll
-                for (int e = 0; e < 8; ++e) {
-                    hz[r][0][e] = d[0][e] - d[1][e];
-                    hz[r][1][e] = 2.f * d[1][e];
-                    hz[r][2][e] = d[1][e] - d[2][e];
-                }
-            }
-            const int64_t trow = (int64_t)(nb0 + img) * HW + t;
-            half_t* dst = V + trow * C + c0 + chunk * 8;
-#pragma unroll
-            for (int j = 0; j < 3; ++j) {
-                half8 o[3];
-#pragma unroll
-                for (int e = 0; e < 8; ++e) {
-                    o[0][e] = (half_t)(hz[0][j][e] - hz[1][j][e]);
-                    o[1][e] = (half_t)(2.f * hz[1][j][e]);
-                    o[2][e] = (half_t)(hz[1][j][e] - hz[2][j][e]);
-                }
-#pragma unroll
-                for (int i = 0; i < 3; ++i) *(half8*)(dst + (int64_t)(i * 3 + j) * group_rows * C) = o[i];
-            }
-        }
-        return;
-    }
-    const int th = (H + 1) >> 1, tw = (W + 1) >> 1, ntile = th * tw;
-    const int bt = (tr1 - tr0) * tw;
-    for (int it = item0; it < nimg * bt; it += 32) {
-        const int img = it / bt, tb_ = it - img * bt;
-        const int ty = tr0 + tb_ / tw, tx = tb_ - (tb_ / tw) * tw;
-        const int t = ty * tw + tx;
-        const char* base = smem + (int64_t)img * SWs * 128 + chunk * 16;
-        float hz[4][4][8];
-#pragma unroll
-        for (int r = 0; r < 4; ++r) {
-            const int iy = 2 * ty - 1 + r;
-            float d[4][8];
-#pragma unroll
-            for (int c = 0; c < 4; ++c) {
-                const int ix = 2 * tx - 1 + c;
-                const bool ok = (unsigned)iy < (unsigned)H && (unsigned)ix < (unsigned)W;
-                half8 v = {0, 0, 0, 0, 0, 0, 0, 0};
-                if (ok) v = *(const half8*)(base + lds_px<UP>((iy - row0) * W + ix) * 128);
-#pragma unroll
-                for (int e = 0; e < 8; ++e) d[c][e] = (float)v[e];
-            }
+#pragma unroll
+        for (int j = 0; j < 3; ++j) {
+            half8 m[3];
+#pragma unroll
+            for (int i = 0; i < 3; ++i) m[i] = *(const half8*)(src + (int64_t)(i * 3 + j) * group_rows * Cout);
+            const int jj = j == 2 ? 3 : j;
 #pragma unroll
             for (int e = 0; e < 8; ++e) {
-                hz[r][0][e] = d[0][e] - d[2][e];
-                hz[r][1][e] = d[1][e] + d[2][e];
-                hz[r][2][e] = d[2][e] - d[1][e];
-                hz[r][3][e] = d[1][e] - d[3][e];
-            }
-        }
-        const int64_t trow = (int64_t)(nb0 + img) * ntile + t;
-        half_t* dst = V + trow * C + c0 + chunk * 8;
+                s[0][jj][e] = (float)m[0][e] + (float)m[1][e];
+                s[1][jj][e] = (float)m[1][e] - (float)m[2][e];
+            }
+        }
+#pragma unroll
+        for (int e = 0; e < 8; ++e) s[0][2][e] = s[1][2][e] = 0.f;
+    } else {
 #pragma unroll
         for (int j = 0; j < 4; ++j) {
-            half8 o[4];
+            half8 m[4];
+#pragma unroll
+            for (int i = 0; i < 4; ++i) m[i] = *(const half8*)(src + (int64_t)(i * 4 + j) * group_rows * Cout);
 #pragma unroll
             for (int e = 0; e < 8; ++e) {
-                o[0][e] = (half_t)(hz[0][j][e] - hz[2][j][e]);
-                o[1][e] = (half_t)(hz[1][j][e] + hz[2][j][e]);
-                o[2][e] = (half_t)(hz[2][j][e] - hz[1][j][e]);
-                o[3][e] = (half_t)(hz[1][j][e] - hz[3][j][e]);
-            }
-#pragma unroll
-            for (int i = 0; i < 4; ++i) *(half8*)(dst + (int64_t)(i * 4 + j) * group_rows * C) = o[i];
-        }
-    }
-}
+                s[0][j][e] = (float)m[0][e] + (float)m[1][e] + (float)m[2][e];
+                s[1][j][e] = (float)m[1][e] - (float)m[2][e] - (float)m[3][e];
+            }
+        }
+    }
+    float b[8];
+    {
+        const float4 b0 = bias ? *(const float4*)(bias + ch) : make_float4(0.f, 0.f, 0.f, 0.f), b1 = bias ? *(const float4*)(bias + ch + 4) : make_float4(0.f, 0.f, 0.f, 0.f);
+        b[0] = b0.x; b[1] = b0.y; b[2] = b0.z; b[3] = b0.w; b[4] = b1.x; b[5] = b1.y; b[6] = b1.z; b[7] = b1.w;
+    }
+    const int64_t m00 = ((int64_t)nb * OH + 2 * ty) * OW + 2 * tx;
+    if (RB) {
+        const float* rb = row_bias + (m00 / rows_per_group) * ld_rb + ch;
+        const float4 r0 = *(const float4*)rb, r1 = *(const float4*)(rb + 4);
+        b[0] += r0.x; b[1] += r0.y; b[2] += r0.z; b[3] += r0.w; b[4] += r1.x; b[5] += r1.y; b[6] += r1.z; b[7] += r1.w;
+    }
+#pragma unroll
+    for (int i = 0; i < 2; ++i)
+#pragma unroll
+        for (int jj = 0; jj < 2; ++jj) {
+            if (!UP && (2 * ty + i >= OH || 2 * tx + jj >= OW)) continue;
+            const int64_t m = m00 + (int64_t)i * OW + jj;
+            float v[8];
+#pragma unroll
+            for (int e = 0; e < 8; ++e)
+                v[e] = (jj == 0 ? s[i][0][e] + s[i][1][e] + s[i][2][e] : s[i][1][e] - s[i][2][e] - s[i][3][e]) + b[e];
+            if (RES) {
+                const half8 r = *(const half8*)(res + m * ldr + ch);
+#pragma unroll
+                for (int e = 0; e < 8; ++e) v[e] += (float)r[e];
+            }
+#pragma unroll
+            for (int e = 0; e < 8; ++e) o[i][jj][e] = (half_t)v[e];
+            *(half8*)(y + m * ldy + ch) = o[i][jj];
+        }
+}
+
 
 template <bool RES, bool RB, bool UP>
 __global__ __launch_bounds__(256) void wino_output_kernel(const half_t* __restrict__ Mo, const float* __restrict__ bias, const float* __restrict__ row_bias,
@@ -141,106 +269,112 @@
     const int64_t idx = (int64_t)blockIdx.x * 256 + threadIdx.x;
     const int64_t tile = idx / c8;
     if (tile >= ntiles_total) return;
-    const int ch = (int)(idx - tile * c8) * 8;
-    const int th = UP ? H : (H + 1) >> 1, tw = UP ? W : (W + 1) >> 1, ntile = th * tw;
-    const int OW = UP ? 2 * W : W, OH = UP ? 2 * H : H;
-    const int nb = (int)(tile / ntile), t = (int)(tile - (int64_t)nb * ntile);
-    const int ty = t / tw, tx = t - ty * tw;
-    const half_t* src = Mo + tile * Cout + ch;
-    float s[2][4][8];
-    if constexpr (UP) {
-#pragma unroll
-        for (int j = 0; j < 3; ++j) {
-            half8 m[3];
-#pragma unroll
-            for (int i = 0; i < 3; ++i) m[i] = *(const half8*)(src + (int64_t)(i * 3 + j) * group_rows * Cout);
-            const int jj = j == 2 ? 3 : j;
-#pragma unroll
-            for (int e = 0; e < 8; ++e) {
-                s[0][jj][e] = (float)m[0][e] + (float)m[1][e];
-                s[1][jj][e] = (float)m[1][e] - (float)m[2][e];
-            }
-        }
-#pragma unroll
-        for (int e = 0; e < 8; ++e) s[0][2][e] = s[1][2][e] = 0.f;
-    } else {
-#pragma unroll
-        for (int j = 0; j < 4; ++j) {
-            half8 m[4];
-#pragma unroll
-            for (int i = 0; i < 4; ++i) m[i] = *(const half8*)(src + (int64_t)(i * 4 + j) * group_rows * Cout);
-#pragma unroll
-            for (int e = 0; e < 8; ++e) {
-                s[0][j][e] = (float)m[0][e] + (float)m[1][e] + (float)m[2][e];
-                s[1][j][e] = (float)m[1][e] - (float)m[2][e] - (float)m[3][e];
-            }
-        }
-    }
-    float b[8];
-    {
-        const float4 b0 = bias ? *(const float4*)(bias + ch) : make_float4(0.f, 0.f, 0.f, 0.f), b1 = bias ? *(const float4*)(bias + ch + 4) : make_float4(0.f, 0.f, 0.f, 0.f);
-        b[0] = b0.x; b[1] = b0.y; b[2] = b0.z; b[3] = b0.w; b[4] = b1.x; b[5] = b1.y; b[6] = b1.z; b[7] = b1.w;
-    }
-    const int64_t m00 = ((int64_t)nb * OH + 2 * ty) * OW + 2 * tx;
-    if (RB) {
-        const float* rb = row_bias + (m00 / rows_per_group) * ld_rb + ch;
-        const float4 r0 = *(const float4*)rb, r1 = *(const float4*)(rb + 4);
-        b[0] += r0.x; b[1] += r0.y; b[2] += r0.z; b[3] += r0.w; b[4] += r1.x; b[5] += r1.y; b[6] += r1.z; b[7] += r1.w;
-    }
-#pragma unroll
-    for (int i = 0; i < 2; ++i)
-#pragma unroll
-        for (int jj = 0; jj < 2; ++jj) {
-            if (!UP && (2 * ty + i >= OH || 2 * tx + jj >= OW)) continue;
-            const int64_t m = m00 + (int64_t)i * OW + jj;
-            float v[8];
-#pragma unroll
-            for (int e = 0; e < 8; ++e)
-                v[e] = (jj == 0 ? s[i][0][e] + s[i][1][e] + s[i][2][e] : s[i][1][e] - s[i][2][e] - s[i][3][e]) + b[e];
-            if (RES) {
-                const half8 r = *(const half8*)(res + m * ldr + ch);
-#pragma unroll
-                for (int e = 0; e < 8; ++e) v[e] += (float)r[e];
-            }
-            half8 o;
-#pragma unroll
-            for (int e = 0; e < 8; ++e) o[e] = (half_t)v[e];
-            *(half8*)(y + m * ldy + ch) = o;
-        }
+    half8 o[2][2];
+    wino_out_tile<RES, RB, UP>(Mo, bias, row_bias, res, y, group_rows, tile, (int)(idx - tile * c8) * 8, Cout, H, W, ld_rb, rows_per_group, ldr, ldy, o);
+}
+
+template <bool RES, bool RB>
+__global__ __launch_bounds__(256) void wino_output_gn_kernel(const half_t* __restrict__ Mo, const float* __restrict__ bias, const float* __restrict__ row_bias,
+                                                             const half_t* __restrict__ res, half_t* __restrict__ y, int64_t group_rows, int Cout, int H,
+                                                             int W, int64_t ld_rb, int rows_per_group, int64_t ldr, int64_t ldy, float* __restrict__ partials,
+                                                             int G, int nsamples, int nchunks, int TT, int64_t tiles_per_sample) {
+    extern __shared__ __attribute__((aligned(16))) char smem[];
+    const int CT = Cout >> 3, cpg = Cout / G;
+    float4* part = (float4*)smem;
+    float* shift = (float*)(part + TT * CT);
+    const int tid = threadIdx.x, tl = tid / CT, ct = tid - tl * CT, ch = ct * 8;
+    const int sample = (int)blockIdx.x / nchunks, chunk = (int)blockIdx.x - sample * nchunks;
+    const int64_t ts = (int64_t)chunk * TT + tl;
+    const bool valid = ts < tiles_per_sample;
+    const int th = (H + 1) >> 1, tw = (W + 1) >> 1, ntile = th * tw;
+    const int g0 = ch / cpg;
+    const int split = (g0 + 1) * cpg - ch;
+    half8 o[2][2];
+    if (valid) {
+        const int64_t tile = (int64_t)sample * tiles_per_sample + ts;
+        wino_out_tile<RES, RB, false>(Mo, bias, row_bias, res, y, group_rows, tile, ch, Cout, H, W, ld_rb, rows_per_group, ldr, ldy, o);
+#pragma unroll
+        for (int e = 0; e < 8; ++e)
+            if ((ch + e) % cpg == 0) shift[tl * G + (ch + e) / cpg] = (float)o[0][0][e];
+    }
+    __syncthreads();
+    float4 sq = make_float4(0.f, 0.f, 0.f, 0.f);
+    if (valid) {
+        const float k0 = shift[tl * G + g0], k1 = split < 8 ? shift[tl * G + g0 + 1] : 0.f;
+        const int t = (int)(((int64_t)sample * tiles_per_sample + ts) % ntile), ty = t / tw, tx = t - ty * tw;
+#pragma unroll
+        for (int i = 0; i < 2; ++i)
+#pragma unroll
+            for (int jj = 0; jj < 2; ++jj) {
+                if (2 * ty + i >= H || 2 * tx + jj >= W) continue;
+#pragma unroll
+                for (int e = 0; e < 8; ++e) {
+                    const float v = (float)o[i][jj][e];
+                    if (e < split) { const float d = v - k0; sq.x += d; sq.y = fmaf(d, d, sq.y); }
+                    else { const float d = v - k1; sq.z += d; sq.w = fmaf(d, d, sq.w); }
+                }
+            }
+    }
+    part[tid] = sq;
+    __syncthreads();
+    if (tid < G) {
+        const int g = tid;
+        const int c_lo = (g * cpg) >> 3, c_hi = (g * cpg + cpg - 1) >> 3;
+        float n = 0.f, mean = 0.f, m2 = 0.f;
+        for (int l = 0; l < TT; ++l) {
+            const int64_t tsl = (int64_t)chunk * TT + l;
+            if (tsl >= tiles_per_sample) break;
+            const int t = (int)(((int64_t)sample * tiles_per_sample + tsl) % ntile), ty = t / tw, tx = t - ty * tw;
+            const float nb = (float)((2 * ty + 1 < H ? 2 : 1) * (2 * tx + 1 < W ? 2 : 1) * cpg);
+            float S = 0.f, Q = 0.f;
+            for (int c = c_lo; c <= c_hi; ++c) {
+                const float4 p = part[l * CT + c];
+                const bool upper = (c * 8) / cpg != g;
+                S += upper ? p.z : p.x;
+                Q += upper ? p.w : p.y;
+            }
+            const float mb = shift[l * G + g] + S / nb, m2b = fmaxf(Q - S * S / nb, 0.f);
+            if (n == 0.f) { n = nb; mean = mb; m2 = m2b; }
+            else {
+                const float nn = n + nb, dlt = mb - mean;
+                mean += dlt * (nb / nn);
+                m2 += m2b + dlt * dlt * (n * nb / nn);
+                n = nn;
+            }
+        }
+        float* out = partials + (int64_t)nsamples * G * 2 + (((int64_t)sample * nchunks + chunk) * G + g) * 3;
+        out[0] = n;
+        out[1] = mean;
+        out[2] = m2;
+    }
 }
 
 }
 
 extern "C" int insv2v_winograd_input(const insv2v_winograd_in_desc* dp, insv2v_stream_t stream) {
+    if (!one_device()) return INSV2V_EINVAL;
     if (!dp) return INSV2V_EINVAL;
     const insv2v_winograd_in_desc& d = *dp;
     if (!d.x || !d.v || d.NB <= 0 || d.H <= 0 || d.W <= 0 || d.C <= 0) return INSV2V_EINVAL;
     if ((d.C % 64) || (d.x2 && (d.C1 <= 0 || d.C1 >= d.C || (d.C1 % 64)))) return INSV2V_EUNSUPPORTED;
     if ((d.ldx & 7) || ((uintptr_t)d.x & 15) || ((uintptr_t)d.v & 15) || (d.x2 && ((d.ldx2 & 7) || ((uintptr_t)d.x2 & 15)))) return INSV2V_EINVAL;
     if (d.gn_ab && (d.gn_images_per_sample <= 0 || ((uintptr_t)d.gn_ab & 15))) return INSV2V_EINVAL;
-    const int HW = d.H * d.W, ntile = d.upsample ? HW : ((d.H + 1) / 2) * ((d.W + 1) / 2);
-    const int HWs = d.upsample ? HW : (HW + 1) & ~1;
-    const int64_t tiles = (int64_t)d.NB * ntile;
-    if (d.v_group_rows < tiles) return INSV2V_EINVAL;
-    const int trows = d.upsample ? d.H : (d.H + 1) / 2;
-    int band_tr = trows, ipb = 1;
-    if (HWs * 128 <= 64 * 1024) {
-        ipb = 32 / ntile;
-        if (ipb < 1) ipb = 1;
-        while (ipb > 1 && ipb * HWs * 128 > 64 * 1024) --ipb;
-    } else {
-        const int max_rows = 64 * 1024 / (d.W * 128);
-        band_tr = d.upsample ? max_rows - 2 : (max_rows - 2) / 2;
-        if (band_tr < 1) return INSV2V_EUNSUPPORTED;
-    }
-    const int nbands = (trows + band_tr - 1) / band_tr;
-    const int srows = nbands == 1 ? d.H : (d.upsample ? band_tr + 2 : 2 * band_tr + 2);
-    const dim3 grid((unsigned)((d.NB + ipb - 1) / ipb), (unsigned)(d.C / 64), (unsigned)nbands);
-    const int slots = srows * d.W;
-    const size_t lds = (size_t)ipb * (d.upsample ? slots : (slots + 1) & ~1) * 128;
+    const wino_in_plan pl = wino_in_make_plan(d.NB, d.H, d.W, d.C, d.upsample);
+    if (!pl.ok) return INSV2V_EUNSUPPORTED;
+    if (d.v_group_rows < (int64_t)d.NB * pl.ntile) return INSV2V_EINVAL;
+    static int num_cu = 0;
+    if (!num_cu) {
+        int dev = 0;
+        hipDeviceProp_t prop;
+        if (hipGetDevice(&dev) != hipSuccess || hipGetDeviceProperties(&prop, dev) != hipSuccess) return INSV2V_EINVAL;
+        num_cu = prop.multiProcessorCount;
+    }
+    const dim3 grid((unsigned)wino_in_grid(pl, num_cu));
+    const size_t lds = (size_t)pl.lds;
+    const int ipb = pl.ipb, band_tr = pl.band_tr;
 #define WINO_IN(NORM, UP)                                                                                                                             \
     hipLaunchKernelGGL((wino_input_kernel<NORM, UP>), grid, dim3(256), lds, as_stream(stream), (const half_t*)d.x, (const half_t*)d.x2, d.gn_ab, (half_t*)d.v, \
-                       d.ldx, d.ldx2, d.x2 ? d.C1 : d.C, d.C, d.NB, d.H, d.W, ipb, d.gn_ab ? d.gn_images_per_sample : 1, d.gn_ab ? d.gn_silu : 0, d.v_group_rows, band_tr)
+                       d.ldx, d.ldx2, d.x2 ? d.C1 : d.C, d.C, d.NB, d.H, d.W, ipb, d.gn_ab ? d.gn_images_per_sample : 1, d.gn_ab ? d.gn_silu : 0, d.v_group_rows, band_tr, pl.nslices, pl.nbands, (int)pl.nitems)
     if (d.gn_ab) { if (d.upsample) WINO_IN(true, true); else WINO_IN(true, false); }
     else { if (d.upsample) WINO_IN(false, true); else WINO_IN(false, false); }
 #undef WINO_IN
@@ -248,6 +382,7 @@
 }
 
 extern "C" int insv2v_winograd_output(const insv2v_winograd_out_desc* dp, insv2v_stream_t stream) {
+    if (!one_device()) return INSV2V_EINVAL;
     if (!dp) return INSV2V_EINVAL;
     const insv2v_winograd_out_desc& d = *dp;
     if (!d.m || !d.y || d.NB <= 0 || d.H <= 0 || d.W <= 0 || d.Cout <= 0) return INSV2V_EINVAL;
@@ -257,6 +392,20 @@
         return INSV2V_EINVAL;
     const int64_t tiles = d.upsample ? (int64_t)d.NB * d.H * d.W : (int64_t)d.NB * ((d.H + 1) / 2) * ((d.W + 1) / 2);
     if (d.m_group_rows < tiles) return INSV2V_EINVAL;
+    if (d.gn_partials) {
+        const wino_out_gn_plan pl = wino_out_gn_make_plan(d.NB, d.H, d.W, d.Cout, d.upsample, d.gn_G, d.gn_rows_per_sample);
+        if (pl.status) return pl.status;
+        if (d.gn_nchunks != pl.nchunks || ((uintptr_t)d.gn_partials & 3)) return INSV2V_EINVAL;
+        const dim3 ggrid((unsigned)((int64_t)pl.nsamples * pl.nchunks));
+#define WINO_OUT_GN(RES, RB)                                                                                                                          \
+    hipLaunchKernelGGL((wino_output_gn_kernel<RES, RB>), ggrid, dim3(pl.threads), (size_t)pl.lds, as_stream(stream), (const half_t*)d.m, d.bias, d.row_bias, \
+                       (const half_t*)d.residual, (half_t*)d.y, d.m_group_rows, d.Cout, d.H, d.W, d.ld_rb, d.rows_per_group, d.ldr, d.ldy, d.gn_partials, \
+                       d.gn_G, pl.nsamples, pl.nchunks, pl.TT, pl.tiles_per_sample)
+        if (d.residual) { if (d.row_bias) WINO_OUT_GN(true, true); else WINO_OUT_GN(true, false); }
+        else { if (d.row_bias) WINO_OUT_GN(false, true); else WINO_OUT_GN(false, false); }
+#undef WINO_OUT_GN
+        return launch_status();
+    }
     const int64_t n = tiles * (d.Cout / 8);
     const dim3 grid((unsigned)((n + 255) / 256));
 #define WINO_OUT(RES, RB, UP)                                                                                                                        \
@@ -272,3 +421,9 @@
 #undef WINO_OUT
     return launch_status();
 }
+
+extern "C" int insv2v_winograd_out_gn_chunks(const insv2v_winograd_out_desc* dp) {
+    if (!dp) return INSV2V_EINVAL;
+    const wino_out_gn_plan pl = wino_out_gn_make_plan(dp->NB, dp->H, dp->W, dp->Cout, dp->upsample, dp->gn_G, dp->gn_rows_per_sample);
+    return pl.status ? pl.status : pl.nchunks;
+}
diff --git a/instruct-video-to-video_amd/csrc/winograd_plan.h b/instruct-video-to-video_amd/csrc/winograd_plan.h
--- /dev/null
+++ b/instruct-video-to-video_amd/csrc/winograd_plan.h
@@ -0,0 +1,88 @@
+#pragma once
+#include <cstdint>
+
+#define WINO_IN_LDS_MAX (64 * 1024)
+#define WINO_IN_WGS_PER_CU 4
+struct wino_in_plan {
+    int ok;
+    int ntile;
+    int trows;
+    int ipb, band_tr, nbands;
+    int ngroups, nslices;
+    int64_t nitems;
+    int slots;
+    int64_t lds;
+};
+
+static inline wino_in_plan wino_in_make_plan(int NB, int H, int W, int C, int upsample) {
+    wino_in_plan p = {};
+    if (NB <= 0 || H <= 0 || W <= 0 || C <= 0 || (C % 64)) return p;
+    const int64_t HW = (int64_t)H * W;
+    if (HW > (1 << 28)) return p;
+    p.ntile = upsample ? (int)HW : ((H + 1) / 2) * ((W + 1) / 2);
+    p.trows = upsample ? H : (H + 1) / 2;
+    const int64_t HWs = upsample ? HW : (HW + 1) & ~(int64_t)1;
+    p.band_tr = p.trows;
+    p.ipb = 1;
+    if (HWs * 128 <= WINO_IN_LDS_MAX) {
+        p.ipb = 32 / p.ntile;
+        if (p.ipb < 1) p.ipb = 1;
+        while (p.ipb > 1 && p.ipb * HWs * 128 > WINO_IN_LDS_MAX) --p.ipb;
+    } else {
+        const int max_rows = WINO_IN_LDS_MAX / (W * 128);
+        p.band_tr = upsample ? max_rows - 2 : (max_rows - 2) / 2;
+        if (p.band_tr < 1) return p;
+    }
+    p.nbands = (p.trows + p.band_tr - 1) / p.band_tr;
+    const int srows = p.nbands == 1 ? H : (upsample ? p.band_tr + 2 : 2 * p.band_tr + 2);
+    const int64_t slots = (int64_t)srows * W;
+    p.slots = (int)(upsample ? slots : (slots + 1) & ~(int64_t)1);
+    p.lds = (int64_t)p.ipb * p.slots * 128;
+    p.ngroups = (NB + p.ipb - 1) / p.ipb;
+    p.nslices = C / 64;
+    p.nitems = (int64_t)p.ngroups * p.nbands * p.nslices;
+    p.ok = p.lds <= WINO_IN_LDS_MAX && p.nitems < ((int64_t)1 << 31);
+    return p;
+}
+
+static inline int wino_in_grid(const wino_in_plan& p, int num_cu) {
+    int wpc = (int)((160 * 1024) / (p.lds > 0 ? p.lds : 1));
+    if (wpc > WINO_IN_WGS_PER_CU) wpc = WINO_IN_WGS_PER_CU;
+    if (wpc < 1) wpc = 1;
+    const int64_t cap = (int64_t)num_cu * wpc;
+    return (int)(p.nitems < cap ? p.nitems : cap);
+}
+
+struct wino_out_gn_plan {
+    int status;
+    int CT, TT, threads;
+    int nsamples;
+    int64_t tiles_per_sample;
+    int nchunks;
+    int64_t lds;
+};
+
+static inline wino_out_gn_plan wino_out_gn_make_plan(int NB, int H, int W, int Cout, int upsample, int G, int rows_per_sample) {
+    wino_out_gn_plan p = {};
+    p.status = -1;
+    if (NB <= 0 || H <= 0 || W <= 0 || Cout <= 0 || G <= 0 || rows_per_sample <= 0 || (Cout % G)) return p;
+    p.status = -2;
+    const int cpg = Cout / G;
+    if (upsample || (Cout & 7) || Cout > 2048 || cpg < 8) return p;
+    const int64_t HW = (int64_t)H * W;
+    if (rows_per_sample % HW) return p;
+    const int64_t images_per_sample = rows_per_sample / HW;
+    if (NB % images_per_sample) { p.status = -1; return p; }
+    p.CT = Cout / 8;
+    p.TT = 256 / p.CT < 1 ? 1 : 256 / p.CT;
+    p.threads = p.CT * p.TT;
+    if (G > p.threads) return p;
+    p.nsamples = (int)(NB / images_per_sample);
+    p.tiles_per_sample = images_per_sample * ((H + 1) / 2) * ((W + 1) / 2);
+    const int64_t nchunks = (p.tiles_per_sample + p.TT - 1) / p.TT;
+    if (nchunks * p.nsamples >= ((int64_t)1 << 31) || nchunks >= (1 << 24)) return p;
+    p.nchunks = (int)nchunks;
+    p.lds = ((int64_t)p.TT * G + (int64_t)p.threads * 4) * 4;
+    p.status = 0;
+    return p;
+}
diff --git a/instruct-video-to-video_amd/insv2v/_lib.py b/instruct-video-to-video_amd/insv2v/_lib.py
--- a/instruct-video-to-video_amd/insv2v/_lib.py
+++ b/instruct-video-to-video_amd/insv2v/_lib.py
@@ -33,7 +33,8 @@
 
 class WinogradOutDesc(C.Structure):
     _fields_ = [("m", c_p), ("bias", c_p), ("row_bias", c_p), ("residual", c_p), ("y", c_p), ("m_group_rows", c_i64),
-                ("ldr", c_i64), ("ldy", c_i64), ("ld_rb", c_i64), ("NB", c_i32), ("H", c_i32), ("W", c_i32), ("Cout", c_i32), ("rows_per_group", c_i32), ("upsample", c_i32)]
+                ("ldr", c_i64), ("ldy", c_i64), ("ld_rb", c_i64), ("NB", c_i32), ("H", c_i32), ("W", c_i32), ("Cout", c_i32), ("rows_per_group", c_i32), ("upsample", c_i32),
+                ("gn_partials", c_p), ("gn_G", c_i32), ("gn_rows_per_sample", c_i32), ("gn_nchunks", c_i32)]
 
 
 class FfnDesc(C.Structure):
@@ -62,7 +63,7 @@
     _fields_ = [("x", c_p), ("x2", c_p), ("y", c_p), ("gamma", c_p), ("beta", c_p), ("partials", c_p),
                 ("ldx", c_i64), ("ldx2", c_i64), ("ldy", c_i64),
                 ("nsamples", c_i32), ("rows_per_sample", c_i32), ("C", c_i32), ("C1", c_i32), ("G", c_i32),
-                ("nchunks", c_i32), ("silu", c_i32), ("eps", c_f32), ("ab", c_p), ("stats_only", c_i32)]
+                ("nchunks", c_i32), ("silu", c_i32), ("eps", c_f32), ("ab", c_p), ("stats_only", c_i32), ("apply_only", c_i32)]
 
 
 class LayerNormDesc(C.Structure):
@@ -114,6 +115,7 @@
     "insv2v_conv3x3_fuses_groupnorm": (c_i32, [C.POINTER(GemmDesc)]),
     "insv2v_winograd_input": (c_i32, [C.POINTER(WinogradInDesc), c_p]),
     "insv2v_winograd_output": (c_i32, [C.POINTER(WinogradOutDesc), c_p]),
+    "insv2v_winograd_out_gn_chunks": (c_i32, [C.POINTER(WinogradOutDesc)]),
     "insv2v_ffn_fused": (c_i32, [C.POINTER(FfnDesc), c_p]),
     "insv2v_ffn_stream_elems": (c_i64, [c_i32, c_i32, c_i32]),
     "insv2v_rowlin": (c_i32, [C.POINTER(RowLinDesc), c_p]),
@@ -127,6 +129,7 @@
     "insv2v_xattn_attn": (c_i32, [C.POINTER(XattnDesc), c_p]),
     "insv2v_xattn_attn_stream_elems": (c_i64, [c_i32, c_i32, c_i32]),
     "insv2v_groupnorm": (c_i32, [C.POINTER(GroupNormDesc), c_p]),
+    "insv2v_groupnorm_finalize": (c_i32, [C.POINTER(GroupNormDesc), c_p]),
     "insv2v_layernorm": (c_i32, [C.POINTER(LayerNormDesc), c_p]),
     "insv2v_layernorm_stats": (c_i32, [c_p, c_p, c_i64, c_i32, c_i32, c_f32, c_p]),
     "insv2v_attention": (c_i32, [C.POINTER(AttentionDesc), c_p]),
diff --git a/instruct-video-to-video_amd/insv2v/ops.py b/instruct-video-to-video_amd/insv2v/ops.py
--- a/instruct-video-to-video_amd/insv2v/ops.py
+++ b/instruct-video-to-video_amd/insv2v/ops.py
@@ -438,19 +438,21 @@
     return W <= 128 and cin % 64 == 0 and c1 % 64 == 0
 
 
-def winograd_conv3x3(x, geom, U, bias=None, *, x2=None, gn_ab=None, gn_images_per_sample=0, gn_silu=False, row_bias=None, rows_per_group=0,
-                     residual=None, out=None, tile=0, upsample=False):
-    lib = _lib.load()
-    _req(x, torch.float16, "winograd.x"), _req(U, torch.float16, "winograd.U")
+def winograd_tiles(geom, upsample=False):
+    NB, H, W = geom
+    tiles = NB * H * W if upsample else NB * ((H + 1) // 2) * ((W + 1) // 2)
+    return tiles, -(-tiles // 256) * 256
+
+
+def winograd_input(x, geom, *, x2=None, gn_ab=None, gn_images_per_sample=0, gn_silu=False, upsample=False):
+    lib = _lib.load()
+    _req(x, torch.float16, "winograd.x")
     NB, H, W = geom
     C1 = x.shape[1]
     C = C1 + (x2.shape[1] if x2 is not None else 0)
-    Cout = U.shape[1]
     ng = 9 if upsample else 16
-    OH, OW = (2 * H, 2 * W) if upsample else (H, W)
-    assert U.shape[0] == ng and U.shape[2] == C and x.shape[0] == NB * H * W
-    tiles = NB * H * W if upsample else NB * ((H + 1) // 2) * ((W + 1) // 2)
-    grows = -(-tiles // 256) * 256
+    assert x.shape[0] == NB * H * W
+    _, grows = winograd_tiles(geom, upsample)
     v = torch.empty((ng * grows, C), device=x.device, dtype=torch.float16)
     di = WinogradInDesc()
     di.x, di.v, di.ldx, di.v_group_rows = x.data_ptr(), v.data_ptr(), x.stride(0), grows
@@ -461,7 +463,16 @@
         di.gn_ab, di.gn_images_per_sample, di.gn_silu = _req(gn_ab, torch.float32, "winograd.gn_ab").data_ptr(), gn_images_per_sample, int(gn_silu)
     with _timed("groupnorm", 0.0, ("wino_in", NB * H * W, C)):
         check(lib.insv2v_winograd_input(_byref(di), _stream()), "insv2v_winograd_input")
-    m = torch.empty((ng * grows, Cout), device=x.device, dtype=torch.float16)
+    return v
+
+
+def winograd_gemm(v, U, geom, *, tile=0, upsample=False):
+    lib = _lib.load()
+    NB, H, W = geom
+    ng, Cout, C = U.shape
+    OH, OW = (2 * H, 2 * W) if upsample else (H, W)
+    _, grows = winograd_tiles(geom, upsample)
+    m = torch.empty((ng * grows, Cout), device=v.device, dtype=torch.float16)
     d = GemmDesc()
     d.a, d.w, d.c = v.data_ptr(), U.data_ptr(), m.data_ptr()
     d.lda, d.ldw, d.ldc = C, C, Cout
@@ -469,9 +480,12 @@
     d.w_group_rows, d.w_group_stride = grows, Cout * C
     with _timed("gemm_kernel", 2.0 * NB * OH * OW * Cout * 9 * C, ("wino_gemm", ng * grows, Cout, C)):
         check(lib.insv2v_gemm(_byref(d), _stream()), "insv2v_gemm (grouped)")
-    del v
-    if out is None:
-        out = torch.empty((NB * OH * OW, Cout), device=x.device, dtype=torch.float16)
+    return m
+
+
+def _winograd_out_desc(m, geom, out, bias, row_bias, rows_per_group, residual, upsample):
+    NB, H, W = geom
+    _, grows = winograd_tiles(geom, upsample)
     do = WinogradOutDesc()
     do.m, do.y, do.m_group_rows, do.ldy = m.data_ptr(), out.data_ptr(), grows, out.stride(0)
     if bias is not None:
@@ -480,10 +494,78 @@
         do.row_bias, do.ld_rb, do.rows_per_group = _req(row_bias, torch.float32, "winograd.row_bias").data_ptr(), row_bias.stride(0), rows_per_group
     if residual is not None:
         do.residual, do.ldr = _req(residual, torch.float16, "winograd.residual").data_ptr(), residual.stride(0)
-    do.NB, do.H, do.W, do.Cout, do.upsample = NB, H, W, Cout, int(upsample)
+    do.NB, do.H, do.W, do.Cout, do.upsample = NB, H, W, m.shape[1], int(upsample)
+    return do
+
+
+def winograd_emit_chunks(geom, Cout, groups, rows_per_sample, upsample=False):
+    do = WinogradOutDesc()
+    do.NB, do.H, do.W = geom
+    do.Cout, do.upsample, do.gn_G, do.gn_rows_per_sample = Cout, int(upsample), groups, rows_per_sample
+    n = int(_lib.load().insv2v_winograd_out_gn_chunks(_byref(do)))
+    return n if n > 0 else 0
+
+
+def winograd_output(m, geom, bias=None, *, row_bias=None, rows_per_group=0, residual=None, out=None, upsample=False, emit_gn=None):
+    lib = _lib.load()
+    _req(m, torch.float16, "winograd.m")
+    NB, H, W = geom
+    Cout = m.shape[1]
+    OH, OW = (2 * H, 2 * W) if upsample else (H, W)
+    if out is None:
+        out = torch.empty((NB * OH * OW, Cout), device=m.device, dtype=torch.float16)
+    do = _winograd_out_desc(m, geom, out, bias, row_bias, rows_per_group, residual, upsample)
+    scratch = None
+    if emit_gn is not None:
+        gamma, beta, groups, eps, nsamples, rows_per_sample = emit_gn
+        assert nsamples * rows_per_sample == NB * OH * OW
+        nchunks = winograd_emit_chunks(geom, Cout, groups, rows_per_sample, upsample)
+        if nchunks:
+            scratch = torch.empty(nsamples * groups * (2 + 3 * nchunks), device=m.device, dtype=torch.float32)
+            do.gn_partials, do.gn_G, do.gn_rows_per_sample, do.gn_nchunks = scratch.data_ptr(), groups, rows_per_sample, nchunks
     with _timed("groupnorm", 0.0, ("wino_out", NB * OH * OW, Cout)):
-        check(lib.insv2v_winograd_output(_byref(do), _stream()), "insv2v_winograd_output")
-    return out
+        rc = lib.insv2v_winograd_output(_byref(do), _stream())
+        if rc == -2 and scratch is not None:
+            scratch, do.gn_partials = None, None
+            rc = lib.insv2v_winograd_output(_byref(do), _stream())
+        check(rc, "insv2v_winograd_output")
+    if emit_gn is None:
+        return out
+    if scratch is None:
+        return out, groupnorm_stats(out, nsamples, rows_per_sample, gamma, beta, groups, eps)
+    ab = torch.empty((nsamples, Cout, 2), device=m.device, dtype=torch.float32)
+    d = GroupNormDesc()
+    d.gamma, d.beta, d.partials, d.ab = gamma.data_ptr(), beta.data_ptr(), scratch.data_ptr(), ab.data_ptr()
+    d.nsamples, d.rows_per_sample, d.C, d.G, d.nchunks, d.eps = nsamples, rows_per_sample, Cout, groups, nchunks, eps
+    with _timed("groupnorm", 0.0, ("gnstats", nsamples, rows_per_sample, Cout)):
+        check(lib.insv2v_groupnorm_finalize(_byref(d), _stream()), "insv2v_groupnorm_finalize")
+    return out, ab
+
+
+def winograd_conv3x3(x, geom, U, bias=None, *, x2=None, gn_ab=None, gn_images_per_sample=0, gn_silu=False, row_bias=None, rows_per_group=0,
+                     residual=None, out=None, tile=0, upsample=False, emit_gn=None):
+    _req(x, torch.float16, "winograd.x"), _req(U, torch.float16, "winograd.U")
+    C = x.shape[1] + (x2.shape[1] if x2 is not None else 0)
+    assert U.shape[0] == (9 if upsample else 16) and U.shape[2] == C
+    v = winograd_input(x, geom, x2=x2, gn_ab=gn_ab, gn_images_per_sample=gn_images_per_sample, gn_silu=gn_silu, upsample=upsample)
+    m = winograd_gemm(v, U, geom, tile=tile, upsample=upsample)
+    del v
+    return winograd_output(m, geom, bias, row_bias=row_bias, rows_per_group=rows_per_group, residual=residual, out=out, upsample=upsample, emit_gn=emit_gn)
+
+
+def groupnorm_apply(x, nsamples, rows_per_sample, ab, groups, silu=False):
+    lib = _lib.load()
+    _req(x, torch.float16, "groupnorm.x"), _req(ab, torch.float32, "groupnorm.ab")
+    C = x.shape[1]
+    assert nsamples * rows_per_sample == x.shape[0] and tuple(ab.shape) == (nsamples, C, 2)
+    y = torch.empty((x.shape[0], C), device=x.device, dtype=torch.float16)
+    d = GroupNormDesc()
+    d.x, d.y, d.ab = x.data_ptr(), y.data_ptr(), ab.data_ptr()
+    d.ldx, d.ldy = x.stride(0), y.stride(0)
+    d.nsamples, d.rows_per_sample, d.C, d.G, d.silu, d.apply_only = nsamples, rows_per_sample, C, groups, int(silu), 1
+    with _timed("groupnorm", 0.0, ("gn", nsamples, rows_per_sample, C)):
+        check(lib.insv2v_groupnorm(_byref(d), _stream()), "insv2v_groupnorm(apply_only)")
+    return y
 
 
 def groupnorm(x, nsamples, rows_per_sample, gamma, beta, groups, eps, silu=False, x2=None):
diff --git a/instruct-video-to-video_amd/insv2v/unet.py b/instruct-video-to-video_amd/insv2v/unet.py
--- a/instruct-video-to-video_amd/insv2v/unet.py
+++ b/instruct-video-to-video_amd/insv2v/unet.py
@@ -16,6 +16,7 @@
 WINOGRAD_MIN_CIN = int(os.environ.get("INSV2V_WINOGRAD_MIN_CIN", "1280"))
 WINOGRAD_MIN_ROWS = int(os.environ.get("INSV2V_WINOGRAD_MIN_ROWS", "4608"))
 WINOGRAD_UP_MIN_CIN = int(os.environ.get("INSV2V_WINOGRAD_UP_MIN_CIN", "640"))
+WINOGRAD_EMIT_GN = os.environ.get("INSV2V_WINOGRAD_EMIT_GN", "1") != "0"
 MERGE_FF2_POST = os.environ.get("INSV2V_MERGE_FF2_POST", "1") != "0"
 NARROW_CONV_OUT = os.environ.get("INSV2V_NARROW_CONV_OUT", "1") != "0"
 NARROW_CONV_MIN_ROWS = int(os.environ.get("INSV2V_NARROW_CONV_MIN_ROWS", "16384"))
@@ -157,9 +158,14 @@
         c1 = x.t.shape[1]
         tb = temb_all[:, self.temb_slice[0]:self.temb_slice[1]]
         wino = x.t.shape[0] >= WINOGRAD_MIN_ROWS
+        ab2 = None
         if self.u1 is not None and wino and ops.winograd_ok(geom, self.cin, c1 if x2 is not None else 0):
             ab = ops.groupnorm_stats(x.t, x.B, rows, *self.n1, self.groups, self.eps, x2=x2)
-            h = ops.winograd_conv3x3(x.t, geom, self.u1, self.b1, x2=x2, gn_ab=ab, gn_images_per_sample=x.F, gn_silu=True, row_bias=tb, rows_per_group=rows)
+            emit = (*self.n2, self.groups, self.eps, x.B, rows) if WINOGRAD_EMIT_GN and ops.winograd_emit_chunks(geom, self.cout, self.groups, rows) else None
+            h = ops.winograd_conv3x3(x.t, geom, self.u1, self.b1, x2=x2, gn_ab=ab, gn_images_per_sample=x.F, gn_silu=True, row_bias=tb, rows_per_group=rows,
+                                     emit_gn=emit)
+            if emit is not None:
+                h, ab2 = h
         elif FUSE_GN and ops.conv3x3_fuses_groupnorm(geom, self.cin, self.cout, c1 if x2 is not None else 0):
             ab = ops.groupnorm_stats(x.t, x.B, rows, *self.n1, self.groups, self.eps, x2=x2)
             h, _ = ops.conv3x3(x.t, geom, self.w1, self.b1, x2=x2, row_bias=tb, rows_per_group=rows,
@@ -172,13 +178,14 @@
         else:
             res = x.t
         if self.u2 is not None and wino and ops.winograd_ok(geom, self.cout):
-            ab = ops.groupnorm_stats(h, x.B, rows, *self.n2, self.groups, self.eps)
+            ab = ab2 if ab2 is not None else ops.groupnorm_stats(h, x.B, rows, *self.n2, self.groups, self.eps)
             out = ops.winograd_conv3x3(h, geom, self.u2, self.b2, gn_ab=ab, gn_images_per_sample=x.F, gn_silu=True, residual=res, out=out)
         elif FUSE_GN and ops.conv3x3_fuses_groupnorm(geom, self.cout, self.cout):
-            ab = ops.groupnorm_stats(h, x.B, rows, *self.n2, self.groups, self.eps)
+            ab = ab2 if ab2 is not None else ops.groupnorm_stats(h, x.B, rows, *self.n2, self.groups, self.eps)
             out, _ = ops.conv3x3(h, geom, self.w2, self.b2, residual=res, gn_ab=ab, gn_images_per_sample=x.F, gn_silu=True, out=out)
         else:
-            n = ops.groupnorm(h, x.B, rows, *self.n2, self.groups, self.eps, silu=True)
+            n = (ops.groupnorm_apply(h, x.B, rows, ab2, self.groups, silu=True) if ab2 is not None
+                 else ops.groupnorm(h, x.B, rows, *self.n2, self.groups, self.eps, silu=True))
             out, _ = ops.conv3x3(n, geom, self.w2, self.b2, residual=res, out=out)
         return x.like(out)
 
```

Result: no change. 16.19 frames/s (-0.6%).
